# TravisWheelerLab/sufr

Hardware: AMD Instinct MI355X
Metric: suffixes sorted/sec (SA+LCP) (higher is better)
Workload: dtype u8 text / u32 indices / u64 packed keys; 1 GPU; syn_human 3.1 Gb stand-in for GRCh38, --dna --ignore-softmask -n 256 (BASELINE configs[3]); text_len=3100000001, num_suffixes=1500223556, parallelism=prefix-bucket shards x1, bits_per_char=3, radix_passes=5, digit_bits=15, levels=7, deep_records=58357696, placement_trials=3

## Files before the change

include/sufr_hip.h:

```cpp
#ifndef SUFR_HIP_H
#define SUFR_HIP_H

#include <stddef.h>
#include <stdint.h>

#ifdef __cplusplus
extern "C" {
#endif

#define SUFR_HIP_ABI_VERSION 3

#define SUFR_OUTFILE_VERSION 6
#define SUFR_SENTINEL_CHARACTER '$'

#define SUFR_HIP_FLAG_DNA              (1u << 0)
#define SUFR_HIP_FLAG_ALLOW_AMBIGUITY  (1u << 1)
#define SUFR_HIP_FLAG_IGNORE_SOFTMASK  (1u << 2)
#define SUFR_HIP_FLAG_RAW_TEXT         (1u << 3)

#define SUFR_HIP_OK              0
#define SUFR_HIP_E_INVALID      -1
#define SUFR_HIP_E_NO_DEVICE    -2
#define SUFR_HIP_E_HIP          -3
#define SUFR_HIP_E_NOMEM        -4
#define SUFR_HIP_E_CAPACITY     -5
#define SUFR_HIP_E_UNSUPPORTED  -6
#define SUFR_HIP_E_IO           -7
#define SUFR_HIP_E_CONFLICT     -8
#define SUFR_HIP_E_SEED_MASK    -9

typedef struct sufr_hip_ctx sufr_hip_ctx;

typedef struct sufr_hip_stats {
    uint64_t text_len;
    uint64_t num_suffixes;
    uint32_t alphabet_size;
    uint32_t bits_per_char;
    uint32_t chars_per_key;
    uint32_t digit_bits;
    uint32_t num_passes;
    uint32_t num_levels;
    uint64_t num_large_groups;
    uint64_t deep_records;
    uint32_t top_lo, top_hi;
    uint32_t partition_workgroups;
    uint32_t partition_variant;
    float ms_total;
    float ms_normalize;
    float ms_hist_text;
    float ms_partition;
    float ms_passes;
    float ms_finish;
    float ms_deep;
    float host_read_s;
    float host_build_s;
    float host_write_s;
    uint32_t num_exceptions;
    float ms_exceptions;
    uint64_t num_reinserted;
} sufr_hip_stats;

int  sufr_hip_abi_version(void);
int  sufr_hip_device_count(void);
sufr_hip_ctx *sufr_hip_create(int device_id);
void sufr_hip_destroy(sufr_hip_ctx *ctx);
const char *sufr_hip_last_error(const sufr_hip_ctx *ctx);
int  sufr_hip_set_stream(sufr_hip_ctx *ctx, void *hip_stream);
int  sufr_hip_synchronize(sufr_hip_ctx *ctx);
int  sufr_hip_set_window(sufr_hip_ctx *ctx, uint64_t window, uint64_t margin);
int  sufr_hip_set_window_retry(sufr_hip_ctx *ctx, uint64_t widest_margin);
uint64_t sufr_hip_window_repairs(const sufr_hip_ctx *ctx);
int  sufr_hip_set_array_budget(sufr_hip_ctx *ctx, uint64_t bytes);
int  sufr_hip_set_overlap_min(sufr_hip_ctx *ctx, uint64_t min_records);
int  sufr_hip_overlapped(const sufr_hip_ctx *ctx);
uint64_t sufr_hip_doublings(const sufr_hip_ctx *ctx);
int  sufr_hip_set_exc_max_affected(sufr_hip_ctx *ctx, uint64_t max_affected);
int  sufr_hip_exc_retry(const sufr_hip_ctx *ctx);
uint64_t sufr_hip_exc_taken(const sufr_hip_ctx *ctx);

int sufr_hip_normalize(const uint8_t *in, uint8_t *out, uint64_t n, int ignore_softmask);

int sufr_hip_sort_device_u32(sufr_hip_ctx *ctx, const void *d_text, uint64_t n, uint32_t flags,
                             uint64_t max_query_len, const char *seed_mask,
                             uint64_t num_partitions, uint64_t random_seed,
                             uint32_t shard_index, uint32_t num_shards,
                             void *d_sa, void *d_lcp, uint64_t cap,
                             uint64_t *num_suffixes_out, sufr_hip_stats *stats);
int sufr_hip_sort_device_u64(sufr_hip_ctx *ctx, const void *d_text, uint64_t n, uint32_t flags,
                             uint64_t max_query_len, const char *seed_mask,
                             uint64_t num_partitions, uint64_t random_seed,
                             uint32_t shard_index, uint32_t num_shards,
                             void *d_sa, void *d_lcp, uint64_t cap,
                             uint64_t *num_suffixes_out, sufr_hip_stats *stats);

int sufr_hip_stitch_device_u32(sufr_hip_ctx *ctx, uint64_t n, const uint64_t *d_bounds, uint32_t shard_index,
                               uint32_t num_shards, void *d_lcp);
int sufr_hip_stitch_device_u64(sufr_hip_ctx *ctx, uint64_t n, const uint64_t *d_bounds, uint32_t shard_index,
                               uint32_t num_shards, void *d_lcp);

int sufr_hip_build_u32(sufr_hip_ctx *ctx, const uint8_t *text, uint64_t n, uint32_t flags,
                       uint64_t max_query_len, const char *seed_mask,
                       uint64_t num_partitions, uint64_t random_seed,
                       uint8_t *norm_text_out, uint32_t *sa_out, uint32_t *lcp_out, uint64_t cap,
                       uint64_t *num_suffixes_out, sufr_hip_stats *stats);
int sufr_hip_build_u64(sufr_hip_ctx *ctx, const uint8_t *text, uint64_t n, uint32_t flags,
                       uint64_t max_query_len, const char *seed_mask,
                       uint64_t num_partitions, uint64_t random_seed,
                       uint8_t *norm_text_out, uint64_t *sa_out, uint64_t *lcp_out, uint64_t cap,
                       uint64_t *num_suffixes_out, sufr_hip_stats *stats);

uint64_t sufr_hip_lcp_pair(const uint8_t *norm_text, uint64_t n, uint64_t a, uint64_t b);

typedef struct sufr_sequence_data {
    uint8_t  *seq;
    uint64_t  seq_len;
    uint64_t *start_positions;
    char    **sequence_names;
    uint64_t  num_sequences;
} sufr_sequence_data;
int  sufr_read_sequence_file(const char *path, uint8_t sequence_delimiter, sufr_sequence_data *out,
                             char *err, size_t errlen);
void sufr_sequence_data_free(sufr_sequence_data *d);

int sufr_write_file(const char *path, int is_dna, int allow_ambiguity, int ignore_softmask,
                    const uint8_t *norm_text, uint64_t text_len, int index_width,
                    const void *sa, const void *lcp, uint64_t num_suffixes,
                    int has_max_query_len, uint64_t max_query_len, const char *seed_mask,
                    const uint64_t *sequence_starts, uint64_t num_sequences,
                    const char *const *sequence_names, char *err, size_t errlen);

typedef struct sufr_create_args {
    const char *input;
    const char *output;
    uint64_t    num_partitions;
    int         has_max_query_len;
    uint64_t    max_query_len;
    int         is_dna;
    int         allow_ambiguity;
    int         ignore_softmask;
    uint8_t     sequence_delimiter;
    const char *seed_mask;
    uint64_t    random_seed;
} sufr_create_args;
int sufr_hip_create_file(sufr_hip_ctx *ctx, const sufr_create_args *args, char *path_out,
                         size_t path_out_len, sufr_hip_stats *stats);
int sufr_hip_create_from_sequence(sufr_hip_ctx *ctx, const sufr_sequence_data *seq,
                                  const sufr_create_args *args, char *path_out, size_t path_out_len,
                                  sufr_hip_stats *stats);


typedef struct sufr_shard_info {
    uint64_t num_suffixes;
    uint64_t first_suffix;
    uint64_t last_suffix;
} sufr_shard_info;
int sufr_hip_shard_build(sufr_hip_ctx *ctx, const sufr_sequence_data *seq, const sufr_create_args *args,
                         uint32_t shard_index, uint32_t num_shards, sufr_shard_info *info, sufr_hip_stats *stats);
int sufr_write_frame(const char *outfile, const sufr_sequence_data *seq, const sufr_create_args *args,
// ... 15 lines not shown
```

sufr_amd/_lib.py:

```python
from __future__ import annotations

import ctypes as C
import os
import subprocess
from pathlib import Path

CSRC = Path(__file__).resolve().parent / "csrc"
LIB_PATH = CSRC / "_build" / "libsufr_hip.so"
if os.environ.get("SUFR_AMD_PROBES_LIB"):
    import sys as _sys
    LIB_PATH = CSRC / "_build" / "libsufr_hip_probes.so"
    print(f"sufr_amd: SUFR_AMD_PROBES_LIB is set -- loading the PROBES build {LIB_PATH.name} (tuning knobs from "
          "SUFR_PROBE_*; for profiling only)", file=_sys.stderr)
CLI_PATH = CSRC / "_build" / "sufr"
HOST_ASAN = bool(os.environ.get("SUFR_AMD_HOST_ASAN_LIB"))
if HOST_ASAN:
    import sys as _sys
    LIB_PATH = CSRC / "_build" / "libsufr_host_asan.so"
    CLI_PATH = CSRC / "_build" / "sufr_host_asan"
    print(f"sufr_amd: SUFR_AMD_HOST_ASAN_LIB is set -- loading the host-only sanitizer build {LIB_PATH.name} (no device code)",
          file=_sys.stderr)


class SufrHipError(RuntimeError):
    def __init__(self, code: int, message: str):
        super().__init__(f"{message} (sufr_hip error {code})")
        self.code = code
        self.message = message


class Stats(C.Structure):
    _fields_ = [
        ("text_len", C.c_uint64), ("num_suffixes", C.c_uint64),
        ("alphabet_size", C.c_uint32), ("bits_per_char", C.c_uint32), ("chars_per_key", C.c_uint32),
        ("digit_bits", C.c_uint32), ("num_passes", C.c_uint32), ("num_levels", C.c_uint32),
        ("num_large_groups", C.c_uint64), ("deep_records", C.c_uint64),
        ("top_lo", C.c_uint32), ("top_hi", C.c_uint32), ("partition_workgroups", C.c_uint32),
        ("partition_variant", C.c_uint32),
        ("ms_total", C.c_float), ("ms_normalize", C.c_float), ("ms_hist_text", C.c_float),
        ("ms_partition", C.c_float), ("ms_passes", C.c_float), ("ms_finish", C.c_float),
        ("ms_deep", C.c_float), ("host_read_s", C.c_float), ("host_build_s", C.c_float),
        ("host_write_s", C.c_float),
        ("num_exceptions", C.c_uint32), ("ms_exceptions", C.c_float), ("num_reinserted", C.c_uint64),
    ]

    def as_dict(self):
        return {n: getattr(self, n) for n, _ in self._fields_}


class SequenceData(C.Structure):
    _fields_ = [("seq", C.POINTER(C.c_uint8)), ("seq_len", C.c_uint64),
                ("start_positions", C.POINTER(C.c_uint64)), ("sequence_names", C.POINTER(C.c_char_p)),
                ("num_sequences", C.c_uint64)]


class CreateArgs(C.Structure):
    _fields_ = [("input", C.c_char_p), ("output", C.c_char_p), ("num_partitions", C.c_uint64),
                ("has_max_query_len", C.c_int), ("max_query_len", C.c_uint64), ("is_dna", C.c_int),
                ("allow_ambiguity", C.c_int), ("ignore_softmask", C.c_int), ("sequence_delimiter", C.c_uint8),
                ("seed_mask", C.c_char_p), ("random_seed", C.c_uint64)]


class ShardInfo(C.Structure):
    _fields_ = [("num_suffixes", C.c_uint64), ("first_suffix", C.c_uint64), ("last_suffix", C.c_uint64)]


FLAG_DNA, FLAG_ALLOW_AMBIGUITY, FLAG_IGNORE_SOFTMASK, FLAG_RAW_TEXT = 1, 2, 4, 8
FLAG_NO_PREFIX_TABLE = 0x100
FLAG_SA_U64 = 0x200

EXPORTS = [
    "sufr_hip_abi_version", "sufr_hip_device_count", "sufr_hip_create", "sufr_hip_destroy",
    "sufr_hip_last_error", "sufr_hip_set_stream", "sufr_hip_synchronize", "sufr_hip_set_window", "sufr_hip_set_window_retry", "sufr_hip_set_array_budget", "sufr_hip_window_repairs", "sufr_hip_set_overlap_min", "sufr_hip_overlapped", "sufr_hip_doublings", "sufr_hip_set_exc_max_affected", "sufr_hip_exc_retry", "sufr_hip_exc_taken", "sufr_hip_normalize", "sufr_hip_sort_device_u32",
    "sufr_hip_sort_device_u64", "sufr_hip_stitch_device_u32", "sufr_hip_stitch_device_u64", "sufr_hip_build_u32", "sufr_hip_build_u64", "sufr_hip_lcp_pair",
    "sufr_read_sequence_file", "sufr_sequence_data_free", "sufr_write_file", "sufr_hip_create_file", "sufr_hip_create_from_sequence",
    "sufr_hip_shard_build", "sufr_write_frame", "sufr_hip_shard_write", "sufr_hip_create_from_sequence_multi",
    "sufr_hip_create_file_multi",
]
QUERY_EXPORTS = [
    "sufr_file_open", "sufr_file_close", "sufr_file_metadata", "sufr_file_text", "sufr_file_seed_mask",
    "sufr_file_suffix_array", "sufr_file_lcp_array", "sufr_file_suffix", "sufr_file_lcp", "sufr_file_sequence_start",
    "sufr_file_sequence_name", "sufr_file_sequence_of", "sufr_file_search", "sufr_file_search_batch",
    "sufr_hip_index_load", "sufr_hip_index_wrap", "sufr_hip_index_free", "sufr_hip_index_width", "sufr_hip_search_batch",
    "sufr_hip_search_batch_device", "sufr_hip_locate_batch_device",
]
MATCH_EXPORTS = [
    "sufr_file_matching_stats", "sufr_file_smems", "sufr_hip_matching_stats_device", "sufr_hip_smems_device", "sufr_hip_smems",
]
MEM_EXPORTS = ["sufr_file_mems", "sufr_hip_mems_device", "sufr_hip_mems"]
MEM_BOTH_STRANDS = 0x1
APPROX_EXPORTS = ["sufr_file_approx", "sufr_hip_approx_device", "sufr_hip_approx"]
APPROX_BOTH_STRANDS = 0x1
EDIT_EXPORTS = ["sufr_file_edit", "sufr_hip_edit_device", "sufr_hip_edit"]
EDIT_BOTH_STRANDS = 0x1
EDIT_LOCAL_MINIMA = 0x2
ALIGN_EXPORTS = ["sufr_file_edit_trace", "sufr_hip_edit_trace_device", "sufr_hip_edit_trace", "sufr_hip_set_trace_scratch"]
KMER_EXPORTS = ["sufr_file_kmers", "sufr_file_unique_lengths", "sufr_hip_kmers_device", "sufr_hip_unique_lengths_device",
                "sufr_hip_set_kmer_tile"]
KMER_BY_POSITION = 0x1


class KmerStats(C.Structure):
    _fields_ = [("whole", C.c_uint64), ("distinct", C.c_uint64), ("unique", C.c_uint64), ("max_count", C.c_uint64)]

    def as_dict(self):
        return {n: int(getattr(self, n)) for n, _ in self._fields_}


REPEAT_EXPORTS = ["sufr_file_repeats", "sufr_hip_repeats_device", "sufr_hip_set_repeat_tile"]
REPEAT_KINDS = {"branching": 0, "maximal": 1, "super": 2, "supermaximal": 2}


class RepeatStats(C.Structure):
    _fields_ = [("records", C.c_uint64), ("longest", C.c_uint64), ("longest_rank", C.c_uint64), ("max_count", C.c_uint64)]

    def as_dict(self):
        return {n: int(getattr(self, n)) for n, _ in self._fields_}


LZ_EXPORTS = ["sufr_file_lpf", "sufr_file_lz", "sufr_hip_lpf_device", "sufr_hip_lz_device", "sufr_hip_set_lz_tile"]


class LzStats(C.Structure):
    _fields_ = [("factors", C.c_uint64), ("literals", C.c_uint64), ("longest", C.c_uint64), ("longest_start", C.c_uint64)]

    def as_dict(self):
        return {n: int(getattr(self, n)) for n, _ in self._fields_}


SHARED_EXPORTS = ["sufr_file_shared", "sufr_file_common", "sufr_hip_shared_device", "sufr_hip_common_device"]


class SharedStats(C.Structure):
    _fields_ = [("records", C.c_uint64), ("longest", C.c_uint64), ("longest_rank", C.c_uint64), ("max_count", C.c_uint64),
                ("max_seqs", C.c_uint64)]

    def as_dict(self):
        return {n: int(getattr(self, n)) for n, _ in self._fields_}


BWT_EXPORTS = ["sufr_file_bwt", "sufr_file_bwt_runs", "sufr_file_lf", "sufr_hip_bwt_device", "sufr_hip_bwt_runs_device", "sufr_hip_lf_device",
               "sufr_hip_set_bwt_tile"]


class BwtStats(C.Structure):
    _fields_ = [("runs", C.c_uint64), ("records", C.c_uint64), ("longest", C.c_uint64), ("longest_rank", C.c_uint64)]

    def as_dict(self):
        return {n: int(getattr(self, n)) for n, _ in self._fields_}


class FileMeta(C.Structure):
    _fields_ = [("version", C.c_uint8), ("is_dna", C.c_uint8), ("allow_ambiguity", C.c_uint8),
                ("ignore_softmask", C.c_uint8), ("index_width", C.c_int),
                ("text_len", C.c_uint64), ("text_pos", C.c_uint64), ("suffix_array_pos", C.c_uint64),
                ("lcp_pos", C.c_uint64), ("len_suffixes", C.c_uint64), ("max_query_len", C.c_uint64),
                ("num_sequences", C.c_uint64), ("seed_mask_len", C.c_uint64), ("file_size", C.c_uint64),
                ("modified", C.c_int64)]

_lib = None


def build_extension(verbose: bool = False) -> Path:
    r = subprocess.run(["make", "-C", str(CSRC)] + (["asan"] if HOST_ASAN else []), capture_output=True, text=True)
    if r.returncode != 0:
        raise RuntimeError("building libsufr_hip.so failed:\n" + r.stdout + r.stderr)
    if verbose:
        print(r.stdout)
    return LIB_PATH


def lib() -> C.CDLL:
    global _lib
    if _lib is not None:
        return _lib
    if not LIB_PATH.exists():
        raise SufrHipError(-2, f"{LIB_PATH} is missing: build it with sufr_amd.build_extension() "
                               "(there is no CPU fallback)")
    import sys
    if "torch" not in sys.modules and not HOST_ASAN:
        try:
            import torch
        except ImportError:
            pass
    L = C.CDLL(str(LIB_PATH))
    vp, u64, u32, cp = C.c_void_p, C.c_uint64, C.c_uint32, C.c_char_p
    L.sufr_hip_abi_version.restype = C.c_int
    L.sufr_hip_device_count.restype = C.c_int
    L.sufr_hip_create.argtypes = [C.c_int]; L.sufr_hip_create.restype = vp
    L.sufr_hip_destroy.argtypes = [vp]; L.sufr_hip_destroy.restype = None
    L.sufr_hip_last_error.argtypes = [vp]; L.sufr_hip_last_error.restype = cp
    L.sufr_hip_set_stream.argtypes = [vp, vp]; L.sufr_hip_set_stream.restype = C.c_int
    L.sufr_hip_synchronize.argtypes = [vp]; L.sufr_hip_synchronize.restype = C.c_int
    L.sufr_hip_set_window.argtypes = [vp, u64, u64]; L.sufr_hip_set_window.restype = C.c_int
    L.sufr_hip_set_window_retry.argtypes = [vp, u64]; L.sufr_hip_set_window_retry.restype = C.c_int
    L.sufr_hip_set_array_budget.argtypes = [vp, u64]; L.sufr_hip_set_array_budget.restype = C.c_int
    L.sufr_hip_window_repairs.argtypes = [vp]; L.sufr_hip_window_repairs.restype = u64
    L.sufr_hip_set_overlap_min.argtypes = [vp, u64]; L.sufr_hip_set_overlap_min.restype = C.c_int
    L.sufr_hip_overlapped.argtypes = [vp]; L.sufr_hip_overlapped.restype = C.c_int
    L.sufr_hip_doublings.argtypes = [vp]; L.sufr_hip_doublings.restype = u64
    L.sufr_hip_set_exc_max_affected.argtypes = [vp, u64]; L.sufr_hip_set_exc_max_affected.restype = C.c_int
    L.sufr_hip_exc_retry.argtypes = [vp]; L.sufr_hip_exc_retry.restype = C.c_int
    L.sufr_hip_exc_taken.argtypes = [vp]; L.sufr_hip_exc_taken.restype = u64
    L.sufr_hip_normalize.argtypes = [vp, vp, u64, C.c_int]; L.sufr_hip_normalize.restype = C.c_int
    dev_sig = [vp, vp, u64, u32, u64, cp, u64, u64, u32, u32, vp, vp, u64, C.POINTER(u64), C.POINTER(Stats)]
    L.sufr_hip_sort_device_u32.argtypes = dev_sig; L.sufr_hip_sort_device_u32.restype = C.c_int
    L.sufr_hip_sort_device_u64.argtypes = dev_sig; L.sufr_hip_sort_device_u64.restype = C.c_int
    host_sig = [vp, vp, u64, u32, u64, cp, u64, u64, vp, vp, vp, u64, C.POINTER(u64), C.POINTER(Stats)]
    L.sufr_hip_build_u32.argtypes = host_sig; L.sufr_hip_build_u32.restype = C.c_int
    L.sufr_hip_build_u64.argtypes = host_sig; L.sufr_hip_build_u64.restype = C.c_int
    L.sufr_hip_lcp_pair.argtypes = [vp, u64, u64, u64]; L.sufr_hip_lcp_pair.restype = u64
    L.sufr_hip_stitch_device_u32.argtypes = [vp, u64, vp, u32, u32, vp]; L.sufr_hip_stitch_device_u32.restype = C.c_int
    L.sufr_hip_stitch_device_u64.argtypes = [vp, u64, vp, u32, u32, vp]; L.sufr_hip_stitch_device_u64.restype = C.c_int
    L.sufr_read_sequence_file.argtypes = [cp, C.c_uint8, C.POINTER(SequenceData), cp, C.c_size_t]
    L.sufr_read_sequence_file.restype = C.c_int
    L.sufr_sequence_data_free.argtypes = [C.POINTER(SequenceData)]; L.sufr_sequence_data_free.restype = None
    L.sufr_write_file.argtypes = [cp, C.c_int, C.c_int, C.c_int, vp, u64, C.c_int, vp, vp, u64, C.c_int, u64, cp,
                                  vp, u64, C.POINTER(cp), cp, C.c_size_t]
    L.sufr_write_file.restype = C.c_int
    L.sufr_hip_create_file.argtypes = [vp, C.POINTER(CreateArgs), cp, C.c_size_t, C.POINTER(Stats)]
    L.sufr_hip_create_file.restype = C.c_int
    L.sufr_hip_create_from_sequence.argtypes = [vp, C.POINTER(SequenceData), C.POINTER(CreateArgs), cp, C.c_size_t,
                                                C.POINTER(Stats)]
    L.sufr_hip_create_from_sequence.restype = C.c_int
    L.sufr_hip_shard_build.argtypes = [vp, C.POINTER(SequenceData), C.POINTER(CreateArgs), u32, u32,
                                       C.POINTER(ShardInfo), C.POINTER(Stats)]
    L.sufr_hip_shard_build.restype = C.c_int
    L.sufr_write_frame.argtypes = [cp, C.POINTER(SequenceData), C.POINTER(CreateArgs), u64, cp, C.c_size_t]
    L.sufr_write_frame.restype = C.c_int
    L.sufr_hip_shard_write.argtypes = [vp, C.POINTER(SequenceData), C.POINTER(CreateArgs), cp, u64, u64, u64, C.c_int,
                                       u64, C.c_int]
    L.sufr_hip_shard_write.restype = C.c_int
    L.sufr_hip_create_from_sequence_multi.argtypes = [C.POINTER(vp), C.c_int, C.POINTER(SequenceData),
                                                      C.POINTER(CreateArgs), cp, C.c_size_t, C.POINTER(Stats)]
    L.sufr_hip_create_from_sequence_multi.restype = C.c_int
    L.sufr_hip_create_file_multi.argtypes = [C.POINTER(vp), C.c_int, C.POINTER(CreateArgs), cp, C.c_size_t,
                                             C.POINTER(Stats)]
    L.sufr_hip_create_file_multi.restype = C.c_int
    L.sufr_file_open.argtypes = [cp, C.POINTER(vp), cp, C.c_size_t]; L.sufr_file_open.restype = C.c_int
    L.sufr_file_close.argtypes = [vp]; L.sufr_file_close.restype = None
    L.sufr_file_metadata.argtypes = [vp, C.POINTER(FileMeta)]; L.sufr_file_metadata.restype = C.c_int
    for name in ("sufr_file_text", "sufr_file_seed_mask", "sufr_file_suffix_array", "sufr_file_lcp_array"):
        getattr(L, name).argtypes = [vp]; getattr(L, name).restype = vp
    for name in ("sufr_file_suffix", "sufr_file_lcp", "sufr_file_sequence_start", "sufr_file_sequence_of"):
        getattr(L, name).argtypes = [vp, u64]; getattr(L, name).restype = u64
    L.sufr_file_sequence_name.argtypes = [vp, u64]; L.sufr_file_sequence_name.restype = cp
    L.sufr_file_search.argtypes = [vp, cp, C.c_size_t, C.c_int, u64, C.POINTER(u64), C.POINTER(u64)]
    L.sufr_file_search.restype = C.c_int
    L.sufr_file_search_batch.argtypes = [vp, vp, vp, u64, C.c_int, u64, vp, vp, C.c_int]; L.sufr_file_search_batch.restype = C.c_int
    L.sufr_hip_index_load.argtypes = [vp, vp, C.POINTER(vp)]; L.sufr_hip_index_load.restype = C.c_int
    L.sufr_hip_index_wrap.argtypes = [vp, vp, u64, vp, u64, u32, u64, cp, C.POINTER(vp)]; L.sufr_hip_index_wrap.restype = C.c_int
    L.sufr_hip_index_free.argtypes = [vp]; L.sufr_hip_index_free.restype = None
    L.sufr_hip_index_width.argtypes = [vp]; L.sufr_hip_index_width.restype = C.c_int
    L.sufr_hip_search_batch.argtypes = [vp, vp, vp, vp, u64, C.c_int, u64, vp, vp]; L.sufr_hip_search_batch.restype = C.c_int
    L.sufr_hip_search_batch_device.argtypes = [vp, vp, vp, vp, u64, C.c_int, u64, vp, vp]
    L.sufr_hip_search_batch_device.restype = C.c_int
    L.sufr_hip_locate_batch_device.argtypes = [vp, vp, vp, vp, u64, u64, vp, vp, u64, C.POINTER(u64)]
    L.sufr_hip_locate_batch_device.restype = C.c_int
    L.sufr_file_matching_stats.argtypes = [vp, vp, vp, u64, vp, C.c_int]; L.sufr_file_matching_stats.restype = C.c_int
    L.sufr_file_smems.argtypes = [vp, vp, vp, u64, u32, u64, vp, vp, vp, vp, vp, C.POINTER(u64), C.c_int]
    L.sufr_file_smems.restype = C.c_int
    L.sufr_hip_matching_stats_device.argtypes = [vp, vp, vp, vp, u64, vp]; L.sufr_hip_matching_stats_device.restype = C.c_int
    L.sufr_hip_smems_device.argtypes = [vp, vp, vp, vp, u64, u32, vp, u64, vp, vp, vp, vp, vp, C.POINTER(u64)]
    L.sufr_hip_smems_device.restype = C.c_int
    L.sufr_hip_smems.argtypes = [vp, vp, vp, vp, u64, u32, u64, vp, vp, vp, vp, vp, C.POINTER(u64)]
    L.sufr_hip_smems.restype = C.c_int
    L.sufr_file_mems.argtypes = [vp, vp, vp, u64, u32, u64, u32, u64, vp, vp, vp, vp, vp, C.POINTER(u64), C.c_int]
    L.sufr_file_mems.restype = C.c_int
    L.sufr_hip_mems_device.argtypes = [vp, vp, vp, vp, u64, u32, u64, u32, u64, vp, vp, vp, vp, vp, C.POINTER(u64)]
    L.sufr_hip_mems_device.restype = C.c_int
    L.sufr_hip_mems.argtypes = [vp, vp, vp, vp, u64, u32, u64, u32, u64, vp, vp, vp, vp, vp, C.POINTER(u64)]
    L.sufr_hip_mems.restype = C.c_int
    L.sufr_file_approx.argtypes = [vp, vp, vp, u64, u32, u64, u32, u64, vp, vp, vp, vp, C.POINTER(u64), C.c_int]
    L.sufr_file_approx.restype = C.c_int
    L.sufr_hip_approx_device.argtypes = [vp, vp, vp, vp, u64, u32, u64, u32, u64, vp, vp, vp, vp, C.POINTER(u64)]
    L.sufr_hip_approx_device.restype = C.c_int
    L.sufr_hip_approx.argtypes = [vp, vp, vp, vp, u64, u32, u64, u32, u64, vp, vp, vp, vp, C.POINTER(u64)]
    L.sufr_hip_approx.restype = C.c_int
    L.sufr_file_edit.argtypes = [vp, vp, vp, u64, u32, u64, u32, u64, vp, vp, vp, vp, C.POINTER(u64), C.c_int]
    L.sufr_file_edit.restype = C.c_int
    L.sufr_hip_edit_device.argtypes = [vp, vp, vp, vp, u64, u32, u64, u32, u64, vp, vp, vp, vp, C.POINTER(u64)]
    L.sufr_hip_edit_device.restype = C.c_int
    L.sufr_hip_edit.argtypes = [vp, vp, vp, vp, u64, u32, u64, u32, u64, vp, vp, vp, vp, C.POINTER(u64)]
# ... 24 lines not shown
    L.sufr_hip_set_lz_tile.argtypes = [vp, u64, u64]; L.sufr_hip_set_lz_tile.restype = C.c_int
    L.sufr_file_shared.argtypes = [vp, u32, u64, u64, u64, u64, u64, u64, vp, vp, vp, vp, C.POINTER(u64), C.POINTER(SharedStats), C.c_int]
    L.sufr_file_shared.restype = C.c_int
    L.sufr_file_common.argtypes = [vp, vp, C.c_int]; L.sufr_file_common.restype = C.c_int
    L.sufr_hip_shared_device.argtypes = [vp, vp, vp, vp, u64, u32, u64, u64, u64, u64, u64, u64, vp, vp, vp, vp, C.POINTER(u64),
                                         C.POINTER(SharedStats)]
    L.sufr_hip_shared_device.restype = C.c_int
    L.sufr_hip_common_device.argtypes = [vp, vp, vp, vp, u64, vp]; L.sufr_hip_common_device.restype = C.c_int
    L.sufr_file_bwt.argtypes = [vp, vp, vp, C.c_int]; L.sufr_file_bwt.restype = C.c_int
    L.sufr_file_bwt_runs.argtypes = [vp, u64, u64, vp, vp, vp, vp, C.POINTER(u64), C.POINTER(BwtStats), C.c_int]; L.sufr_file_bwt_runs.restype = C.c_int
    L.sufr_file_lf.argtypes = [vp, vp, C.c_int]; L.sufr_file_lf.restype = C.c_int
    L.sufr_hip_bwt_device.argtypes = [vp, vp, vp, vp]; L.sufr_hip_bwt_device.restype = C.c_int
    L.sufr_hip_bwt_runs_device.argtypes = [vp, vp, u64, u64, vp, vp, vp, vp, C.POINTER(u64), C.POINTER(BwtStats)]
    L.sufr_hip_bwt_runs_device.restype = C.c_int
    L.sufr_hip_lf_device.argtypes = [vp, vp, vp]; L.sufr_hip_lf_device.restype = C.c_int
    L.sufr_hip_set_bwt_tile.argtypes = [vp, u64]; L.sufr_hip_set_bwt_tile.restype = C.c_int
    _lib = L
    return L


class Context:

    def __init__(self, device: int = 0):
        L = lib()
        self._h = L.sufr_hip_create(device)
        if not self._h:
            raise SufrHipError(-2, L.sufr_hip_last_error(None).decode())
        self.device = device

    def close(self):
        if getattr(self, "_h", None):
            lib().sufr_hip_destroy(self._h)
            self._h = None

    def __del__(self):
        try:
            self.close()
        except Exception:
            pass

    def check(self, rc: int):
        if rc != 0:
            raise SufrHipError(rc, lib().sufr_hip_last_error(self._h).decode())

    def set_window(self, window: int = 0, margin: int = 0):
        self.check(lib().sufr_hip_set_window(self._h, window, margin))

    def set_window_retry(self, widest_margin: int = 0):
        self.check(lib().sufr_hip_set_window_retry(self._h, widest_margin))

    def set_array_budget(self, nbytes: int = 0):
        self.check(lib().sufr_hip_set_array_budget(self._h, nbytes))

    def set_trace_scratch(self, nbytes: int = 0):
        self.check(lib().sufr_hip_set_trace_scratch(self._h, nbytes))

    def set_kmer_tile(self, ranks: int = 0):
        self.check(lib().sufr_hip_set_kmer_tile(self._h, ranks))

    def set_repeat_tile(self, ranks: int = 0):
        self.check(lib().sufr_hip_set_repeat_tile(self._h, ranks))

    def set_lz_tile(self, ranks: int = 0, positions: int = 0):
        self.check(lib().sufr_hip_set_lz_tile(self._h, ranks, positions))

    def set_bwt_tile(self, ranks: int = 0):
        self.check(lib().sufr_hip_set_bwt_tile(self._h, ranks))

    @property
    def window_repairs(self) -> int:
        return int(lib().sufr_hip_window_repairs(self._h))

    def set_overlap_min(self, min_records: int = 0):
        self.check(lib().sufr_hip_set_overlap_min(self._h, min_records))

    @property
    def overlapped(self) -> int:
        return int(lib().sufr_hip_overlapped(self._h))

    @property
    def doublings(self) -> int:
        return int(lib().sufr_hip_doublings(self._h))

    def set_exc_max_affected(self, max_affected: int = 0):
        self.check(lib().sufr_hip_set_exc_max_affected(self._h, max_affected))

    @property
    def exc_retry(self) -> int:
        return int(lib().sufr_hip_exc_retry(self._h))

    @property
    def exc_taken(self) -> int:
        return int(lib().sufr_hip_exc_taken(self._h))

    def synchronize(self):
        self.check(lib().sufr_hip_synchronize(self._h))

    @property
    def handle(self):
        return self._h
```

sufr_amd/csrc/sufr_capi.inc:

```

struct sufr_hip_ctx {
    sufr::Pipeline pl;
    uint64_t wide_window = 0, wide_margin = 0;
    uint64_t array_budget = 0;
    sufr::DevBuf wtext, wsa, wlcp, wblk;
    sufr::DevBuf mtmp, mpoff, mbytes;
    sufr::DevBuf xq, xoff, xlo, xhi, xcand, xsum;
    sufr::DevBuf ecnt, ekeys, ekeys2, ehist;
    sufr::DevBuf tsc, trows, tmisc;
    uint64_t trace_scratch = 0;
    sufr::DevBuf kbits, ksum, kstarts;
    std::vector<uint64_t> kmer_starts;
    uint32_t kmer_tile = 0;
    sufr::DevBuf rell, rpyr, rbits, rsum;
    uint32_t repeat_tile = 0;
    sufr::DevBuf lzpyr, lzarr, lztab, lzsum;
    uint32_t lz_rank_tile = 0, lz_pos_tile = 0;
    sufr::DevBuf bwtbytes, bwtsum, bwttab;
    uint32_t bwt_tile = 0;
    sufr::DevBuf shkeys, shhist, shpre, shsum;
    bool wide(uint64_t n) const { return n >= sufr::SUFR_MAX_TEXT_LEN || (wide_window && n > wide_window); }
};

#include <atomic>
// ... 170 lines not shown
        delete ctx;
        return nullptr;
    }
    return ctx;
}

extern "C" void sufr_io_release_ctx_(const sufr_hip_ctx* ctx);

void sufr_hip_destroy(sufr_hip_ctx* ctx)
{
    if (!ctx) return;
    sufr_io_release_ctx_(ctx);
    (void)hipSetDevice(ctx->pl.device);
    for (sufr::DevBuf* b : {&ctx->wtext, &ctx->wsa, &ctx->wlcp, &ctx->wblk, &ctx->mtmp, &ctx->mpoff, &ctx->mbytes,
                            &ctx->xq, &ctx->xoff, &ctx->xlo, &ctx->xhi, &ctx->xcand, &ctx->xsum,
                            &ctx->ecnt, &ctx->ekeys, &ctx->ekeys2, &ctx->ehist, &ctx->tsc, &ctx->trows, &ctx->tmisc,
                            &ctx->kbits, &ctx->ksum, &ctx->kstarts, &ctx->rell, &ctx->rpyr, &ctx->rbits, &ctx->rsum,
                            &ctx->lzpyr, &ctx->lzarr, &ctx->lztab, &ctx->lzsum,
                            &ctx->bwtbytes, &ctx->bwtsum, &ctx->bwttab,
                            &ctx->shkeys, &ctx->shhist, &ctx->shpre, &ctx->shsum}) ctx->pl.release(*b);
    ctx->pl.destroy();
    delete ctx;
}

const char* sufr_hip_last_error(const sufr_hip_ctx* ctx)
{
    return ctx ? ctx->pl.err.c_str() : g_create_error.c_str();
}

int sufr_hip_is_wide_(const sufr_hip_ctx* ctx, uint64_t n) { return ctx && ctx->wide(n) ? 1 : 0; }
int sufr_hip_ctx_device_(const sufr_hip_ctx* ctx) { return ctx ? ctx->pl.device : -1; }

void sufr_hip_set_error_(sufr_hip_ctx* ctx, const char* msg)
{
    if (ctx) ctx->pl.set_error(msg ? msg : "");
}

int sufr_hip_set_stream(sufr_hip_ctx* ctx, void* hip_stream)
{
    if (!ctx) return SUFR_HIP_E_INVALID;
    if (ctx->pl.own_stream && ctx->pl.stream) (void)hipStreamDestroy(ctx->pl.stream);
    ctx->pl.own_stream = false;
    ctx->pl.stream = (hipStream_t)hip_stream;
    return 0;
}

int sufr_hip_set_window(sufr_hip_ctx* ctx, uint64_t window, uint64_t margin)
{
    if (!ctx) return SUFR_HIP_E_INVALID;
    if (window && window < 16) { ctx->pl.set_error("window below 16 positions"); return SUFR_HIP_E_INVALID; }
    ctx->wide_window = window;
    ctx->wide_margin = margin;
    return 0;
}

int sufr_hip_set_array_budget(sufr_hip_ctx* ctx, uint64_t bytes)
{
    if (!ctx) return SUFR_HIP_E_INVALID;
    ctx->array_budget = bytes;
    return 0;
}

uint64_t sufr_hip_array_budget_(const sufr_hip_ctx* ctx) { return ctx ? ctx->array_budget : 0; }

int sufr_hip_set_window_retry(sufr_hip_ctx* ctx, uint64_t widest_margin)
{
    if (!ctx) return SUFR_HIP_E_INVALID;
    ctx->pl.opt_wide_retry = widest_margin;
    return 0;
}

uint64_t sufr_hip_window_repairs(const sufr_hip_ctx* ctx) { return ctx ? ctx->pl.wide_orphans : 0; }

int sufr_hip_set_overlap_min(sufr_hip_ctx* ctx, uint64_t min_records)
{
    if (!ctx) return SUFR_HIP_E_INVALID;
    ctx->pl.opt_overlap_min = min_records;
    return 0;
}

int sufr_hip_overlapped(const sufr_hip_ctx* ctx) { return ctx ? (int)ctx->pl.last_overlapped : 0; }
uint64_t sufr_hip_doublings(const sufr_hip_ctx* ctx) { return ctx ? ctx->pl.last_doublings : 0; }

int sufr_hip_set_exc_max_affected(sufr_hip_ctx* ctx, uint64_t max_affected)
{
    if (!ctx) return SUFR_HIP_E_INVALID;
    if (max_affected > sufr::Pipeline::EXC_MAX_AFFECTED_DEFAULT) {
        ctx->pl.set_error("max_affected " + std::to_string(max_affected) + " > 2^22: the whole-text sort of the affected suffixes and its buffers are sized for 2^22");
        return SUFR_HIP_E_INVALID;
    }
    ctx->pl.opt_exc_max_affected = max_affected;
    return 0;
}

int sufr_hip_exc_retry(const sufr_hip_ctx* ctx) { return ctx ? (int)ctx->pl.last_exc_retry : 0; }
uint64_t sufr_hip_exc_taken(const sufr_hip_ctx* ctx) { return ctx ? ctx->pl.last_exc_taken : 0; }

int sufr_hip_synchronize(sufr_hip_ctx* ctx)
{
    if (!ctx) return SUFR_HIP_E_INVALID;
    if (hipSetDevice(ctx->pl.device) != hipSuccess || hipStreamSynchronize(ctx->pl.stream) != hipSuccess) {
        ctx->pl.set_error("hipStreamSynchronize failed");
        return SUFR_HIP_E_HIP;
    }
    return 0;
}

int sufr_hip_sort_device_u32(sufr_hip_ctx* ctx, const void* d_text, uint64_t n, uint32_t flags,
                             uint64_t max_query_len, const char* seed_mask, uint64_t num_partitions,
                             uint64_t random_seed, uint32_t shard_index, uint32_t num_shards, void* d_sa,
                             void* d_lcp, uint64_t cap, uint64_t* num_suffixes_out, sufr_hip_stats* stats)
{
    (void)num_partitions; (void)random_seed;
    if (!ctx) return SUFR_HIP_E_INVALID;
    ctx->pl.err.clear();
    int rc = take_options(ctx, max_query_len, seed_mask);
    if (rc) return rc;
    if (ctx->wide(n)) {
        if (n >= 0xFFFFFFFFull) { ctx->pl.set_error("text_len >= 2^32 - 1 takes the u64 entry points (suffix_array.rs:461)"); return SUFR_HIP_E_INVALID; }
        if (num_shards == 0 || shard_index >= num_shards) { ctx->pl.set_error("bad shard index"); return SUFR_HIP_E_INVALID; }
        ctx->pl.wide_shard_index = shard_index; ctx->pl.wide_num_shards = num_shards;
        rc = sufr::sort_device_wide<uint32_t>(ctx->pl, d_text, n, flags, ctx->wide_window, ctx->wide_margin, (uint32_t*)d_sa,
                                              (uint32_t*)d_lcp, cap, num_suffixes_out, stats, ctx->wtext, ctx->wsa, ctx->wlcp, ctx->wblk);
        ctx->pl.wide_shard_index = 0; ctx->pl.wide_num_shards = 1;
        return rc;
    }
    return ctx->pl.sort_device_u32(d_text, n, flags, shard_index, num_shards, (uint32_t*)d_sa, (uint32_t*)d_lcp,
                                   cap, num_suffixes_out, stats);
}

int sufr_hip_sort_device_u64(sufr_hip_ctx* ctx, const void* d_text, uint64_t n, uint32_t flags,
                             uint64_t max_query_len, const char* seed_mask, uint64_t num_partitions,
                             uint64_t random_seed, uint32_t shard_index, uint32_t num_shards, void* d_sa,
                             void* d_lcp, uint64_t cap, uint64_t* num_suffixes_out, sufr_hip_stats* stats)
{
    (void)num_partitions; (void)random_seed;
    if (!ctx) return SUFR_HIP_E_INVALID;
    ctx->pl.err.clear();
    int rc = take_options(ctx, max_query_len, seed_mask);
    if (rc) return rc;
    sufr::Pipeline& pl = ctx->pl;
    if (ctx->wide(n)) {
        if (num_shards == 0 || shard_index >= num_shards) { pl.set_error("bad shard index"); return SUFR_HIP_E_INVALID; }
        pl.wide_shard_index = shard_index; pl.wide_num_shards = num_shards;
        rc = sufr::sort_device_wide<uint64_t>(pl, d_text, n, flags, ctx->wide_window, ctx->wide_margin, (uint64_t*)d_sa,
                                              (uint64_t*)d_lcp, cap, num_suffixes_out, stats, ctx->wtext, ctx->wsa, ctx->wlcp, ctx->wblk);
        pl.wide_shard_index = 0; pl.wide_num_shards = 1;
        return rc;
    }
    if (hipSetDevice(pl.device) != hipSuccess) { pl.set_error("hipSetDevice failed"); return SUFR_HIP_E_HIP; }
    uint64_t cap32 = cap < n ? cap : n;
    if ((rc = pl.ensure(pl.sa32, cap32 * 4 + 4))) return rc;
    if ((rc = pl.ensure(pl.lcp32, cap32 * 4 + 4))) return rc;
    uint64_t s = 0;
    rc = pl.sort_device_u32(d_text, n, flags, shard_index, num_shards, (uint32_t*)pl.sa32.p, (uint32_t*)pl.lcp32.p,
                            cap32, &s, stats);
    if (num_suffixes_out) *num_suffixes_out = s;
    if (rc) return rc;
    if (s) {
        hipLaunchKernelGGL(sufr::k_widen, dim3((uint32_t)((s + 255) / 256)), dim3(256), 0, pl.stream,
                           (const uint32_t*)pl.sa32.p, (uint64_t*)d_sa, s);
        hipLaunchKernelGGL(sufr::k_widen, dim3((uint32_t)((s + 255) / 256)), dim3(256), 0, pl.stream,
                           (const uint32_t*)pl.lcp32.p, (uint64_t*)d_lcp, s);
        if (hipStreamSynchronize(pl.stream) != hipSuccess) { pl.set_error("widen failed"); return SUFR_HIP_E_HIP; }
    }
    return 0;
// ... 244 lines not shown
```

sufr_amd/csrc/sufr_host_stubs.cpp:

```cpp
#include <stdint.h>
#include <stddef.h>
#include <string>

#include <hip/hip_runtime_api.h>

#include "../../include/sufr_hip.h"
#include "../../include/sufr_query.h"
#include "../../include/sufr_match.h"
#include "../../include/sufr_mem.h"
#include "../../include/sufr_approx.h"
#include "../../include/sufr_edit.h"
#include "../../include/sufr_align.h"
#include "../../include/sufr_kmer.h"
#include "../../include/sufr_repeat.h"
#include "../../include/sufr_lz.h"
#include "../../include/sufr_shared.h"
#include "../../include/sufr_bwt.h"

struct sufr_hip_ctx { std::string err; };

namespace {
const char* const NO_DEVICE = "host-only sanitizer build: no HIP device (libsufr_host_asan.so has no device code)";
int no_device(sufr_hip_ctx* ctx) { if (ctx) ctx->err = NO_DEVICE; return SUFR_HIP_E_NO_DEVICE; }
}

extern "C" {

hipError_t hipHostMalloc(void** p, size_t, unsigned int) { if (p) *p = nullptr; return hipErrorNoDevice; }
hipError_t hipHostFree(void*) { return hipSuccess; }
const char* hipGetErrorString(hipError_t) { return "no device"; }
hipError_t hipMalloc(void** p, size_t) { if (p) *p = nullptr; return hipErrorNoDevice; }
hipError_t hipFree(void*) { return hipSuccess; }
hipError_t hipMemcpy(void*, const void*, size_t, hipMemcpyKind) { return hipErrorNoDevice; }
hipError_t hipMemcpyAsync(void*, const void*, size_t, hipMemcpyKind, hipStream_t) { return hipErrorNoDevice; }
hipError_t hipSetDevice(int) { return hipErrorNoDevice; }
hipError_t hipStreamCreateWithFlags(hipStream_t* s, unsigned int) { if (s) *s = nullptr; return hipErrorNoDevice; }
hipError_t hipStreamDestroy(hipStream_t) { return hipSuccess; }
hipError_t hipStreamSynchronize(hipStream_t) { return hipErrorNoDevice; }

int sufr_hip_abi_version(void) { return SUFR_HIP_ABI_VERSION; }
int sufr_hip_device_count(void) { return 0; }
sufr_hip_ctx* sufr_hip_create(int) { return nullptr; }
void sufr_hip_destroy(sufr_hip_ctx* ctx) { delete ctx; }
const char* sufr_hip_last_error(const sufr_hip_ctx* ctx) { return ctx ? ctx->err.c_str() : NO_DEVICE; }
int sufr_hip_set_stream(sufr_hip_ctx* ctx, void*) { return no_device(ctx); }
int sufr_hip_synchronize(sufr_hip_ctx* ctx) { return no_device(ctx); }
int sufr_hip_set_window(sufr_hip_ctx* ctx, uint64_t, uint64_t) { return no_device(ctx); }
int sufr_hip_set_window_retry(sufr_hip_ctx* ctx, uint64_t) { return no_device(ctx); }
int sufr_hip_set_array_budget(sufr_hip_ctx* ctx, uint64_t) { return no_device(ctx); }
uint64_t sufr_hip_window_repairs(const sufr_hip_ctx*) { return 0; }
int sufr_hip_set_overlap_min(sufr_hip_ctx* ctx, uint64_t) { return no_device(ctx); }
int sufr_hip_overlapped(const sufr_hip_ctx*) { return 0; }
uint64_t sufr_hip_doublings(const sufr_hip_ctx*) { return 0; }
int sufr_hip_set_exc_max_affected(sufr_hip_ctx* ctx, uint64_t) { return no_device(ctx); }
int sufr_hip_exc_retry(const sufr_hip_ctx*) { return 0; }
uint64_t sufr_hip_exc_taken(const sufr_hip_ctx*) { return 0; }
int sufr_hip_sort_device_u32(sufr_hip_ctx* ctx, const void*, uint64_t, uint32_t, uint64_t, const char*, uint64_t, uint64_t,
                             uint32_t, uint32_t, void*, void*, uint64_t, uint64_t*, sufr_hip_stats*) { return no_device(ctx); }
int sufr_hip_sort_device_u64(sufr_hip_ctx* ctx, const void*, uint64_t, uint32_t, uint64_t, const char*, uint64_t, uint64_t,
                             uint32_t, uint32_t, void*, void*, uint64_t, uint64_t*, sufr_hip_stats*) { return no_device(ctx); }
int sufr_hip_stitch_device_u32(sufr_hip_ctx* ctx, uint64_t, const uint64_t*, uint32_t, uint32_t, void*) { return no_device(ctx); }
int sufr_hip_stitch_device_u64(sufr_hip_ctx* ctx, uint64_t, const uint64_t*, uint32_t, uint32_t, void*) { return no_device(ctx); }
int sufr_hip_build_u32(sufr_hip_ctx* ctx, const uint8_t*, uint64_t, uint32_t, uint64_t, const char*, uint64_t, uint64_t, uint8_t*,
                       uint32_t*, uint32_t*, uint64_t, uint64_t*, sufr_hip_stats*) { return no_device(ctx); }
int sufr_hip_build_u64(sufr_hip_ctx* ctx, const uint8_t*, uint64_t, uint32_t, uint64_t, const char*, uint64_t, uint64_t, uint8_t*,
                       uint64_t*, uint64_t*, uint64_t, uint64_t*, sufr_hip_stats*) { return no_device(ctx); }

void sufr_hip_set_error_(sufr_hip_ctx* ctx, const char* msg) { if (ctx) ctx->err = msg ? msg : ""; }
int sufr_hip_is_wide_(const sufr_hip_ctx*, uint64_t) { return 0; }
int sufr_hip_ctx_device_(const sufr_hip_ctx*) { return -1; }
uint64_t sufr_hip_array_budget_(const sufr_hip_ctx*) { return 0; }
void sufr_hip_release_build_arrays_(sufr_hip_ctx*, int) {}
void sufr_hip_release_wide_arrays_(sufr_hip_ctx*) {}
int sufr_hip_build_resident_(sufr_hip_ctx* ctx, const uint8_t*, uint64_t, uint32_t, uint64_t, const char*, uint32_t, uint32_t,
                             uint64_t*, sufr_hip_stats*, int*, const void**, const void**, const void**) { return no_device(ctx); }
int sufr_hip_resident_ends_(sufr_hip_ctx* ctx, uint64_t, uint64_t*, uint64_t*) { return no_device(ctx); }
int sufr_hip_resident_stitch_(sufr_hip_ctx* ctx, uint64_t, uint64_t, uint64_t*) { return no_device(ctx); }
int sufr_hip_resident_arrays_(sufr_hip_ctx* ctx, int*, const void**, const void**, const void**) { return no_device(ctx); }

struct sufr_hip_index { int unused; };
int sufr_hip_index_load(sufr_hip_ctx* ctx, const sufr_file*, sufr_hip_index** out) { if (out) *out = nullptr; return no_device(ctx); }
int sufr_hip_index_wrap(sufr_hip_ctx* ctx, const void*, uint64_t, const void*, uint64_t, uint32_t, uint64_t, const char*,
                        sufr_hip_index** out) { if (out) *out = nullptr; return no_device(ctx); }
void sufr_hip_index_free(sufr_hip_index*) {}
int sufr_hip_index_width(const sufr_hip_index*) { return 0; }
int sufr_hip_search_batch(sufr_hip_ctx* ctx, const sufr_hip_index*, const uint8_t*, const uint64_t*, uint64_t, int, uint64_t,
                          uint64_t*, uint64_t*) { return no_device(ctx); }
int sufr_hip_search_batch_device(sufr_hip_ctx* ctx, const sufr_hip_index*, const void*, const void*, uint64_t, int, uint64_t,
                                 void*, void*) { return no_device(ctx); }
int sufr_hip_locate_batch_device(sufr_hip_ctx* ctx, const sufr_hip_index*, const void*, const void*, uint64_t, uint64_t, void*,
                                 void*, uint64_t, uint64_t*) { return no_device(ctx); }


int sufr_hip_matching_stats_device(sufr_hip_ctx* ctx, const sufr_hip_index*, const void*, const void*, uint64_t, void*) { return no_device(ctx); }
int sufr_hip_smems_device(sufr_hip_ctx* ctx, const sufr_hip_index*, const void*, const void*, uint64_t, uint32_t, void*, uint64_t, void*,
                          void*, void*, void*, void*, uint64_t* total_out) { if (total_out) *total_out = 0; return no_device(ctx); }
int sufr_hip_smems(sufr_hip_ctx* ctx, const sufr_hip_index*, const uint8_t*, const uint64_t*, uint64_t, uint32_t, uint64_t, uint64_t*,
                   uint32_t*, uint32_t*, uint64_t*, uint64_t*, uint64_t* total_out) { if (total_out) *total_out = 0; return no_device(ctx); }

int sufr_hip_mems_device(sufr_hip_ctx* ctx, const sufr_hip_index*, const void*, const void*, uint64_t, uint32_t, uint64_t, uint32_t,
                         uint64_t, void*, void*, void*, void*, void*, uint64_t* total_out) { if (total_out) *total_out = 0; return no_device(ctx); }
int sufr_hip_mems(sufr_hip_ctx* ctx, const sufr_hip_index*, const uint8_t*, const uint64_t*, uint64_t, uint32_t, uint64_t, uint32_t, uint64_t,
                  uint64_t*, uint32_t*, uint8_t*, uint32_t*, uint64_t*, uint64_t* total_out) { if (total_out) *total_out = 0; return no_device(ctx); }

int sufr_hip_approx_device(sufr_hip_ctx* ctx, const sufr_hip_index*, const void*, const void*, uint64_t, uint32_t, uint64_t, uint32_t,
                           uint64_t, void*, void*, void*, void*, uint64_t* total_out) { if (total_out) *total_out = 0; return no_device(ctx); }
int sufr_hip_approx(sufr_hip_ctx* ctx, const sufr_hip_index*, const uint8_t*, const uint64_t*, uint64_t, uint32_t, uint64_t, uint32_t, uint64_t,
                    uint64_t*, uint8_t*, uint64_t*, uint8_t*, uint64_t* total_out) { if (total_out) *total_out = 0; return no_device(ctx); }

int sufr_hip_edit_device(sufr_hip_ctx* ctx, const sufr_hip_index*, const void*, const void*, uint64_t, uint32_t, uint64_t, uint32_t,
                         uint64_t, void*, void*, void*, void*, uint64_t* total_out) { if (total_out) *total_out = 0; return no_device(ctx); }
int sufr_hip_edit(sufr_hip_ctx* ctx, const sufr_hip_index*, const uint8_t*, const uint64_t*, uint64_t, uint32_t, uint64_t, uint32_t, uint64_t,
                  uint64_t*, uint8_t*, uint64_t*, uint8_t*, uint64_t* total_out) { if (total_out) *total_out = 0; return no_device(ctx); }

int sufr_hip_edit_trace_device(sufr_hip_ctx* ctx, const sufr_hip_index*, const void*, const void*, uint64_t, uint64_t, const void*, const void*,
                               const void*, const void*, uint64_t, void*, void*, void*, uint64_t* total_out) { if (total_out) *total_out = 0; return no_device(ctx); }
int sufr_hip_edit_trace(sufr_hip_ctx* ctx, const sufr_hip_index*, const uint8_t*, const uint64_t*, uint64_t, uint64_t, const uint64_t*, const uint8_t*,
                        const uint64_t*, const uint8_t*, uint64_t, uint64_t*, uint64_t*, uint32_t*, uint64_t* total_out) { if (total_out) *total_out = 0; return no_device(ctx); }
int sufr_hip_set_trace_scratch(sufr_hip_ctx* ctx, uint64_t) { return no_device(ctx); }

int sufr_hip_kmers_device(sufr_hip_ctx* ctx, const sufr_hip_index*, const void*, const uint64_t*, uint64_t, uint64_t, uint32_t, uint64_t, void*,
                          void*, sufr_kmer_stats* stats_out) { if (stats_out) *stats_out = sufr_kmer_stats{0, 0, 0, 0}; return no_device(ctx); }
int sufr_hip_unique_lengths_device(sufr_hip_ctx* ctx, const sufr_hip_index*, const void*, const uint64_t*, uint64_t, uint32_t, void*) { return no_device(ctx); }
int sufr_hip_set_kmer_tile(sufr_hip_ctx* ctx, uint64_t) { return no_device(ctx); }

int sufr_hip_repeats_device(sufr_hip_ctx* ctx, const sufr_hip_index*, const void*, const uint64_t*, uint64_t, uint32_t, uint64_t, uint64_t, uint64_t,
                            uint64_t, void*, void*, void*, uint64_t* total_out, sufr_repeat_stats* stats_out)
{
    if (total_out) *total_out = 0;
    if (stats_out) *stats_out = sufr_repeat_stats{0, 0, 0, 0};
    return no_device(ctx);
}
int sufr_hip_set_repeat_tile(sufr_hip_ctx* ctx, uint64_t) { return no_device(ctx); }

int sufr_hip_lpf_device(sufr_hip_ctx* ctx, const sufr_hip_index*, const void*, const uint64_t*, uint64_t, void*, void*) { return no_device(ctx); }
int sufr_hip_lz_device(sufr_hip_ctx* ctx, const sufr_hip_index*, const void*, const uint64_t*, uint64_t, uint64_t, void*, void*, void*,
// ... 30 lines not shown
```

sufr_amd/csrc/sufr_kernels.hip:

```cpp

#include <hip/hip_runtime.h>
#include <stdint.h>
#include <type_traits>

#include "sufr_device.h"
#include "sufr_runkey.h"

namespace sufr {
#ifdef SUFR_HIP_PROBES
__device__ unsigned long long g_phase[3][16];
#define SUFR_STAMP(acc, i) { const unsigned long long t__ = __builtin_amdgcn_s_memtime(); acc[i] += t__ - stamp__; stamp__ = t__; }
#define SUFR_STAMP_DECL(n) unsigned long long ph__[n] = {}; unsigned long long stamp__ = __builtin_amdgcn_s_memtime();
#define SUFR_STAMP_FLUSH(k, n) if ((threadIdx.x & 63u) == 0 && (threadIdx.x >> 6) == gridDim.y * 0 + (blockDim.x >> 6) - 1) { for (int i__ = 0; i__ < n; i__++) atomicAdd(&g_phase[k][i__], ph__[i__]); }
#else
#define SUFR_STAMP(acc, i)
#define SUFR_STAMP_DECL(n)
#define SUFR_STAMP_FLUSH(k, n)
#endif
}

namespace sufr {

static constexpr int WAVE = 64;
static_assert(RUN_TILE == (uint32_t)TILE, "run-end table granularity");

__device__ __forceinline__ uint32_t lane_id() { return threadIdx.x & 63u; }
__device__ __forceinline__ uint64_t rec_key(const Rec& r) { return ((uint64_t)r.khi << 32) | r.klo; }
__device__ __forceinline__ Rec make_rec(uint64_t key, uint32_t idx)
{
    Rec r; r.klo = (uint32_t)key; r.khi = (uint32_t)(key >> 32); r.idx = idx;
    return r;
}

#define SUFR_LDS_VOLATILE(T, p) ((__attribute__((address_space(3))) volatile T*)(p))

__device__ __forceinline__ uint64_t shfl64(uint64_t v, int src)
{
    uint32_t lo = (uint32_t)v, hi = (uint32_t)(v >> 32);
    lo = __shfl(lo, src, WAVE);
    hi = __shfl(hi, src, WAVE);
    return ((uint64_t)hi << 32) | lo;
}
__device__ __forceinline__ uint64_t shfl64_xor(uint64_t v, int m)
{
    uint32_t lo = (uint32_t)v, hi = (uint32_t)(v >> 32);
    lo = __shfl_xor(lo, m, WAVE);
    hi = __shfl_xor(hi, m, WAVE);
    return ((uint64_t)hi << 32) | lo;
}
__device__ __forceinline__ uint64_t shfl64_up1(uint64_t v)
{
    uint32_t lo = (uint32_t)v, hi = (uint32_t)(v >> 32);
    lo = __shfl_up(lo, 1, WAVE);
    hi = __shfl_up(hi, 1, WAVE);
    return ((uint64_t)hi << 32) | lo;
}

__global__ void __launch_bounds__(256)
k_normalize_bytehist(const uint8_t* __restrict__ in, uint8_t* __restrict__ out, uint64_t n,
                     int normalize, int ignore_softmask, unsigned long long* __restrict__ ghist,
                     uint32_t* __restrict__ first_end, uint64_t* __restrict__ run_ends,
                     uint64_t* __restrict__ tile_any)
{
    __shared__ uint32_t h[256 * 32];
    __shared__ uint8_t s_first[256 + 4];
    __shared__ uint32_t s_min;
    __shared__ uint32_t s_any[2];
    for (int i = threadIdx.x; i < 256 * 32; i += 256) h[i] = 0;
    __syncthreads();
    const uint32_t copy = threadIdx.x & 31u;
    const uint64_t ntiles = (n + TILE - 1) / TILE;
    auto norm = [&](uint32_t b) -> uint32_t {
        if (normalize && b >= 97u && b <= 122u) b = ignore_softmask ? 78u : (b & 0x5Fu);
        return b;
    };
    for (uint64_t tile = blockIdx.x; tile < ntiles; tile += gridDim.x) {
        const uint64_t p0 = tile * TILE + (uint64_t)threadIdx.x * 16;
        uint32_t by[17];
        if (threadIdx.x == 0) { s_min = 0xffffffffu; s_any[0] = 0; s_any[1] = 0; }
        if (p0 + 16 <= n) {
            uint4 w = *reinterpret_cast<const uint4*>(in + p0);
            uint32_t ws[4] = {w.x, w.y, w.z, w.w};
#pragma unroll
            for (int k = 0; k < 4; k++) {
                uint32_t y = 0;
#pragma unroll
                for (int j = 0; j < 4; j++) {
                    uint32_t b = norm((ws[k] >> (8 * j)) & 0xffu);
                    by[4 * k + j] = b;
// ... 1231 lines not shown
    uint64_t m = M0 & (~0ull >> (63 - slot));
    return m ? 63 - __clzll(m) : -1;
}
__device__ __forceinline__ int mask_next_set(uint64_t M0, uint64_t M1, int slot, int none)
{
    if (slot < 64) {
        uint64_t m = slot == 63 ? 0ull : (M0 & (~0ull << (slot + 1)));
        if (m) return __builtin_ctzll(m);
        return M1 ? 64 + __builtin_ctzll(M1) : none;
    }
    uint64_t m = slot == 127 ? 0ull : (M1 & (~0ull << (slot - 63)));
    return m ? 64 + __builtin_ctzll(m) : none;
}

#ifdef SUFR_HIP_PROBES
__device__ unsigned long long g_walk_stats[4];
#endif

static constexpr uint32_t WALK_CAP = 4096;

__device__ __forceinline__ uint64_t walk_lcp(const uint8_t* __restrict__ text, uint64_t n, uint64_t a, uint64_t b,
                                             uint64_t cap = ~0ull)
{
    uint64_t lim = n - (a > b ? a : b);
    if (lim > cap) lim = cap;
    uint64_t k = 0;
    while (k + 64 <= lim) {
        uint64_t x[8];
#pragma unroll
        for (int u = 0; u < 8; u++) x[u] = load_u64_unaligned(text + a + k + 8 * u) ^ load_u64_unaligned(text + b + k + 8 * u);
#pragma unroll
        for (int u = 0; u < 8; u++)
            if (x[u]) return k + 8 * u + (uint64_t)(__builtin_ctzll(x[u]) >> 3);
        k += 64;
    }
    while (k < lim && text[a + k] == text[b + k]) k++;
    return k;
}

__device__ __forceinline__ uint64_t walk_lcp_packed(const uint8_t* __restrict__ packed, int bits, uint64_t n, uint64_t a, uint64_t b,
                                                    uint64_t cap, uint32_t& ca, uint32_t& cb)
{
    uint64_t lim = n - (a > b ? a : b);
    if (lim > cap) lim = cap;
    const uint32_t K = div_by_bits(64u, bits);
    uint64_t k = 0;
    ca = cb = 0;
    while (k < lim) {
        const uint64_t oa = (a + k) * (uint64_t)bits, ob = (b + k) * (uint64_t)bits;
        const uint8_t* pa = packed + (oa >> 3);
        const uint8_t* pb = packed + (ob >> 3);
        uint64_t wa[3], wb[3];
#pragma unroll
        for (int u = 0; u < 3; u++) { wa[u] = __builtin_bswap64(load_u64_unaligned(pa + 8 * u)); wb[u] = __builtin_bswap64(load_u64_unaligned(pb + 8 * u)); }
        const uint32_t sa = (uint32_t)(oa & 7u), sb = (uint32_t)(ob & 7u);
        const uint32_t K3raw = div_by_bits(192u - 7u - 2u * K * (uint32_t)bits, bits);
        const uint32_t K3 = K3raw < K ? K3raw : K;
#pragma unroll
        for (int j = 0; j < 3; j++) {
            const uint32_t qa = sa + (uint32_t)j * K * (uint32_t)bits, qb = sb + (uint32_t)j * K * (uint32_t)bits;
            const uint32_t ra = qa & 63u, rb = qb & 63u;
            const uint64_t ha = qa < 64u ? wa[0] : (qa < 128u ? wa[1] : wa[2]), la = qa < 64u ? wa[1] : (qa < 128u ? wa[2] : 0ull);
            const uint64_t hb = qb < 64u ? wb[0] : (qb < 128u ? wb[1] : wb[2]), lb = qb < 64u ? wb[1] : (qb < 128u ? wb[2] : 0ull);
            const uint64_t va = ra ? ((ha << ra) | (la >> (64u - ra))) : ha;
            const uint64_t vb = rb ? ((hb << rb) | (lb >> (64u - rb))) : hb;
            const uint32_t Kj = j < 2 ? K : K3;
            const int sparej = 64 - (int)Kj * bits;
            if (Kj == 0u) break;
            const uint64_t x = (va ^ vb) >> sparej;
            if (x) {
                const uint32_t c = div_by_bits((uint32_t)__builtin_clzll(x << sparej), bits);
                k += c;
                if (k >= lim) return lim;
                const int sh = 64 - (int)(c + 1u) * bits;
                ca = (uint32_t)(va >> sh) & ((1u << bits) - 1u);
                cb = (uint32_t)(vb >> sh) & ((1u << bits) - 1u);
                return k;
            }
            k += Kj;
            if (k >= lim) return lim;
        }
    }
    return lim;
}

static constexpr uint64_t WALK_MAX = (1ull << 62) - 1;
__device__ __forceinline__ uint64_t walk_key(bool is_ref, bool below, uint64_t L)
{
    return is_ref ? (1ull << 62) : (below ? L : ((2ull << 62) | (WALK_MAX - L)));
}
__device__ __forceinline__ uint64_t walk_key_len(uint64_t k)
{
    const uint32_t cls = (uint32_t)(k >> 62);
    return cls == 0 ? k : (cls == 1 ? (uint64_t)WALK_CAP : WALK_MAX - (k & WALK_MAX));
}
__device__ __forceinline__ uint32_t walk_key_common(uint64_t a, uint64_t b)
{
    const uint64_t la = walk_key_len(a), lb = walk_key_len(b);
    return (uint32_t)(la < lb ? la : lb);
}

template <bool DEEP, bool TIES_OUT, bool PLANNED>
__global__ void __launch_bounds__(256, 5)
k_finish(const uint64_t* __restrict__ keys, const uint32_t* idxs,
         const uint32_t* __restrict__ segs, const uint32_t* __restrict__ opos,
         const uint32_t* __restrict__ segdepth, uint32_t m,
         const uint8_t* __restrict__ text, uint64_t n, RunTable R,
         const uint16_t* __restrict__ glut, KeyParams kp, int sorted_bits,
         uint32_t* __restrict__ SA, uint32_t* __restrict__ LCP,
         uint32_t* __restrict__ wl_flag, uint32_t* __restrict__ wl_head,
         uint32_t* idx_writeback, unsigned long long* __restrict__ wmask, uint32_t* __restrict__ wcnt,
         uint32_t ncross)
{
#ifdef SUFR_HIP_PROBES
    const uint32_t popts = ncross >> 29;
    ncross &= 0x1fffffffu;
#else
    constexpr uint32_t popts = 0;
#endif
    __shared__ uint64_t sh_key[4][128];
    __shared__ uint32_t sh_idx[4][128];
    __shared__ uint32_t sh_gid[4][128];
    __shared__ uint16_t s_lut[256];
    for (int i = threadIdx.x; i < 256; i += 256) s_lut[i] = glut[i];
    __syncthreads();

    const uint32_t wave = (blockIdx.x * 256 + threadIdx.x) >> 6;
    if (PLANNED ? (wave >= ncross) : ((uint64_t)wave * 128 >= m)) return;
    uint64_t base64 = PLANNED ? (uint64_t)wl_head[wave] : (uint64_t)wave * 128;
    const uint32_t wcount = PLANNED ? wl_flag[wave] : 128u;
    const int wv = threadIdx.x >> 6;
    auto sk = SUFR_LDS_VOLATILE(uint64_t, sh_key[wv]);
    auto si = SUFR_LDS_VOLATILE(uint32_t, sh_idx[wv]);
    auto sg = SUFR_LDS_VOLATILE(uint32_t, sh_gid[wv]);
    const int ln = (int)lane_id();
    const bool whole = sorted_bits == 0;
    const int group_shift = whole ? 0 : 64 - sorted_bits;
    uint32_t own_limit = 128u;
    if (DEEP && !TIES_OUT && !PLANNED) {
        const uint32_t b0 = (uint32_t)base64;
        const uint32_t a0 = b0 + (uint32_t)ln, a1 = b0 + 64u + (uint32_t)ln;
        const bool v0 = a0 < m, v1 = a1 < m;
        const uint64_t pk0 = v0 ? keys[a0] : ~0ull, pk1 = v1 ? keys[a1] : ~0ull;
        const uint32_t ps_0 = v0 ? segs[a0] : 0xffffffffu, ps_1 = v1 ? segs[a1] : 0xffffffffu;
        uint64_t q0 = shfl64_up1(pk0), q1 = shfl64_up1(pk1);
        uint32_t r0 = __shfl_up(ps_0, 1, WAVE), r1 = __shfl_up(ps_1, 1, WAVE);
        const uint64_t l0k = shfl64(pk0, 63); const uint32_t l0s = __shfl(ps_0, 63, WAVE);
        if (ln == 0) {
            q1 = l0k; r1 = l0s;
            if (b0 > 0) { q0 = keys[b0 - 1]; r0 = segs[b0 - 1]; }
        }
        const bool e0 = !v0 || (ln == 0 && b0 == 0) || r0 != ps_0 || (!whole && (q0 >> group_shift) != (pk0 >> group_shift));
        const bool e1 = !v1 || r1 != ps_1 || (!whole && (q1 >> group_shift) != (pk1 >> group_shift));
        const uint64_t E0 = __ballot(e0), E1 = __ballot(e1);
        const uint32_t first = E0 ? (uint32_t)__builtin_ctzll(E0) : (E1 ? 64u + (uint32_t)__builtin_ctzll(E1) : 128u);
        if (first >= 128u || (uint64_t)b0 + first >= m) {
            if (ln == 0) wl_flag[wave] = 0u;
            return;
        }
        base64 += first;
        own_limit = 128u - first;
    }
    const uint32_t base = (uint32_t)base64;
    const uint32_t j0 = base + ln, j1 = base + 64 + ln;
    const bool in0 = j0 < m && (uint32_t)ln < wcount, in1 = j1 < m && 64u + (uint32_t)ln < wcount;

// ... 47 lines not shown
    }
    if (!PLANNED) {
        const uint64_t any_large = __ballot(lg0 || lg1);
        if (ln == 0) wl_flag[wave] = any_large ? 1u : 0u;
    }
    bool act0 = small0 && !(h0 && nx0 == ln + 1);
    bool act1 = small1 && !(h1 && nx1 == 64 + ln + 1);
    uint32_t gid0 = act0 ? (uint32_t)g0 : (0x10000u | (uint32_t)ln);
    uint32_t gid1 = act1 ? (uint32_t)g1 : (0x10000u | (uint32_t)(64 + ln));
    uint32_t ge0 = act0 ? (uint32_t)nx0 : 0u, ge1 = act1 ? (uint32_t)nx1 : 0u;

    int ktype = DEEP ? 1 : 0;
    uint32_t extra0 = 0, extra1 = 0;
    const uint64_t max_round = n + 8;
    bool lt0 = false, lt1 = false;
    SUFR_STAMP_DECL(8)
    for (uint64_t round = 0; __ballot(act0 || act1) != 0ull && round < max_round; round++) {
        SUFR_STAMP(ph__, 0)
#ifdef SUFR_HIP_PROBES
        ph__[5] += 1000;
#endif
        sk[ln] = k0; sk[64 + ln] = k1;
        uint32_t np0 = (uint32_t)ln, np1 = (uint32_t)(64 + ln);
        auto rank_in = [&](uint64_t kme, uint32_t me, uint32_t g, uint32_t e) -> uint32_t {
            uint32_t cnt = 0, t = g;
            for (; t + 4u <= e; t += 4u) {
                const uint64_t a = sk[t], b = sk[t + 1], c = sk[t + 2], d = sk[t + 3];
                cnt += (a < kme || (a == kme && t < me)) ? 1u : 0u;
                cnt += (b < kme || (b == kme && t + 1u < me)) ? 1u : 0u;
                cnt += (c < kme || (c == kme && t + 2u < me)) ? 1u : 0u;
                cnt += (d < kme || (d == kme && t + 3u < me)) ? 1u : 0u;
            }
            for (; t < e; t++) {
                const uint64_t a = sk[t];
                cnt += (a < kme || (a == kme && t < me)) ? 1u : 0u;
            }
            return cnt;
        };
        if (act0) np0 = gid0 + rank_in(k0, (uint32_t)ln, gid0, ge0);
        if (act1) np1 = gid1 + rank_in(k1, (uint32_t)(64 + ln), gid1, ge1);
        if (act0) { sk[np0] = k0; si[np0] = i0; }
        if (act1) { sk[np1] = k1; si[np1] = i1; }
        if (act0) { k0 = sk[ln]; i0 = si[ln]; }
        if (act1) { k1 = sk[64 + ln]; i1 = si[64 + ln]; }
        uint64_t q0 = (act0 && ln > 0) ? sk[ln - 1] : 0ull;
        uint64_t q1 = act1 ? sk[63 + ln] : 0ull;
        const bool same0 = act0 && (uint32_t)ln > gid0;
        const bool same1 = act1 && (uint32_t)(64 + ln) > gid1;
        const bool tie0 = same0 && q0 == k0, tie1 = same1 && q1 == k1;
        auto common = [&](uint64_t a, uint64_t b2) -> uint32_t {
            return ktype == 0 ? plain_key_common(a, b2, kp.b, kp.K) : (ktype == 1 ? run_key_common(a, b2, kp.b) : walk_key_common(a, b2));
        };
        auto advance = [&](uint64_t k) -> uint32_t {
            return ktype == 0 ? (uint32_t)kp.K : (ktype == 1 ? run_key_advance(k, 64, kp.b) : (uint32_t)walk_key_len(k));
        };
        if (same0 && !tie0) lcp0 = dd0 + common(q0, k0);
        if (same1 && !tie1) lcp1 = dd1 + common(q1, k1);
        const uint64_t T0 = __ballot(tie0), T1 = __ballot(tie1);
        const int ng0 = mask_prev_set(~T0, ~T1, ln), ng1 = mask_prev_set(~T0, ~T1, 64 + ln);
        const bool s0n = ln < 63 ? ((T0 >> (ln + 1)) & 1ull) : (T1 & 1ull);
        const bool s1n = ln < 63 ? ((T1 >> (ln + 1)) & 1ull) : false;
        act0 = act0 && (tie0 || s0n);
        act1 = act1 && (tie1 || s1n);
        gid0 = act0 ? (uint32_t)ng0 : (0x10000u | (uint32_t)ln);
        gid1 = act1 ? (uint32_t)ng1 : (0x10000u | (uint32_t)(64 + ln));
        ge0 = (uint32_t)mask_next_set(~T0, ~T1, ln, 128);
        ge1 = (uint32_t)mask_next_set(~T0, ~T1, 64 + ln, 128);
        lt0 = tie0; lt1 = tie1;
        if (TIES_OUT) break;
        SUFR_STAMP(ph__, 1)
        const uint64_t TN0 = (T0 >> 1) | (T1 << 63), TN1 = T1 >> 1;
        const uint64_t TNN0 = (T0 >> 2) | (T1 << 62), TNN1 = T1 >> 2;
        const uint64_t TP0 = T0 << 1, TP1 = (T1 << 1) | (T0 >> 63);
        const uint64_t PH0 = ~T0 & TN0 & ~TNN0, PH1 = ~T1 & TN1 & ~TNN1;
        const uint64_t PS0 = T0 & ~TN0 & ~TP0, PS1 = T1 & ~TN1 & ~TP1;
        if (!(popts & 1u) && (PH0 | PH1) != 0ull) {
            const bool ph0 = act0 && ((PH0 >> ln) & 1ull) != 0ull;
            const bool ph1 = act1 && ((PH1 >> ln) & 1ull) != 0ull;
            const bool ps0 = act0 && ((PS0 >> ln) & 1ull) != 0ull;
            const bool ps1 = act1 && ((PS1 >> ln) & 1ull) != 0ull;
            if (__ballot(ph0 || ph1) != 0ull) {
                auto walk = [&](uint32_t slot, uint32_t mine, uint32_t dnew) {
                    const uint32_t other = si[slot + 1];
                    const uint64_t a = (uint64_t)mine + dnew, b = (uint64_t)other + dnew;
                    const uint64_t lim = n - (a > b ? a : b);
                    uint32_t ca = 0, cb = 0;
                    const uint64_t k = kp.packed ? walk_lcp_packed(kp.packed, kp.b, n, a, b, WALK_CAP, ca, cb)
                                                 : walk_lcp(text, n, a, b, WALK_CAP);
                    if (k == WALK_CAP && k < lim) {
                        sg[slot] = 0xffffffffu; sg[slot + 1] = 0xffffffffu;
                        return;
                    }
                    const bool mine_first = k == lim ? a > b : (kp.packed ? ca < cb : text[a + k] < text[b + k]);
                    si[slot] = mine_first ? mine : other;
                    si[slot + 1] = mine_first ? other : mine;
                    sg[slot] = 0u;
                    sg[slot + 1] = dnew + (uint32_t)k;
#ifdef SUFR_HIP_PROBES
                    if (popts & 4u) {
                        atomicAdd(&g_walk_stats[0], 1ull); atomicAdd(&g_walk_stats[1], (unsigned long long)k);
                        atomicMax(&g_walk_stats[2], (unsigned long long)k);
                    }
#endif
                };
                if (ph0) walk((uint32_t)ln, i0, dd0 + advance(k0));
                if (ph1) walk((uint32_t)(64 + ln), i1, dd1 + advance(k1));
                if (ph0 || ps0) {
                    const uint32_t v = sg[ln];
                    if (v == 0xffffffffu) extra0 = WALK_CAP;
                    else { i0 = si[ln]; if (ps0) lcp0 = v; act0 = false; gid0 = 0x10000u | (uint32_t)ln; lt0 = false; }
                }
                if (ph1 || ps1) {
                    const uint32_t v = sg[64 + ln];
                    if (v == 0xffffffffu) extra1 = WALK_CAP;
                    else { i1 = si[64 + ln]; if (ps1) lcp1 = v; act1 = false; gid1 = 0x10000u | (uint32_t)(64 + ln); lt1 = false; }
                }
            }
        }
        SUFR_STAMP(ph__, 2)
        const bool walk_next = ktype == 1 && round >= 1 && !(popts & 2u) && __ballot(extra0 | extra1) == 0ull;
        if (walk_next) {
            auto wkey = [&](uint32_t mine, uint32_t ref, uint32_t d) -> uint64_t {
                const uint64_t a = (uint64_t)mine + d, r2 = (uint64_t)ref + d;
                const uint64_t lim = n - (a > r2 ? a : r2);
                uint32_t ca = 0, cb = 0;
                const uint64_t L = kp.packed ? walk_lcp_packed(kp.packed, kp.b, n, a, r2, WALK_CAP, ca, cb)
                                             : walk_lcp(text, n, a, r2, WALK_CAP);
                if (L == WALK_CAP && L < lim) return walk_key(true, false, 0);
                const bool below = L == lim ? a > r2 : (kp.packed ? ca < cb : text[a + L] < text[r2 + L]);
                return walk_key(false, below, L);
            };
            if (act0) {
                dd0 += advance(k0);
                const uint32_t ref = si[gid0];
                k0 = gid0 == (uint32_t)ln ? walk_key(true, false, 0) : wkey(i0, ref, dd0);
            }
            if (act1) {
                dd1 += advance(k1);
                const uint32_t ref = si[gid1];
                k1 = gid1 == (uint32_t)(64 + ln) ? walk_key(true, false, 0) : wkey(i1, ref, dd1);
            }
            ktype = 2;
        } else {
            if (act0) { dd0 += advance(k0) + extra0; extra0 = 0; }
            if (act1) { dd1 += advance(k1) + extra1; extra1 = 0; }
            if (kp.packed) {
                PackedPair f0 = {0ull, 0ull}, f1 = {0ull, 0ull};
                if (act0) f0 = packed_fetch16(kp.packed, kp.b, (uint64_t)i0 + dd0 - 1u);
                if (act1) f1 = packed_fetch16(kp.packed, kp.b, (uint64_t)i1 + dd1 - 1u);
                if (act0) k0 = make_run_key_packed(n, R, kp.b, (uint64_t)i0 + dd0, kp.packed, f0);
                if (act1) k1 = make_run_key_packed(n, R, kp.b, (uint64_t)i1 + dd1, kp.packed, f1);
            } else {
                if (act0) k0 = make_run_key(text, n, R, s_lut, kp.b, (uint64_t)i0 + dd0, 1u, nullptr);
                if (act1) k1 = make_run_key(text, n, R, s_lut, kp.b, (uint64_t)i1 + dd1, 1u, nullptr);
            }
            ktype = 1;
        }
        SUFR_STAMP(ph__, 3)
    }
    SUFR_STAMP(ph__, 0)
    if (TIES_OUT) {
        const uint64_t M0 = __ballot(act0), M1 = __ballot(act1);
        const uint64_t Hd0 = __ballot(act0 && !lt0), Hd1 = __ballot(act1 && !lt1);
        if (ln == 0) {
            wmask[(size_t)wave * 4 + 0] = M0; wmask[(size_t)wave * 4 + 1] = M1;
            wmask[(size_t)wave * 4 + 2] = Hd0; wmask[(size_t)wave * 4 + 3] = Hd1;
            const uint32_t nwin = (m + 127u) / 128u;
            wcnt[wave] = (uint32_t)(__popcll(M0) + __popcll(M1));
            wcnt[(size_t)nwin + wave] = (uint32_t)(__popcll(Hd0) + __popcll(Hd1));
        }
        if (act0) idx_writeback[j0] = i0;
        if (act1) idx_writeback[j1] = i1;
    }
    if (small0) {
        const bool tied = TIES_OUT && act0;
        uint32_t o = DEEP ? opos[j0] : j0;
        if (!tied) SA[o] = i0;
        if (!tied || !lt0) {
            if (!first0) LCP[o] = lcp0;
            else if (!DEEP) LCP[o] = 0;
        }
    }
    if (small1) {
        const bool tied = TIES_OUT && act1;
        uint32_t o = DEEP ? opos[j1] : j1;
        if (!tied) SA[o] = i1;
        if ((!tied || !lt1) && !first1) LCP[o] = lcp1;
    }
    SUFR_STAMP(ph__, 4)
    if (DEEP && !TIES_OUT) { SUFR_STAMP_FLUSH(2, 8) }
}

static constexpr uint32_t PLAN_CH = 2048, PLAN_W = 48, PLAN_L = 24;

__global__ void __launch_bounds__(256)
k_plan_windows(const uint64_t* __restrict__ keys, const uint32_t* __restrict__ segs, const uint32_t* __restrict__ opos,
               const uint32_t* __restrict__ segdepth, uint32_t m, int sorted_bits, int bits,
               uint32_t* __restrict__ LCP, uint2* __restrict__ wslots, uint32_t* __restrict__ lslots,
               uint32_t* __restrict__ wcnt, uint32_t* __restrict__ lcnt, uint32_t nchunk)
{
    const uint32_t chunk = (blockIdx.x * 256 + threadIdx.x) >> 6;
    if (chunk >= nchunk) return;
    const uint32_t ln = lane_id();
    const uint64_t c0 = (uint64_t)chunk * PLAN_CH;
    const bool whole = sorted_bits == 0;
    const int shift = whole ? 0 : 64 - sorted_bits;
    uint64_t hv = 0;
    uint64_t lastk = 0; uint32_t lasts = 0;
    if (c0 > 0) { lastk = keys[c0 - 1]; lasts = segs[c0 - 1]; }
#pragma unroll 2
    for (uint32_t it = 0; it < 34u; it++) {
        const uint64_t j = c0 + 64ull * it + ln;
        const bool valid = j < m;
// ... 41 lines not shown
            }
            nl++;
            pos = next_head(lim + 1u, 32);
        }
    }
    if (ln == 0) { wcnt[chunk] = nw < PLAN_W ? nw : PLAN_W; lcnt[chunk] = nl < PLAN_L ? nl : PLAN_L; }
}

__global__ void __launch_bounds__(256)
k_plan_compact(const uint2* __restrict__ wslots, const uint32_t* __restrict__ lslots, const uint32_t* __restrict__ wcnt,
               const uint32_t* __restrict__ lcnt, const uint32_t* __restrict__ woff, const uint32_t* __restrict__ loff,
               uint32_t nchunk, uint32_t* __restrict__ win_start, uint32_t* __restrict__ win_count,
               uint32_t* __restrict__ heads)
{
    const uint32_t t = blockIdx.x * 256 + threadIdx.x;
    const uint32_t chunk = t / (PLAN_W + PLAN_L), slot = t % (PLAN_W + PLAN_L);
    if (chunk >= nchunk) return;
    if (slot < PLAN_W) {
        if (slot < wcnt[chunk]) {
            const uint2 w = wslots[(size_t)chunk * PLAN_W + slot];
            win_start[woff[chunk] + slot] = w.x; win_count[woff[chunk] + slot] = w.y;
        }
    } else if (slot - PLAN_W < lcnt[chunk])
        heads[loff[chunk] + slot - PLAN_W] = lslots[(size_t)chunk * PLAN_L + slot - PLAN_W];
}

template <bool DENSE>
__global__ void __launch_bounds__(256)
k_build_ties(const unsigned long long* __restrict__ wmask, const uint32_t* __restrict__ rec_off,
             const uint32_t* __restrict__ run_off, const uint32_t* __restrict__ idxs, uint32_t m,
             uint32_t depth0, uint32_t* __restrict__ idx_new, uint32_t* __restrict__ seg_new,
             uint32_t* __restrict__ opos_new, uint32_t* __restrict__ newdepth, uint8_t* __restrict__ newperiod)
{
    const uint32_t w = DENSE ? (blockIdx.x * 256 + threadIdx.x) >> 6 : blockIdx.x * 256 + threadIdx.x;
    const uint64_t base64 = (uint64_t)w * 128;
    if (base64 >= m) return;
    const uint32_t base = (uint32_t)base64;
    const ulonglong2 mm = *reinterpret_cast<const ulonglong2*>(wmask + (size_t)w * 4);
    if ((mm.x | mm.y) == 0ull) return;
    const ulonglong2 hh = *reinterpret_cast<const ulonglong2*>(wmask + (size_t)w * 4 + 2);
    const uint32_t t0 = rec_off[w];
    const uint32_t s0 = run_off[w] - 1u;
    if (DENSE) {
        const uint64_t M0 = mm.x, M1 = mm.y, H0 = hh.x, H1 = hh.y;
        const uint32_t ln = lane_id();
        const uint64_t lt = (1ull << ln) - 1ull, le = lt | (1ull << ln);
        if ((M0 >> ln) & 1ull) {
            const uint32_t t = t0 + (uint32_t)__popcll(M0 & lt);
            const uint32_t g = s0 + (uint32_t)__popcll(H0 & le);
            idx_new[t] = idxs[base + ln];
            seg_new[t] = g;
            opos_new[t] = base + ln;
            if ((H0 >> ln) & 1ull) { newdepth[g] = depth0; newperiod[g] = 1; }
        }
        if ((M1 >> ln) & 1ull) {
            const uint32_t t = t0 + (uint32_t)(__popcll(M0) + __popcll(M1 & lt));
            const uint32_t g = s0 + (uint32_t)(__popcll(H0) + __popcll(H1 & le));
            idx_new[t] = idxs[base + 64u + ln];
            seg_new[t] = g;
            opos_new[t] = base + 64u + ln;
            if ((H1 >> ln) & 1ull) { newdepth[g] = depth0; newperiod[g] = 1; }
        }
    } else {
        const uint64_t M[2] = {mm.x, mm.y}, H[2] = {hh.x, hh.y};
        uint32_t t = t0, sgm = s0;
        for (int half = 0; half < 2; half++) {
            uint64_t left = M[half];
            while (left) {
                const int bit = __builtin_ctzll(left);
                left &= left - 1;
                const uint32_t slot = (uint32_t)(half * 64 + bit);
                if ((H[half] >> bit) & 1ull) {
                    sgm++;
                    newdepth[sgm] = depth0;
                    newperiod[sgm] = 1;
                }
                idx_new[t] = idxs[base + slot];
                seg_new[t] = sgm;
                opos_new[t] = base + slot;
                t++;
            }
        }
    }
}

__global__ void __launch_bounds__(256)
k_compact_large(const uint32_t* __restrict__ wl_flag, const uint32_t* __restrict__ wl_off,
                const uint32_t* __restrict__ wl_head, uint32_t nwin, uint32_t* __restrict__ heads)
{
    uint32_t w = blockIdx.x * 256 + threadIdx.x;
    if (w < nwin && wl_flag[w]) heads[wl_off[w]] = wl_head[w];
}

__global__ void __launch_bounds__(256)
k_gather_keys(const uint8_t* __restrict__ text, uint64_t n, RunTable R,
              const uint16_t* __restrict__ glut, const uint32_t* __restrict__ idx,
              const uint32_t* __restrict__ seg, const uint32_t* __restrict__ segdepth,
              const uint8_t* __restrict__ segperiod, uint32_t m, KeyParams kp, uint64_t* __restrict__ keys,
              uint32_t* __restrict__ max_token_bits)
{
    __shared__ uint16_t s_lut[256];
    for (int i = threadIdx.x; i < 256; i += 256) s_lut[i] = glut[i];
    __syncthreads();
    uint32_t e = blockIdx.x * 256 + threadIdx.x;
    uint32_t tb = 0;
    if (e < m) {
        const uint64_t k =
            make_run_key(text, n, R, s_lut, kp.b, (uint64_t)idx[e] + segdepth[seg[e]], segperiod[seg[e]], kp.packed);
        keys[e] = k;
        tb = (uint32_t)decode_run_token(k).tokbits;
    }
    if (max_token_bits) {
#pragma unroll
        for (int o = 32; o > 0; o >>= 1) tb = max(tb, (uint32_t)__shfl_down(tb, o, WAVE));
        if (lane_id() == 0 && tb > 34u) atomicMax(max_token_bits, tb);
    }
}

__global__ void __launch_bounds__(256)
k_gather_keys_listed(const uint8_t* __restrict__ text, uint64_t n, RunTable R, const uint16_t* __restrict__ glut,
                     const uint32_t* __restrict__ idx, const uint32_t* __restrict__ list, const uint32_t* __restrict__ start,
                     const uint32_t* __restrict__ size, const uint32_t* __restrict__ segdepth,
                     const uint8_t* __restrict__ segperiod, KeyParams kp, uint64_t* __restrict__ keys)
{
    __shared__ uint16_t s_lut[256];
    for (int i = threadIdx.x; i < 256; i += 256) s_lut[i] = glut[i];
    __syncthreads();
    const uint32_t g = list[blockIdx.x];
    const uint32_t t0 = start[g], t1 = t0 + size[g];
    const uint32_t d = segdepth[g], pi = segperiod[g];
    for (uint32_t t = t0 + blockIdx.y * 256u + threadIdx.x; t < t1; t += 256u * gridDim.y)
        keys[t] = make_run_key(text, n, R, s_lut, kp.b, (uint64_t)idx[t] + d, pi, kp.packed);
}

template <bool DEEP>
__global__ void __launch_bounds__(256)
k_group_extent(const uint64_t* __restrict__ keys, const uint32_t* __restrict__ segs,
               const uint32_t* __restrict__ segdepth, uint32_t m, int sorted_bits, KeyParams kp,
               const uint32_t* __restrict__ heads, const uint32_t* __restrict__ idxs,
               const uint8_t* __restrict__ text, uint32_t L, uint32_t* __restrict__ sizes,
               uint32_t* __restrict__ newdepth, uint8_t* __restrict__ newperiod, uint32_t* __restrict__ maxsize,
               uint32_t* __restrict__ periodic_list = nullptr)
{
    uint32_t k = blockIdx.x * 256 + threadIdx.x;
    if (k >= L) return;
    const bool whole = sorted_bits == 0;
    const int group_shift = whole ? 0 : 64 - sorted_bits;
    uint32_t h = heads[k];
    uint64_t hk = keys[h];
    uint64_t top = whole ? 0ull : (hk >> group_shift);
    uint32_t sg = DEEP ? segs[h] : 0u;
    uint32_t lo = h + 1, hi = m;
    while (lo < hi) {
        uint32_t mid = lo + (hi - lo) / 2;
        bool in_group = (!DEEP || segs[mid] == sg) && (whole || (keys[mid] >> group_shift) == top);
        if (in_group) lo = mid + 1; else hi = mid;
    }
    uint32_t sz = lo - h;
    sizes[k] = sz;
    const uint32_t nd = DEEP ? segdepth[sg] + run_key_advance(hk, sorted_bits, kp.b)
                             : (uint32_t)(sorted_bits / kp.b);
    newdepth[k] = nd;
    uint32_t pi = 1;
    if (nd >= 12 && kp.detect_period) {
        const uint8_t* e = text + (uint64_t)idxs[h] + nd;
        const uint32_t win = nd < 16 ? nd : 16;
// ... 648 lines not shown
```

sufr_amd/csrc/sufr_launch.inc:

```

#include <math.h>
#include <stdio.h>
#include <stdlib.h>
#include <string.h>

#include <chrono>
#include <functional>
#include <memory>
#include <string>
#include <thread>
#include <vector>

#include "../../include/sufr_hip.h"

namespace sufr {

#define HIP_TRY(call)                                                                        \
    do {                                                                                     \
        hipError_t e__ = (call);                                                             \
        if (e__ != hipSuccess) {                                                             \
            set_error(std::string(#call) + ": " + hipGetErrorString(e__));                   \
            return SUFR_HIP_E_HIP;                                                           \
        }                                                                                    \
    } while (0)

static constexpr uint64_t SUFR_MAX_TEXT_LEN = 0xFFFFFFFFull - (1ull << 24);

struct DevBuf {
    void* p = nullptr;
    size_t cap = 0;
};

struct LevelArrays {
    DevBuf keyA, keyB, idxA, idxB, segA, segB, opos;
};

class Pipeline;
struct ExcShard { int sharded; uint32_t raw_lo, raw_hi; int D; int allow_amb; uint32_t cap; };
int exc_reinsert(Pipeline& pl, uint8_t* d_text, uint64_t n, const uint32_t* bsa, const uint32_t* blcp, uint32_t s,
                 const uint32_t* d_exc, uint32_t E, uint32_t* out_sa, uint32_t* out_lcp, uint64_t out_cap, uint64_t* affected_out,
                 const ExcShard& shard, uint64_t* s_out);
static constexpr uint32_t EXC_MAX_LIST = 1u << 20;

class Pipeline {
public:
    int device = 0;
    hipStream_t stream = nullptr;
    bool own_stream = false;
    std::string err;
    uint64_t resident_text_len = 0;
    uint32_t stitch_weight = 0;
    uint64_t stitch_cap = 0;
    DevBuf stitchoffs;
    StitchOrder stitch_order() const { StitchOrder so; so.offs = stitch_weight ? (const uint32_t*)stitchoffs.p : nullptr; so.weight = stitch_weight; so.cap = stitch_cap; return so; }
    bool debug = false;

    DevBuf text, bytehist, lut, table, bintot, binbase, scalars;
    DevBuf keyA, keyB, idxA, idxB;
    DevBuf recA, recB;
    DevBuf rankbuf, dposbuf, deferbuf, unresbuf, posbitsbuf, dblf[7], dblg[6];
    DevBuf headsA, headsB, sizes, starts, partials;
    DevBuf tilefirst, runends, tileany, nexttile, nextblk, depthA, depthB, period, remapbuf, flagsbuf, packedbuf, wmaskbuf, wcntbuf, recoff, runoff, wlflag, wlhead, wloff, candbuf, keepbuf, plancnt, fixbuf;
    DevBuf rg_misc, rg_blk, rg_blkoff, rg_rs, rg_rl, rg_E, rg_L, rg_V, rg_tab[2], rg_off[2], rg_long[2], rg_tmax[2], rg_hist, rg_depth;
    DevBuf cumbuf, dmapbuf, identbuf[16], grouptab, gcur, leafcnt, leafoff, leafbase, leafcur, bigflag, bigoff;
    DevBuf rawtab, presbuf, rawtot, valsbuf, startbuf;
    DevBuf exc_pos, exc_byte, exc_sorted, exc_sa, exc_lcp, exc_bits, exc_blk, exc_off, exc_list, exc_list2, exc_pmin, exc_roff;
    std::unique_ptr<Pipeline> helper;
    bool overlap_chains = true;
    static constexpr uint64_t OVERLAP_MIN_DEFAULT = (uint64_t)1 << 22;
    uint64_t opt_overlap_min = 0;
    uint32_t last_overlapped = 0;
    uint64_t dbl_entries = 0;
    uint64_t last_doublings = 0;
    std::function<int()> before_doubling;
    uint32_t exc_pending = 0;
    bool mql_fast_ok = true;
    bool exc_disable = false;
    static constexpr uint64_t EXC_MAX_AFFECTED_DEFAULT = (uint64_t)1 << 22;
    uint64_t opt_exc_max_affected = 0;
    uint64_t exc_max_affected() const { return opt_exc_max_affected ? opt_exc_max_affected : EXC_MAX_AFFECTED_DEFAULT; }
    uint32_t last_exc_retry = 0;
    uint64_t last_exc_taken = 0;
    DevBuf exc_all_sa, exc_all_lcp;
    bool no_exceptions = false;
    std::vector<uint32_t> rawtot_host, valshost;
    uint16_t h_lut[256];
    uint32_t h_seg0[2];
    DevBuf segst[2], segsz[2], tunits, upre, tdesc, wunits, wpre, wdesc, wslow;
    std::vector<uint8_t> dmaphost, identhost[16];
    std::vector<uint16_t> remaphost;
    std::vector<uint32_t> cumhost;
    int segcur = 0;
    uint32_t text_wgs = 2048, pairs_wgs = 1024;
    uint32_t num_cus = 0;
    bool part_r3 = false;
    bool no_dna_table = false;
    bool detect_period = true;
    uint32_t msd_groups = 8;
    int deep_digit_bits = 10;
    uint32_t dbl_min_share = 1;
    int mask_digit_bits = 10;
    bool mask_lcp_from_keys = true;
    bool group_sort = true;
    static constexpr uint32_t GS_CAP = 4096;
    uint32_t gs_giant = 1u << 14;
    uint32_t gs_giant_knob = 0;
    DevBuf gs_leafbase, gs_pst, gs_psz, gs_wcnt, gs_wpre, gs_wdesc, gs_flag, gs_off, gs_big, gs_lg, gs_lsz, gs_loff;
    bool run_groups = true;
    bool key_carry = true;
    int p2min_knob = 0;
    int key_chars_knob = 0;
    static bool packed_ok_for_knob(int b) { return b >= 2 && b <= 4; }
    uint32_t finish_opts = 0;
    LevelArrays lv[2];
    RunTable rtab{nullptr, nullptr, nullptr, nullptr, 0};
    DevBuf sa32, lcp32;
    DevBuf optA, optB, optC, optD, optE;
    DevBuf wideoffs;
    uint64_t opt_max_query_len = 0;
    uint64_t opt_wide_retry = 0;
    uint32_t wide_shard_index = 0, wide_num_shards = 1;
    uint64_t wide_text_len = 0;
    uint64_t wide_orphans = 0;
    std::vector<uint32_t> opt_mask_offsets;
    hipEvent_t ev[16];
    bool have_events = false;

    static constexpr int LEAF_E = 8;
    int leaf_nt = 512;
    uint32_t LEAF_CAP = 4096;
    uint32_t LEAF_BIG = 4096;
    bool leaf_dna3 = false;
    uint32_t leaf_bmax = 256;
    int leaf_t1 = 12;
    int ms_e = 8;
    static constexpr int ms_nt = 512;

    void set_error(const std::string& s) { err = s; }

    static constexpr size_t PIN_CAP = (size_t)512 << 10;
    uint8_t* pin = nullptr;
    size_t pin_used = 0;
    struct PinItem { void* dst; size_t off, bytes; };
    std::vector<PinItem> pin_items;
    hipError_t d2h_at(void* dst, const void* src, size_t bytes)
    {
        if (!pin || pin_used + bytes > PIN_CAP) { copies_queued = true; return hipMemcpyAsync(dst, src, bytes, hipMemcpyDeviceToHost, stream); }
        const hipError_t e = hipMemcpyAsync(pin + pin_used, src, bytes, hipMemcpyDeviceToHost, stream);
        if (e == hipSuccess) { pin_items.push_back({dst, pin_used, bytes}); pin_used += (bytes + 63) & ~(size_t)63; copies_queued = true; }
        return e;
    }
    static constexpr size_t PUB_CAP = 8192;
    uint8_t* pub = nullptr;
// ... 86 lines not shown
        return e;
    }

    int init(int dev)
    {
        device = dev;
        int cnt = 0;
        if (hipGetDeviceCount(&cnt) != hipSuccess || cnt <= 0) {
            set_error("no HIP device available (libsufr_hip has no CPU fallback)");
            return SUFR_HIP_E_NO_DEVICE;
        }
        if (dev < 0 || dev >= cnt) { set_error("device id out of range"); return SUFR_HIP_E_INVALID; }
        HIP_TRY(hipSetDevice(dev));
        {
            int cus = 0;
            if (hipDeviceGetAttribute(&cus, hipDeviceAttributeMultiprocessorCount, dev) == hipSuccess && cus > 0) num_cus = (uint32_t)cus;
        }
        HIP_TRY(hipStreamCreateWithFlags(&stream, hipStreamNonBlocking));
        own_stream = true;
        for (auto& e : ev) HIP_TRY(hipEventCreate(&e));
        have_events = true;
        if (hipHostMalloc((void**)&pin, PIN_CAP, hipHostMallocDefault) != hipSuccess) { pin = nullptr; (void)hipGetLastError(); }
        if (hipHostMalloc((void**)&pub, PUB_CAP + 64, hipHostMallocMapped) != hipSuccess ||
            hipHostGetDevicePointer((void**)&pub_dev, pub, 0) != hipSuccess) {
            if (pub) (void)hipHostFree(pub);
            pub = nullptr; pub_dev = nullptr; (void)hipGetLastError();
        } else {
            memset(pub, 0, PUB_CAP + 64);
        }
        read_env();
        return 0;
    }

    void read_env()
    {
        const char* d = getenv("SUFR_HIP_DEBUG");
        debug = d && d[0] && d[0] != '0';
#ifdef SUFR_HIP_PROBES
        pub_drop = getenv("SUFR_PROBE_PUBLISH_DROP") && atoi(getenv("SUFR_PROBE_PUBLISH_DROP"));
        if (const char* e = getenv("SUFR_PROBE_TEXT_WGS")) if (atoi(e) > 0) text_wgs = (uint32_t)atoi(e);
        if (const char* e = getenv("SUFR_PROBE_PAIRS_WGS")) if (atoi(e) > 0) pairs_wgs = (uint32_t)atoi(e);
        if (const char* e = getenv("SUFR_PROBE_GROUPS")) if (atoi(e) > 0 && atoi(e) <= 64) msd_groups = (uint32_t)atoi(e);
        part_r3 = getenv("SUFR_PROBE_PART_R3") && atoi(getenv("SUFR_PROBE_PART_R3"));
        if (const char* e = getenv("SUFR_PROBE_DEEP_BITS")) { int v = atoi(e); if (v >= 4 && v <= 12) deep_digit_bits = v; }
        no_dna_table = getenv("SUFR_PROBE_NO_DNA_TABLE") && atoi(getenv("SUFR_PROBE_NO_DNA_TABLE"));
        no_exceptions = getenv("SUFR_PROBE_NO_EXCEPTIONS") && atoi(getenv("SUFR_PROBE_NO_EXCEPTIONS"));
        mql_fast_ok = !(getenv("SUFR_PROBE_NO_MQL_FAST") && atoi(getenv("SUFR_PROBE_NO_MQL_FAST")));
        overlap_chains = !(getenv("SUFR_PROBE_NO_OVERLAP") && atoi(getenv("SUFR_PROBE_NO_OVERLAP")));
        detect_period = !getenv("SUFR_PROBE_NO_PERIOD");
        if (const char* e = getenv("SUFR_PROBE_LEAF_NT")) if (atoi(e) == 512 || atoi(e) == 1024) leaf_nt = atoi(e);
        LEAF_CAP = (uint32_t)(leaf_nt * LEAF_E); LEAF_BIG = 4096;
        leaf_t1 = 12;
        if (const char* e = getenv("SUFR_PROBE_LEAF_BIG")) if (atoi(e) >= 64) LEAF_BIG = (uint32_t)atoi(e);
        if (LEAF_BIG > LEAF_CAP) LEAF_BIG = LEAF_CAP;
        if (const char* e = getenv("SUFR_PROBE_FINISH_OPTS")) finish_opts = (uint32_t)atoi(e) << 29;
        if (const char* e = getenv("SUFR_PROBE_DBL_SHARE")) dbl_min_share = (uint32_t)atoi(e);
        if (const char* e = getenv("SUFR_PROBE_P2MIN")) p2min_knob = atoi(e);
        key_carry = !getenv("SUFR_PROBE_NO_KEY_CARRY");
        run_groups = !getenv("SUFR_PROBE_NO_RUN_GROUPS");
        mask_lcp_from_keys = !getenv("SUFR_PROBE_MASK_LCP_TEXT");
        if (const char* e = getenv("SUFR_PROBE_MASK_DIGIT_BITS")) { int v = atoi(e); if (v >= 4 && v <= 12) mask_digit_bits = v; }
        if (const char* e = getenv("SUFR_PROBE_GROUP_SORT")) group_sort = atoi(e) != 0;
        if (const char* e = getenv("SUFR_PROBE_GIANT")) if (atoi(e) >= (int)GS_CAP) gs_giant_knob = (uint32_t)atoi(e);
        if (const char* e = getenv("SUFR_PROBE_KEY_CHARS")) key_chars_knob = atoi(e);
        if (const char* e = getenv("SUFR_PROBE_BMAX")) if (atoi(e) >= 1) leaf_bmax = (uint32_t)atoi(e);
        if (const char* e = getenv("SUFR_PROBE_LEAF_ABL")) leaf_bmax |= (uint32_t)atoi(e) << 24;
        if (const char* e = getenv("SUFR_PROBE_MS_E")) if (atoi(e) == 4 || atoi(e) == 6 || atoi(e) == 8) ms_e = atoi(e);
        if (const char* e = getenv("SUFR_PROBE_T1")) if (atoi(e) >= 11 && atoi(e) <= 13) leaf_t1 = atoi(e);
        if (leaf_nt == 512 && leaf_t1 == 13) leaf_t1 = 12;
        if (leaf_nt == 1024 && leaf_t1 == 11) leaf_t1 = 12;
#endif
        if (text_wgs > 16384u) text_wgs = 16384u;
        if (pairs_wgs > 16384u) pairs_wgs = 16384u;
    }

    void release(DevBuf& b) { if (b.p) (void)hipFree(b.p); b.p = nullptr; b.cap = 0; }

    void destroy()
    {
        if (helper) { helper->destroy(); helper.reset(); }
        (void)hipSetDevice(device);
        DevBuf* all[] = {&text, &bytehist, &lut, &table, &bintot, &binbase, &scalars, &keyA, &keyB, &idxA,
                         &idxB, &recA, &recB, &headsA, &headsB, &sizes, &starts, &partials, &sa32, &lcp32,
                         &tilefirst, &runends, &tileany, &nexttile, &nextblk, &depthA, &depthB, &period, &remapbuf, &flagsbuf, &packedbuf, &wmaskbuf, &wcntbuf, &recoff, &runoff, &wlflag, &wlhead, &wloff, &candbuf, &keepbuf, &plancnt, &fixbuf,
                         &rg_misc, &rg_blk, &rg_blkoff, &rg_rs, &rg_rl, &rg_E, &rg_L, &rg_V, &rg_tab[0], &rg_tab[1], &rg_off[0], &rg_off[1], &rg_long[0], &rg_long[1], &rg_tmax[0], &rg_tmax[1], &rg_hist, &rg_depth,
                         &exc_pos, &exc_byte, &exc_sorted, &exc_sa, &exc_lcp, &exc_bits, &exc_blk, &exc_off, &exc_list, &exc_list2, &exc_pmin, &exc_roff, &exc_all_sa, &exc_all_lcp,
                         &cumbuf, &dmapbuf, &rawtab, &presbuf, &rawtot, &valsbuf, &startbuf, &grouptab, &gcur, &leafcnt, &leafoff, &leafbase, &leafcur, &bigflag, &bigoff,
                         &segst[0], &segst[1], &segsz[0], &segsz[1], &tunits, &upre, &tdesc, &wunits, &wpre, &wdesc, &wslow,
                         &optA, &optB, &optC, &optD, &optE, &stitchoffs, &wideoffs,
                         &gs_leafbase, &gs_pst, &gs_psz, &gs_wcnt, &gs_wpre, &gs_wdesc, &gs_flag, &gs_off, &gs_big, &gs_lg, &gs_lsz, &gs_loff};
        for (auto& b : identbuf) release(b);
        for (auto& b : dblf) release(b);
        for (auto& b : dblg) release(b);
        release(rankbuf); release(dposbuf); release(deferbuf); release(unresbuf); release(posbitsbuf);
        for (auto* b : all) release(*b);
        for (auto& l : lv) { release(l.keyA); release(l.keyB); release(l.idxA); release(l.idxB);
                             release(l.segA); release(l.segB); release(l.opos); }
        if (have_events) for (auto& e : ev) (void)hipEventDestroy(e);
        if (pin) { (void)hipHostFree(pin); pin = nullptr; }
        if (pub) { (void)hipHostFree(pub); pub = nullptr; pub_dev = nullptr; }
        if (own_stream && stream) (void)hipStreamDestroy(stream);
    }

    void release_build_arrays(bool also_text)
    {
        if (helper) helper->release_build_arrays(false);
        (void)hipSetDevice(device);
        if (also_text) { release(text); resident_text_len = 0; }
        DevBuf* big[] = {&recA, &recB, &keyA, &keyB, &idxA, &idxB, &packedbuf, &runends, &startbuf, &wmaskbuf, &wcntbuf, &fixbuf, &exc_sa, &exc_lcp, &exc_bits, &exc_all_sa, &exc_all_lcp,
                         &headsA, &headsB, &rankbuf, &dposbuf, &deferbuf, &unresbuf, &posbitsbuf, &depthA, &depthB, &period,
                         &recoff, &runoff, &candbuf, &keepbuf, &optA, &optB, &optC, &optD, &optE};
        for (auto* b : big) if (b->cap >= ((size_t)16 << 20)) release(*b);
        for (auto& b : dblf) release(b);
        for (auto& b : dblg) release(b);
        for (auto& l : lv) { release(l.keyA); release(l.keyB); release(l.idxA); release(l.idxB);
                             release(l.segA); release(l.segB); release(l.opos); }
    }

    int ensure_keep(DevBuf& b, size_t bytes)
    {
        if (b.cap >= bytes || !b.p) return ensure(b, bytes);
        DevBuf nb;
        int rc = ensure(nb, bytes + bytes / 2);
        if (rc) return rc;
        if (hipMemcpyAsync(nb.p, b.p, b.cap, hipMemcpyDeviceToDevice, stream) != hipSuccess || sync_reads() != hipSuccess) {
            (void)hipFree(nb.p);
            set_error("growing a buffer failed");
            return SUFR_HIP_E_HIP;
        }
        (void)hipFree(b.p);
        b = nb;
        return 0;
    }
    int ensure(DevBuf& b, size_t bytes)
    {
        if (bytes < 256) bytes = 256;
        if (b.cap >= bytes) return 0;
        if (b.p) { (void)hipFree(b.p); b.p = nullptr; b.cap = 0; }
        size_t want = bytes + bytes / 16;
        hipError_t e = hipMalloc(&b.p, want);
        if (e != hipSuccess) {
            b.p = nullptr;
            (void)hipGetLastError();
            set_error("hipMalloc(" + std::to_string(want) + " bytes): " + hipGetErrorString(e));
            return SUFR_HIP_E_NOMEM;
        }
        b.cap = want;
        return 0;
    }
    enum { SC_TOTAL = 0, SC_LARGE = 1, SC_MAXSIZE = 2, SC_SCANTOTAL = 3, SC_BAD = 4, SC_MAXTOK = 5, SC_WTOTAL = 6,
           SC_UTOTAL = 7, SC_NBIG = 8, SC_MBIG = 9, SC_MAXBIG = 10, SC_NFIX = 11, SC_TMP0 = 13, SC_TMP1 = 14, SC_GSBIG = 15, SC_GSLARGE = 16 , SC_N = 24 };
    unsigned long long* sc(int i) { return reinterpret_cast<unsigned long long*>(scalars.p) + i; }

    static int ceil_log2_u64(uint64_t v) { int b = 0; while ((1ull << b) < v && b < 63) b++; return b; }

    int radix_pass_pairs(const uint64_t* in_key, const uint32_t* in_idx, const uint32_t* in_seg, uint32_t m,
                         uint32_t nbins, uint32_t raw_bins, const uint16_t* remap, int shift, bool from_seg,
                         uint64_t* out_key, uint32_t* out_idx, uint32_t* out_seg)
    {
        const uint32_t tiles = (m + TILE - 1) / TILE;
        uint32_t nwg = tiles < pairs_wgs ? tiles : pairs_wgs;
        if (nwg < 1) nwg = 1;
        uint32_t tiles_per = (tiles + nwg - 1) / nwg;
        tiles_per = (tiles_per + 1u) & ~1u;
        uint32_t chunk = tiles_per * TILE;
        nwg = (m + chunk - 1) / chunk;
        const int nbits = ceil_log2_u64(nbins) < 1 ? 1 : ceil_log2_u64(nbins);
        int rc;
        if ((rc = ensure(table, (size_t)nwg * nbins * 4))) return rc;
        if ((rc = ensure(bintot, (size_t)nbins * 4))) return rc;
        if ((rc = ensure(binbase, (size_t)nbins * 4))) return rc;
        const size_t rm_bytes = remap ? (size_t)((raw_bins + 7u) & ~7u) * 2 : 0;
        hipLaunchKernelGGL(k_hist_pairs, dim3(nwg), dim3(THREADS), (size_t)nbins * 4 + rm_bytes, stream, in_key,
                           from_seg ? in_seg : (const uint32_t*)nullptr, m, nbins, raw_bins, remap, shift, chunk,
                           (uint32_t*)table.p);
        hipLaunchKernelGGL(k_scan_table_cols, dim3((nbins + 255) / 256), dim3(256), 0, stream,
                           (uint32_t*)table.p, nwg, nbins, (uint32_t*)bintot.p);
        hipLaunchKernelGGL(k_scan_bins, dim3(1), dim3(256), 0, stream, (const uint32_t*)bintot.p, nbins,
                           (uint32_t*)binbase.p, (unsigned long long*)nullptr);
        const bool has_seg = in_seg != nullptr;
        const size_t nba = (nbins + 3u) & ~3u;
#define SUFR_LAUNCH_PAIRS_NB(SEG, NT_, E_, NB_)                                                                 \
        {                                                                                                      \
            size_t stage = (size_t)(NT_ * E_) * (SEG ? 16 : 12);                                              \
            size_t wc = ((size_t)(NT_ / 64) * nbins * 2 + 15) & ~(size_t)15;                                  \
            size_t lds = nba * 12 + 128 + rm_bytes + (stage > wc ? stage : wc);                               \
            HIP_TRY(hipFuncSetAttribute((const void*)k_scatter_pairs<SEG, NT_, E_, NB_>,                      \
                                        hipFuncAttributeMaxDynamicSharedMemorySize, (int)lds));               \
            hipLaunchKernelGGL((k_scatter_pairs<SEG, NT_, E_, NB_>), dim3(nwg), dim3(NT_), lds, stream, in_key, \
                               in_idx, in_seg, m, nbins, nbits, raw_bins, remap, shift, from_seg ? 1 : 0,     \
                               chunk, (const uint32_t*)table.p, (const uint32_t*)binbase.p, out_key, out_idx, \
                               out_seg);                                                                      \
        }
#define SUFR_LAUNCH_PAIRS(SEG, NT_, E_)                                                   \
// ... 1079 lines not shown
                           (const uint32_t*)segst[segcur].p, (const uint32_t*)segsz[segcur].p, nseg,
                           (const uint32_t*)leafbase.p, NB, (uint32_t)LEAF_CAP, (uint32_t)LEAF_BIG, (uint32_t*)wunits.p,
                           (const uint32_t*)nullptr, (uint4*)nullptr, (uint32_t*)bigflag.p);
        if ((rc = scan_u32((const uint32_t*)wunits.p, nseg, (uint32_t*)wpre.p, sc(SC_WTOTAL)))) return rc;
        hipLaunchKernelGGL(k_pack_windows<true>, dim3((nseg + 3) / 4), dim3(256), 0, stream,
                           (const uint32_t*)segst[segcur].p, (const uint32_t*)segsz[segcur].p, nseg,
                           (const uint32_t*)leafbase.p, NB, (uint32_t)LEAF_CAP, (uint32_t)LEAF_BIG, (uint32_t*)nullptr,
                           (const uint32_t*)wpre.p, (uint4*)wdesc.p, (uint32_t*)nullptr);
        if ((rc = scan_u32((const uint32_t*)bigflag.p, (uint32_t)cells, (uint32_t*)bigoff.p, sc(SC_NBIG)))) return rc;
        const uint64_t bigcap = m / (LEAF_BIG + 1) + 1;
        if ((rc = ensure(segst[segcur ^ 1], bigcap * 4))) return rc;
        if ((rc = ensure(segsz[segcur ^ 1], bigcap * 4))) return rc;
        hipLaunchKernelGGL(k_compact_big, dim3((uint32_t)((cells + 255) / 256)), dim3(256), 0, stream,
                           (const uint32_t*)bigflag.p, (const uint32_t*)bigoff.p, (const uint32_t*)leafbase.p,
                           (const uint32_t*)segst[segcur].p, (const uint32_t*)segsz[segcur].p, nseg, NB,
                           (uint32_t*)segst[segcur ^ 1].p, (uint32_t*)segsz[segcur ^ 1].p, sc(SC_MBIG));
        unsigned long long two[3] = {0, 0, 0};
        {
            const uint32_t gmax = leaf_nt == 1024 ? 1024u : 2048u;
            const uint32_t grid = wub < gmax ? wub : gmax;
            const size_t lds = (size_t)LEAF_CAP * 12 + (size_t)LEAF_KEY_PAD * 8 + msd_map_bytes_host(dm.rows) +
                               (leaf_dna3 ? (size_t)DNA3_HALF_ENTRIES * 2 : (size_t)LEAF_CS_MAX * 8) +
                               128 + ((size_t)1 << leaf_t1) * 4;
#define SUFR_LEAF(NT_, T1_, D3_)                                                                                         \
            {                                                                                                            \
                HIP_TRY(hipFuncSetAttribute((const void*)k_leaf_sort<NT_, LEAF_E, T1_, D3_>,                            \
                                            hipFuncAttributeMaxDynamicSharedMemorySize, (int)lds));                     \
                hipLaunchKernelGGL((k_leaf_sort<NT_, LEAF_E, T1_, D3_>), dim3(grid), dim3(NT_), lds, stream, rsrc,      \
                                   rdst, (const uint4*)wdesc.p, (const unsigned long long*)sc(SC_WTOTAL),              \
                                   (uint32_t*)wslow.p, hibit, dm, cc, fo, leaf_bmax);                                   \
            }
#define SUFR_LEAF_D(NT_, T1_) { if (leaf_dna3) SUFR_LEAF(NT_, T1_, true) else SUFR_LEAF(NT_, T1_, false) }
            if (leaf_nt == 1024) { if (leaf_t1 == 13) SUFR_LEAF_D(1024, 13) else SUFR_LEAF_D(1024, 12) }
            else { if (leaf_t1 == 11) SUFR_LEAF_D(512, 11) else SUFR_LEAF_D(512, 12) }
#undef SUFR_LEAF_D
#undef SUFR_LEAF
            const size_t lds2 = (size_t)LEAF_CAP * 12 + msd_map_bytes_host(dm.rows) + 128 + 256 * 4 +
                                (size_t)(leaf_nt / 64) * 256 * 2;
#define SUFR_LEAF_LSD(NT_)                                                                                               \
            {                                                                                                            \
                HIP_TRY(hipFuncSetAttribute((const void*)k_leaf_sort_lsd<NT_, LEAF_E>,                                  \
                                            hipFuncAttributeMaxDynamicSharedMemorySize, (int)lds2));                    \
                hipLaunchKernelGGL((k_leaf_sort_lsd<NT_, LEAF_E>), dim3(grid), dim3(NT_), lds2, stream, rsrc, rdst,     \
                                   (const uint4*)wdesc.p, (const unsigned long long*)sc(SC_WTOTAL),                    \
                                   (const uint32_t*)wslow.p, hibit, cc.lastbit, dm, fo);                               \
            }
            if (leaf_nt == 1024) SUFR_LEAF_LSD(1024) else SUFR_LEAF_LSD(512)
#undef SUFR_LEAF_LSD
            hipLaunchKernelGGL(k_advance_fix, dim3(1), dim3(64), 0, stream, (uint32_t*)sc(SC_NFIX),
                               (const unsigned long long*)sc(SC_WTOTAL), 0u);
        }
        HIP_TRY(hipGetLastError());
        HIP_TRY(read_at_sync(two, sc(SC_NBIG), 24));
        HIP_TRY(sync_reads());
        nbig = (uint32_t)two[0];
        mbig = two[1];
        maxbig = two[2];
        return 0;
    }

    int plan_tiles(uint32_t nseg, uint64_t m, uint32_t G, uint32_t unit, uint32_t& SG, uint32_t& tub)
    {
        int rc;
        SG = (nseg + G - 1) / G;
        const uint32_t slots = G * SG;
        tub = (uint32_t)(m / unit + nseg);
        if ((rc = ensure(tunits, (size_t)slots * 4))) return rc;
        if ((rc = ensure(upre, (size_t)slots * 4))) return rc;
        if ((rc = ensure(tdesc, (size_t)tub * 16))) return rc;
        hipLaunchKernelGGL(k_seg_units, dim3((slots + 255) / 256), dim3(256), 0, stream, (const uint32_t*)segsz[segcur].p,
                           nseg, G, SG, unit, (uint32_t*)tunits.p);
        if ((rc = scan_u32((const uint32_t*)tunits.p, slots, (uint32_t*)upre.p, sc(SC_UTOTAL)))) return rc;
        hipLaunchKernelGGL(k_msd_tiles, dim3((tub + 255) / 256), dim3(256), 0, stream, (const uint32_t*)segst[segcur].p,
                           (const uint32_t*)segsz[segcur].p, G, SG, unit, (const uint32_t*)upre.p,
                           (const unsigned long long*)sc(SC_UTOTAL), (uint4*)tdesc.p);
        HIP_TRY(hipGetLastError());
        return 0;
    }

    int sort_device_u32(const void* d_in, uint64_t n, uint32_t flags, uint32_t shard_index,
                        uint32_t num_shards, uint32_t* d_sa, uint32_t* d_lcp, uint64_t cap,
                        uint64_t* num_suffixes_out, sufr_hip_stats* st_out)
    {
        last_overlapped = 0; last_doublings = 0; dbl_entries = 0;
        if (helper) helper->dbl_entries = 0;
        if (!exc_disable) { last_exc_retry = 0; last_exc_taken = 0; }
        const int rc = sort_build(d_in, n, flags, shard_index, num_shards, d_sa, d_lcp, cap, num_suffixes_out, st_out);
        before_doubling = nullptr;
        last_doublings = dbl_entries + (helper ? helper->dbl_entries : 0);
        if (exc_pending) {
            const uint32_t E = exc_pending;
            exc_pending = 0;
            hipLaunchKernelGGL(k_exc_restore, dim3((E + 255) / 256), dim3(256), 0, stream, (uint8_t*)text.p,
                               (const uint32_t*)exc_pos.p, (const uint8_t*)exc_byte.p, E);
            if ((hipGetLastError() != hipSuccess || hipStreamSynchronize(stream) != hipSuccess) && !rc) {
                set_error("putting the listed bytes back into the text failed");
                return SUFR_HIP_E_HIP;
            }
        }
        return rc;
    }

    struct Build {
        const void* d_in_caller = nullptr;
        uint64_t n = 0, cap = 0;
        uint32_t flags = 0, shard_index = 0, num_shards = 1;
        bool is_dna = false, allow_amb = false, raw = false, softmask = false, masked = false;
        uint32_t* caller_sa = nullptr; uint32_t* caller_lcp = nullptr;
        uint64_t* num_suffixes_out = nullptr;
        sufr_hip_stats* st_out = nullptr;
        sufr_hip_stats st;
        uint8_t* d_text = nullptr;
        const void* d_in = nullptr;
        uint32_t ngrid = 0, G1 = 0;
        uint64_t nwg_t = 0, tchunk = 0;
        bool small_tiles = false;
        bool dna_table = false;
        uint32_t nexc = 0;
        unsigned long long hist[256];
        std::vector<uint64_t> pwords;
        std::vector<uint32_t> pflags;
        KeyParams kp;
        uint64_t eligible_total = 0;
        bool packed_path = false, mql_fast = false;
        int mql_charbits = 0, mbits = 0;
        DigitMap dm;
        std::vector<uint32_t> present_vals;
        uint32_t NB = 0;
        const uint16_t* d_remap = nullptr;
        CharModel cc;
        uint32_t raw_lo = 0, raw_hi = 0, bin_lo = 0, bin_hi = 0;
        uint64_t s = 0;
        uint32_t m0 = 0;
        uint32_t* d_sa = nullptr; uint32_t* d_lcp = nullptr;
        Rec* xr[2] = {nullptr, nullptr};
        uint32_t nwin = 0, wcnt_stride = 0, fixcap = 0;
        FinishOut fo;
        uint32_t mql_count = 0;
    };
    struct LeftOver { uint32_t groups = 0; uint64_t records = 0; uint32_t depth = 0; uint64_t maxbig = 0; };
    struct LeftChain { std::thread th; int rc = 0; sufr_hip_stats st = {}; ~LeftChain() { if (th.joinable()) th.join(); } };

    int done(Build& B) { if (B.st_out) *B.st_out = B.st; return 0; }
    int check_capacity(uint64_t s, uint64_t cap, const uint32_t* d_sa, const uint32_t* d_lcp)
    {
        if (s > cap || !d_sa || !d_lcp) {
            set_error("output capacity " + std::to_string(cap) + " < num_suffixes " + std::to_string(s));
            return SUFR_HIP_E_CAPACITY;
        }
        return 0;
    }

    int sort_build(const void* d_in, uint64_t n, uint32_t flags, uint32_t shard_index,
                   uint32_t num_shards, uint32_t* d_sa, uint32_t* d_lcp, uint64_t cap,
                   uint64_t* num_suffixes_out, sufr_hip_stats* st_out)
    {
        Build B;
        LeftChain chain;
        int rc;
        if ((rc = check_call(B, d_in, n, flags, shard_index, num_shards, d_sa, d_lcp, cap, num_suffixes_out, st_out))) return rc;
        if (n == 0) return done(B);
        if ((rc = open_text(B))) return rc;
        if ((rc = plan_text_chunks(B))) return rc;
        if ((rc = text_stage(B))) return rc;
        if ((rc = code_table(B))) return rc;
        if (B.eligible_total == 0) return done(B);
        if (B.masked) {
// ... 647 lines not shown
                if (lds > PART_LDS_MAX) { set_error("first-level digit map too large for the partition kernel"); return SUFR_HIP_E_UNSUPPORTED; } \
                HIP_TRY(hipFuncSetAttribute((const void*)k_msd_part_text<BB, NT_, RN_, SH>,                             \
                                            hipFuncAttributeMaxDynamicSharedMemorySize, (int)lds));                     \
                if (BB == 3 && mql_fast) {                                                                               \
                    HIP_TRY(hipFuncSetAttribute((const void*)k_msd_part_text<3, NT_, RN_, SH, true>,                     \
                                                hipFuncAttributeMaxDynamicSharedMemorySize, (int)lds));                 \
                    hipLaunchKernelGGL((k_msd_part_text<3, NT_, RN_, SH, true>), dim3((uint32_t)nwg_t), dim3(NT_), lds, stream, \
                                       n, kp, dm, tchunk, raw_lo, raw_hi, G1, (uint32_t*)gcur.p, xr[0],                 \
                                       (const uint64_t*)startbuf.p, (uint32_t)(~0ull << (64 - kp.K * kp.b)),            \
                                       (uint32_t)(kp.K * kp.b - 32));                                                   \
                } else                                                                                                   \
                hipLaunchKernelGGL((k_msd_part_text<BB, NT_, RN_, SH>), dim3((uint32_t)nwg_t), dim3(NT_), lds, stream,  \
                                   n, kp, dm, tchunk, raw_lo, raw_hi, G1, (uint32_t*)gcur.p, xr[0],                     \
                                   (const uint64_t*)startbuf.p, (uint32_t)(~0ull << (64 - kp.K * kp.b)), 0u);           \
            }
#define SUFR_PART_TEXT(BB, NT_, SH)                                                                                      \
            {                                                                                                            \
                if (BB == 3 && NT_ == 1024 && PartGeom<3, 1024, 2>::lds_bytes(dm.raw_mask + 1u, NB) > PART_LDS_MAX) {    \
                    half_tiles = true;                                                                                   \
                    SUFR_PART_TEXT_G(3, 1024, 1, SH)                                                                     \
                } else SUFR_PART_TEXT_G(BB, NT_, 2, SH)                                                                  \
            }
#ifdef SUFR_HIP_PROBES
#define SUFR_PART_TEXT_R3(BB, NT_, SH)                                                                                   \
            {                                                                                                            \
                using Geom = PartGeomR3<BB, NT_, 2>;                                                                     \
                const size_t lds = Geom::lds_bytes((uint32_t)msd_map_bytes_host(dm.rows), NB);                          \
                HIP_TRY(hipFuncSetAttribute((const void*)k_msd_part_text_r3<BB, NT_, 2, SH>,                            \
                                            hipFuncAttributeMaxDynamicSharedMemorySize, (int)lds));                     \
                hipLaunchKernelGGL((k_msd_part_text_r3<BB, NT_, 2, SH>), dim3((uint32_t)nwg_t), dim3(NT_), lds, stream, \
                                   n, kp, dm, tchunk, raw_lo, raw_hi, G1, (uint32_t*)gcur.p, xr[0],                     \
                                   (const uint64_t*)startbuf.p, (uint32_t)(~0ull << (64 - kp.K * kp.b)));               \
            }
#define SUFR_PART_TEXT_V(BB, NT_, SH) { if (part_r3) SUFR_PART_TEXT_R3(BB, NT_, SH) else SUFR_PART_TEXT(BB, NT_, SH) }
#else
#define SUFR_PART_TEXT_V(BB, NT_, SH) SUFR_PART_TEXT(BB, NT_, SH)
#endif
#define SUFR_PART_TEXT_B(BB)                                                                                             \
            {                                                                                                            \
                if (small_tiles) { if (sh) SUFR_PART_TEXT_V(BB, 256, true) else SUFR_PART_TEXT_V(BB, 256, false) }       \
                else { if (sh) SUFR_PART_TEXT_V(BB, 1024, true) else SUFR_PART_TEXT_V(BB, 1024, false) }                 \
            }
            const bool sh = num_shards > 1;
            bool half_tiles = false;
            if (!B.dna_table) {
                const uint32_t nw64 = (uint32_t)((n + 63) / 64);
#define SUFR_STARTBITS(BB) hipLaunchKernelGGL(k_startbits_packed<BB>, dim3((nw64 + 255) / 256), dim3(256), 0, stream, \
                                              kp.packed, n, kp.elig_codes, (uint64_t*)startbuf.p)
                if (kp.b == 2) SUFR_STARTBITS(2); else if (kp.b == 3) SUFR_STARTBITS(3); else SUFR_STARTBITS(4);
#undef SUFR_STARTBITS
            }
            if (kp.b == 2) SUFR_PART_TEXT_B(2) else if (kp.b == 3) SUFR_PART_TEXT_B(3) else SUFR_PART_TEXT_B(4)
#undef SUFR_PART_TEXT_B
#undef SUFR_PART_TEXT_V
#undef SUFR_PART_TEXT
#undef SUFR_PART_TEXT_G
            B.st.partition_variant = half_tiles ? 4u : 3u;
        } else {
            if ((rc = launch_scatter_text((uint32_t)nwg_t, B.d_text, n, kp, B.d_remap, kp.top_shift, tchunk, raw_lo, raw_hi,
                                          num_shards > 1, xr[0]))) return rc;
            B.st.partition_variant = 0u;
        }
        HIP_TRY(hipEventRecord(ev[5], stream));
        HIP_TRY(hipGetLastError());
        return 0;
    }

    int msd_levels(Build& B, LeftOver& left)
    {
        const uint64_t n = B.n, s = B.s;
        const uint32_t m0 = B.m0, NB = B.NB;
        const int mbits = B.mbits;
        const bool mql_fast = B.mql_fast;
        const KeyParams& kp = B.kp; const DigitMap& dm = B.dm; Rec* const* const xr = B.xr; FinishOut& fo = B.fo;
        int rc;
        const uint32_t nwin = B.nwin = (m0 + 127) / 128;
        const uint32_t fixcap = B.fixcap = (uint32_t)(s / 32 + 65536);
        if ((rc = ensure(wmaskbuf, (size_t)nwin * 32))) return rc;
        B.wcnt_stride = (nwin + 3u) & ~3u;
        if ((rc = ensure(wcntbuf, (size_t)B.wcnt_stride * 8))) return rc;
        if ((rc = ensure(fixbuf, (size_t)fixcap * 4))) return rc;
        HIP_TRY(zero_later(wmaskbuf.p, (size_t)nwin * 32));
        HIP_TRY(zero_later(sc(SC_NFIX), 8));
        HIP_TRY(zero_flush());
        fo.SA = B.d_sa; fo.LCP = B.d_lcp; fo.wmask = (unsigned long long*)wmaskbuf.p; fo.fixlist = (uint32_t*)fixbuf.p;
        fo.nfix = (uint32_t*)sc(SC_NFIX); fo.fixcap = fixcap; fo.b = kp.b; fo.K = kp.K;
        rg_active.clear(); rg_run_off = 0;
        if ((rc = ensure(segst[0], 256))) return rc;
        if ((rc = ensure(segsz[0], 256))) return rc;
        segcur = 0;
        h_seg0[0] = 0u; h_seg0[1] = m0;
        HIP_TRY(hipMemcpyAsync(segst[0].p, &h_seg0[0], 4, hipMemcpyHostToDevice, stream));
        HIP_TRY(hipMemcpyAsync(segsz[0].p, &h_seg0[1], 4, hipMemcpyHostToDevice, stream));
        uint32_t nseg = 1;
        uint64_t m = s;
        int src = 0;
        int bits_done = mbits;
        DigitMap dl = dm;
        const int maxbits = mql_fast ? 64 : kp.K * kp.b;
        const int charbits = mql_fast ? B.mql_charbits : maxbits;
        uint32_t levels = 1;
        for (;;) {
            uint32_t nbig = 0; uint64_t mbig = 0, maxbig = 0;
            if ((rc = leaf_stage(xr[src], xr[1], nseg, m, dl, B.cc, fo, 64 - bits_done, nbig, mbig, maxbig)))
                return rc;
            if (debug) fprintf(stderr, "[sufr_hip debug] msd level %u: segments=%u records=%llu bits=%d -> big leaves=%u records=%llu\n",
                               levels, nseg, (unsigned long long)m, bits_done, nbig, (unsigned long long)mbig);
            if (!nbig) break;
            segcur ^= 1; nseg = nbig; m = mbig;
            if (levels == 1 && B.packed_path && !mql_fast) {
                if ((rc = run_groups_extract(B.d_text, n, kp, xr[src], xr[1], (uint32_t)(mbits / kp.b), s, fo, nseg, m, maxbig))) return rc;
                if (!nseg) break;
            }
            int w = 0;
            const bool in_chars = bits_done < charbits;
            const int digit_end = in_chars ? charbits : maxbits;
            bool char_digit = false;
            if (bits_done < digit_end) {
                w = mbits;
                if (bits_done + w > digit_end) w = digit_end - bits_done;
                uint64_t budget = (1ull << 26) / nseg;
                int wb = 0; while (wb < 12 && (2ull << wb) <= budget) wb++;
                char_digit = in_chars && bits_done % mbits == 0 && w == mbits && (uint64_t)NB <= budget;
                if (!char_digit) { if (w > wb) w = wb; if (w < 1) w = 1; }
            }
            const uint32_t G = (nseg >= 64 && maxbig * msd_groups <= m + m / 2) ? msd_groups : 1u;
            uint32_t SG = 0, tub = 0;
            if ((rc = plan_tiles(nseg, m, G, (uint32_t)(ms_nt * ms_e), SG, tub))) return rc;
            if (w == 0) {
                if (src != 1)
                    hipLaunchKernelGGL(k_copy_tiles, dim3(1024), dim3(256), 0, stream, (const Rec*)xr[src],
                                       (const uint4*)tdesc.p, (const unsigned long long*)sc(SC_UTOTAL), xr[1]);
                hipLaunchKernelGGL(k_append_starts, dim3((nseg + 255) / 256), dim3(256), 0, stream,
                                   (const uint32_t*)segst[segcur].p, nseg, fo.fixlist, fo.nfix, fo.fixcap);
                hipLaunchKernelGGL(k_advance_fix, dim3(1), dim3(64), 0, stream, (uint32_t*)sc(SC_NFIX),
                                   (const unsigned long long*)nullptr, nseg);
                HIP_TRY(hipGetLastError());
                left.groups = nseg; left.records = m; left.depth = (uint32_t)(bits_done / kp.b); left.maxbig = maxbig;
                break;
            }
            DigitMap dn = dm;
            if (!char_digit) { if ((rc = identity_digit_map(w, dn))) return rc; }
            bits_done += w;
            const int shift = 64 - bits_done;
            const uint32_t NBn = dn.nbins;
            const uint64_t cells = (uint64_t)nseg * NBn;
            if ((rc = ensure(leafcnt, cells * 4))) return rc;
            if ((rc = ensure(leafoff, cells * 4))) return rc;
            if ((rc = ensure(leafbase, cells * 4))) return rc;
            if ((rc = ensure(leafcur, cells * 4))) return rc;
            HIP_TRY(hipMemsetAsync(leafcnt.p, 0, cells * 4, stream));
            {
                const size_t lds = msd_map_bytes_host(dn.rows) + (size_t)NBn * 4;
                hipLaunchKernelGGL(k_msd_hist, dim3(2048), dim3(THREADS), lds, stream, (const Rec*)xr[src],
                                   (const uint4*)tdesc.p, (const unsigned long long*)sc(SC_UTOTAL), shift, dn,
                                   (uint32_t*)leafcnt.p);
            }
            if ((rc = scan_u32((const uint32_t*)leafcnt.p, (uint32_t)cells, (uint32_t*)leafoff.p))) return rc;
            hipLaunchKernelGGL(k_msd_leafbase, dim3((uint32_t)((cells + 255) / 256)), dim3(256), 0, stream,
                               (const uint32_t*)leafoff.p, (const uint32_t*)segst[segcur].p, nseg, NBn,
                               (uint32_t*)leafbase.p, (uint32_t*)leafcur.p);
            {
#define SUFR_MSD_SCATTER(NT_, E_)                                                                                        \
                {                                                                                                    \
                    const size_t lds = (size_t)(NT_ * E_) * 14 + msd_map_bytes_host(dn.rows) +                      \
                                       (size_t)((NBn + 3u) & ~3u) * 4 + 128;                                        \
                    HIP_TRY(hipFuncSetAttribute((const void*)k_msd_scatter<NT_, E_>,                                \
                                                hipFuncAttributeMaxDynamicSharedMemorySize, (int)lds));             \
                    hipLaunchKernelGGL((k_msd_scatter<NT_, E_>), dim3(ms_e == 8 ? 1024 : 2048), dim3(NT_), lds, stream, \
                                       (const Rec*)xr[src], (const uint4*)tdesc.p, (const uint32_t*)upre.p, G, SG,  \
                                       (const unsigned long long*)sc(SC_UTOTAL), shift, dn, (uint32_t*)leafcur.p,   \
                                       xr[src ^ 1]);                                                                \
                }
                if (ms_e == 4) SUFR_MSD_SCATTER(512, 4) else if (ms_e == 6) SUFR_MSD_SCATTER(512, 6) else SUFR_MSD_SCATTER(512, 8)
#undef SUFR_MSD_SCATTER
            }
            HIP_TRY(hipGetLastError());
            src ^= 1;
            dl = dn;
            levels++;
        }
        B.st.num_passes = levels;
        HIP_TRY(hipEventRecord(ev[6], stream));
        hipLaunchKernelGGL(k_fix_window_lcp, dim3(1024), dim3(256), 0, stream, (const uint32_t*)fixbuf.p,
                           (const uint32_t*)sc(SC_NFIX), fixcap, (const Rec*)xr[1], B.d_lcp, kp.b, kp.K);
        hipLaunchKernelGGL(k_tie_counts, dim3((nwin + 255) / 256), dim3(256), 0, stream,
                           (const unsigned long long*)wmaskbuf.p, nwin, (uint32_t*)wcntbuf.p, B.wcnt_stride);
        HIP_TRY(hipGetLastError());
        HIP_TRY(hipEventRecord(ev[7], stream));
        B.st.num_levels = 1;
        return 0;
    }

    int join_left_chain(Build& B, LeftChain& chain)
    {
        if (!chain.th.joinable()) return 0;
        chain.th.join();
        if (chain.rc) { err = helper->err; return chain.rc; }
        B.st.num_levels += chain.st.num_levels;
        B.st.num_large_groups += chain.st.num_large_groups;
        B.st.deep_records += chain.st.deep_records;
        return run_groups_expand(B.d_text, B.n, B.kp, B.d_sa, B.d_lcp);
    }

    int start_left_chain(Build& B, const LeftOver& left, LeftChain& chain)
    {
        const uint64_t n = B.n;
        const bool mql_fast = B.mql_fast;
        const KeyParams kp = B.kp;
        uint8_t* const d_text = B.d_text; uint32_t* const d_sa = B.d_sa; uint32_t* const d_lcp = B.d_lcp; Rec* const* const xr = B.xr;
        uint32_t left_groups = left.groups;
        int rc;
        if (left_groups && left.maxbig >= RG_MIN_SIZE && !mql_fast && (rc = run_groups_find(d_text, n, kp, xr[1], xr[1], (const uint32_t*)segst[segcur].p, (uint32_t*)segsz[segcur].p,
                                                 left_groups, (uint32_t)kp.K, RG_MIN_SIZE, false))) return rc;
        uint32_t early = 0;
        for (const RunGroupState& S : rg_active) if (S.K != (uint32_t)kp.K) early++;
        const uint32_t* depth_of = nullptr;
        if (early) {
            const uint32_t Lall = left_groups + early;
            std::vector<uint32_t> hs(early), hz(early), hd(Lall, left.depth);
            uint32_t e = 0;
            for (const RunGroupState& S : rg_active)
                if (S.K != (uint32_t)kp.K) { hs[e] = S.g.start; hz[e] = S.M; hd[left_groups + e] = S.K; e++; }
            if ((rc = ensure_keep(segst[segcur], (size_t)Lall * 4)) || (rc = ensure_keep(segsz[segcur], (size_t)Lall * 4))) return rc;
            if ((rc = ensure(rg_depth, (size_t)Lall * 4))) return rc;
            HIP_TRY(hipMemcpyAsync((uint32_t*)segst[segcur].p + left_groups, hs.data(), (size_t)early * 4, hipMemcpyHostToDevice, stream));
            HIP_TRY(hipMemcpyAsync((uint32_t*)segsz[segcur].p + left_groups, hz.data(), (size_t)early * 4, hipMemcpyHostToDevice, stream));
            HIP_TRY(hipMemcpyAsync(rg_depth.p, hd.data(), (size_t)Lall * 4, hipMemcpyHostToDevice, stream));
            HIP_TRY(sync_reads());
            depth_of = (const uint32_t*)rg_depth.p;
            left_groups = Lall;
        }
        if (!left_groups) return 0;
        LevelState lg;
        lg.k = nullptr; lg.i = (const uint32_t*)xr[1] + 2; lg.istride = 3; lg.s = nullptr; lg.o = nullptr; lg.m = B.m0; lg.deep = false; lg.sbits = 0;
        lg.L = left_groups; lg.heads_cur = &headsA; lg.heads_nxt = &headsB; lg.depth_cur = &depthA;
        lg.depth_nxt = &depthB; lg.which = 0;
        lg.seg_start = (const uint32_t*)segst[segcur].p; lg.seg_size = (const uint32_t*)segsz[segcur].p;
        lg.seg_depth = left.depth; lg.seg_depth_of = depth_of;
        lg.pos_keys = mql_fast;
        if (mql_fast) lg.seg_depth = (uint32_t)kp.K;
        const bool side_by_side = overlap_chains && left.records >= (opt_overlap_min ? opt_overlap_min : OVERLAP_MIN_DEFAULT);
        if (debug) fprintf(stderr, "[sufr_hip debug] left-over buckets: groups=%u records=%llu%s\n", left_groups,
                           (unsigned long long)left.records, side_by_side ? " (on the helper pipeline)" : "");
        if (side_by_side) {
            if (!helper) {
                helper.reset(new Pipeline);
                if ((rc = helper->init(device))) { err = helper->err; helper->destroy(); helper.reset(); return rc; }
            }
            Pipeline& H = *helper;
            H.read_env();
            H.debug = debug;
            H.rtab = rtab;
            if ((rc = H.ensure(H.lut, 512)) || (rc = H.ensure(H.scalars, SC_N * 8))) { err = H.err; return rc; }
            HIP_TRY(hipMemcpyAsync(H.lut.p, lut.p, sizeof h_lut, hipMemcpyDeviceToDevice, stream));
            HIP_TRY(hipEventRecord(ev[11], stream));
            HIP_TRY(hipStreamWaitEvent(H.stream, ev[11], 0));
            lg.heads_cur = &H.headsA; lg.heads_nxt = &H.headsB; lg.depth_cur = &H.depthA; lg.depth_nxt = &H.depthB;
            H.reset_reads();
            chain.st = sufr_hip_stats(); chain.rc = 0;
            H.dbl_entries = 0;
            last_overlapped = 1;
            chain.th = std::thread([&H, &chain, lg, d_text, n, kp, d_sa, d_lcp, this]() {
                (void)hipSetDevice(device);
                chain.rc = H.run_levels(lg, d_text, n, kp, d_sa, d_lcp, chain.st);
                if (hipStreamSynchronize(H.stream) != hipSuccess && !chain.rc) { H.set_error("the helper stream failed"); chain.rc = SUFR_HIP_E_HIP; }
            });
        } else {
            if ((rc = run_levels(lg, d_text, n, kp, d_sa, d_lcp, B.st))) return rc;
            if ((rc = run_groups_expand(d_text, n, kp, d_sa, d_lcp))) return rc;
        }
        return 0;
    }

    template <bool WAVE>
    void launch_build_ties(uint32_t nwin, const uint32_t* icur, uint32_t m0, uint32_t K, LevelArrays& A)
    {
        hipLaunchKernelGGL(k_build_ties<WAVE>, dim3(WAVE ? (nwin + 3) / 4 : (nwin + 255) / 256), dim3(256), 0, stream,
                           (const unsigned long long*)wmaskbuf.p, (const uint32_t*)recoff.p, (const uint32_t*)runoff.p, icur, m0, K,
                           (uint32_t*)A.idxA.p, (uint32_t*)A.segA.p, (uint32_t*)A.opos.p, (uint32_t*)depthA.p, (uint8_t*)period.p);
    }

    int tie_level(Build& B, LeftChain& chain)
    {
        const uint64_t n = B.n;
        const uint32_t m0 = B.m0, nwin = B.nwin, wcnt_stride = B.wcnt_stride, num_shards = B.num_shards;
        const bool mql_fast = B.mql_fast;
        const KeyParams& kp = B.kp; sufr_hip_stats& st = B.st;
        uint8_t* const d_text = B.d_text; uint32_t* const d_sa = B.d_sa; uint32_t* const d_lcp = B.d_lcp;
        int rc;
        uint32_t* cnt = (uint32_t*)wcntbuf.p;
        const uint32_t* icur = d_sa;
        if ((rc = ensure(recoff, (size_t)nwin * 4))) return rc;
        if ((rc = ensure(runoff, (size_t)nwin * 4))) return rc;
        if ((rc = scan_u32((const uint32_t*)cnt, nwin, (uint32_t*)recoff.p, sc(SC_TMP0)))) return rc;
        unsigned long long tot2[2] = {0, 0};
        if ((rc = scan_u32((const uint32_t*)(cnt + wcnt_stride), nwin, (uint32_t*)runoff.p, sc(SC_TMP1)))) return rc;
        unsigned long long nf = 0;
        HIP_TRY(read_at_sync(tot2, sc(SC_TMP0), 16));
        HIP_TRY(read_at_sync(&nf, sc(SC_NFIX), 8));
        HIP_TRY(sync_reads());
        if ((uint32_t)nf > B.fixcap) { set_error("internal error: window list overflow"); return SUFR_HIP_E_HIP; }
        const unsigned long long tot_rec = tot2[0], tot_run = tot2[1];
        const uint32_t m2 = (uint32_t)tot_rec, L2 = (uint32_t)tot_run;
        if (debug) fprintf(stderr, "[sufr_hip debug] tie level: runs=%u records=%u\n", L2, m2);
        if (m2 == 0) return 0;
        st.num_levels++;
        st.num_large_groups += L2;
        st.deep_records += m2;
        LevelArrays& A = lv[0];
        if ((rc = ensure(A.keyA, (size_t)m2 * 8))) return rc;
        if ((rc = ensure(A.idxA, (size_t)m2 * 4))) return rc;
        if ((rc = ensure(A.segA, (size_t)m2 * 4))) return rc;
        if ((rc = ensure(A.opos, (size_t)m2 * 4))) return rc;
        if ((rc = ensure(depthA, (size_t)L2 * 4))) return rc;
        if ((rc = ensure(period, (size_t)L2))) return rc;
        if ((rc = ensure(headsA, ((size_t)m2 / 64 + 2) * 4))) return rc;
        if ((uint64_t)m2 >= (uint64_t)nwin * 8) launch_build_ties<true>(nwin, icur, m0, (uint32_t)kp.K, A);
        else launch_build_ties<false>(nwin, icur, m0, (uint32_t)kp.K, A);
        if (mql_fast)
            hipLaunchKernelGGL(k_pos_keys, dim3((m2 + 255) / 256), dim3(256), 0, stream, (const uint32_t*)A.idxA.p, m2, (uint64_t*)A.keyA.p);
        else
        hipLaunchKernelGGL(k_gather_keys, dim3((m2 + 255) / 256), dim3(256), 0, stream,
                           (const uint8_t*)d_text, n, rtab, (const uint16_t*)lut.p,
                           (const uint32_t*)A.idxA.p, (const uint32_t*)A.segA.p, (const uint32_t*)depthA.p,
                           (const uint8_t*)period.p, m2, kp, (uint64_t*)A.keyA.p, (uint32_t*)nullptr);
        uint32_t Lt = 0;
        if ((rc = finish_level((const uint64_t*)A.keyA.p, (const uint32_t*)A.idxA.p, (const uint32_t*)A.segA.p,
                               (const uint32_t*)A.opos.p, (const uint32_t*)depthA.p, m2, 0, d_text, n, kp, d_sa, d_lcp,
                               &headsA, Lt))) return rc;
        LevelState lt;
        lt.k = (const uint64_t*)A.keyA.p; lt.i = (const uint32_t*)A.idxA.p; lt.s = (const uint32_t*)A.segA.p;
        lt.o = (const uint32_t*)A.opos.p; lt.m = m2; lt.deep = true; lt.sbits = 0; lt.L = Lt;
        lt.heads_cur = &headsA; lt.heads_nxt = &headsB; lt.depth_cur = &depthA; lt.depth_nxt = &depthB;
        lt.which = 1;
        dbl_shard = DblShard{kp.packed, kp.b, B.mbits, B.raw_lo, B.raw_hi, num_shards > 1 ? 1 : 0};
        lt.allow_doubling = !mql_fast && (num_shards <= 1 || (B.packed_path && kp.packed != nullptr)); lt.s_total = m0;
        lt.pos_keys = mql_fast;
        before_doubling = [this, &B, &chain]() { return join_left_chain(B, chain); };
        rc = run_levels(lt, d_text, n, kp, d_sa, d_lcp, st);
        before_doubling = nullptr;
        return rc;
    }

    int finish_stats(Build& B)
    {
        sufr_hip_stats& st = B.st;
#ifdef SUFR_HIP_PROBES
        if (debug) {
            unsigned long long ws[4] = {0, 0, 0, 0}, zero[4] = {0, 0, 0, 0};
            (void)hipMemcpyFromSymbol(ws, HIP_SYMBOL(g_walk_stats), sizeof ws);
            (void)hipMemcpyToSymbol(HIP_SYMBOL(g_walk_stats), zero, sizeof zero);
            fprintf(stderr, "[sufr_hip debug] pair walks: %llu, characters walked: %llu, longest: %llu\n", ws[0], ws[1], ws[2]);
            unsigned long long ph[3][16], phz[3][16];
            memset(phz, 0, sizeof phz);
            (void)hipMemcpyFromSymbol(ph, HIP_SYMBOL(g_phase), sizeof ph);
            (void)hipMemcpyToSymbol(HIP_SYMBOL(g_phase), phz, sizeof phz);
            static const char* names[3] = {"k_msd_part_text", "k_msd_scatter", "k_finish<DEEP> (0 load/flags, 1 ranking, 2 pair walks, 3 re-key, 4 writes, 5 rounds x 1000)"};
            for (int k = 0; k < 3; k++) {
                unsigned long long tot = 0;
                for (int i = 0; i < 16; i++) tot += ph[k][i];
                if (!tot) continue;
                fprintf(stderr, "[sufr_hip debug] %s phases (share of wave 0's cycles):", names[k]);
                for (int i = 0; i < 16; i++) if (ph[k][i]) fprintf(stderr, " %d:%.3f", i, (double)ph[k][i] / (double)tot);
                fprintf(stderr, "  (total %.3g cycles)\n", (double)tot);
            }
        }
#endif
        (void)hipEventElapsedTime(&st.ms_total, ev[0], ev[8]);
        (void)hipEventElapsedTime(&st.ms_normalize, ev[0], ev[1]);
        (void)hipEventElapsedTime(&st.ms_hist_text, ev[2], ev[3]);
        (void)hipEventElapsedTime(&st.ms_partition, ev[4], ev[5]);
        (void)hipEventElapsedTime(&st.ms_passes, ev[5], ev[6]);
        (void)hipEventElapsedTime(&st.ms_finish, ev[6], ev[7]);
        (void)hipEventElapsedTime(&st.ms_deep, ev[7], ev[8]);
        if (B.nexc) (void)hipEventElapsedTime(&st.ms_exceptions, ev[9], ev[10]);
        return done(B);
    }

    static void choose_shard(const std::vector<uint32_t>& tot, uint64_t total, uint32_t r, uint32_t R,
                             uint32_t& lo, uint32_t& hi, uint64_t& count)
    {
        auto boundary = [&](uint32_t k) -> uint32_t {
            if (k == 0) return 0;
            if (k >= R) return (uint32_t)tot.size();
            uint64_t target = (uint64_t)((__uint128_t)total * k / R);
            uint64_t cum = 0;
// ... 14 lines not shown
```

sufr_amd/csrc/sufr_wide.inc:

```

namespace sufr {

static constexpr int WIDE_MAX_WINDOWS = 32;
struct WideWindow { const uint32_t* sa; const uint32_t* lcp; uint64_t base, count; };
struct WideWindows { WideWindow w[WIDE_MAX_WINDOWS]; int num; };

__global__ void __launch_bounds__(256)
k_wide_normalize(const uint8_t* __restrict__ in, uint8_t* __restrict__ out, uint64_t n, int raw, int softmask)
{
    const uint64_t stride = (uint64_t)gridDim.x * 256 * 16;
    for (uint64_t at = ((uint64_t)blockIdx.x * 256 + threadIdx.x) * 16; at < n; at += stride) {
        const int m = n - at < 16 ? (int)(n - at) : 16;
        uint8_t v[16];
        if (m == 16) *reinterpret_cast<uint4*>(v) = *reinterpret_cast<const uint4*>(in + at);
        else for (int k = 0; k < m; k++) v[k] = in[at + k];
        if (raw)
            for (int k = 0; k < 16; k++) if (v[k] >= 97 && v[k] <= 122) v[k] = softmask ? (uint8_t)'N' : (uint8_t)(v[k] & 0x5F);
        if (m == 16) *reinterpret_cast<uint4*>(out + at) = *reinterpret_cast<const uint4*>(v);
        else for (int k = 0; k < m; k++) out[at + k] = v[k];
    }
}

static constexpr int WIDE_BLK = 4096;

// ... 432 lines not shown
        const uint64_t c = wide_rank(wo, text, n, a, y, a_lo + 1, a_hi, l);
        const uint64_t own = b.lcp[k];
        out_sa[k + c] = (OUT)y; out_lcp[k + c] = (OUT)(l > own ? l : own);
    }
}

struct WidePlan { uint64_t H; uint64_t margin; int num; };

inline WidePlan wide_plan(uint64_t n, uint64_t window, uint64_t margin)
{
    const uint64_t limit = SUFR_MAX_TEXT_LEN - 1;
    WidePlan p;
    p.margin = margin ? margin : ((uint64_t)1 << 26);
    if (window) { if (window > limit - 1) window = limit - 1; if (p.margin > limit - window) p.margin = limit - window; }
    else {
        if (p.margin > limit / 2) p.margin = limit / 2;
        window = limit - p.margin;
    }
    const uint64_t cnt = (n + window - 1) / window;
    p.H = (n + cnt - 1) / cnt;
    p.H = (p.H + 15) & ~(uint64_t)15;
    const uint64_t num = (n + p.H - 1) / p.H;
    p.num = num > (uint64_t)WIDE_MAX_WINDOWS ? -1 : (int)num;
    return p;
}

template <typename ORPH>
int repair_window(Pipeline& pl, const WideOrder& wo, const uint8_t* t, uint64_t n, uint64_t base, uint64_t len, uint32_t* out_sa,
                  uint32_t* out_lcp, uint64_t kept, DevBuf& wblk, ORPH& orphans, uint32_t** l_sa, uint32_t** l_lcp, uint64_t* nshort,
                  uint64_t* nrest)
{
    hipStream_t st = pl.stream;
    int rc;
    if ((rc = pl.ensure(pl.sa32, kept * 4 + 4)) || (rc = pl.ensure(pl.lcp32, kept * 4 + 4))) return rc;
    uint8_t* flags = nullptr;
    if (hipMalloc((void**)&flags, kept * 2 + 16) != hipSuccess) { pl.set_error("out of device memory (window repair)"); return SUFR_HIP_E_NOMEM; }
    orphans.bufs.push_back(flags);
    uint8_t *is_short = flags, *not_short = flags + kept;
    if (hipMemcpyAsync(pl.sa32.p, out_sa, kept * 4, hipMemcpyDeviceToDevice, st) != hipSuccess ||
        hipMemcpyAsync(pl.lcp32.p, out_lcp, kept * 4, hipMemcpyDeviceToDevice, st) != hipSuccess) { pl.set_error("window repair: copy failed"); return SUFR_HIP_E_HIP; }
    hipLaunchKernelGGL(k_wide_short_mark, dim3((uint32_t)((kept + 255) / 256)), dim3(256), 0, st, (const uint32_t*)pl.sa32.p,
                       (const uint32_t*)pl.lcp32.p, kept, len, is_short, not_short);
    const uint32_t nblk = (uint32_t)((kept + WIDE_BLK - 1) / WIDE_BLK);
    if ((rc = pl.ensure(wblk, (size_t)nblk * 4))) return rc;
    unsigned long long cnt = 0;
    hipLaunchKernelGGL(k_wide_count, dim3(nblk), dim3(256), 0, st, (const uint32_t*)pl.sa32.p, kept, 0u, (uint32_t*)wblk.p, (const uint8_t*)not_short);
    hipLaunchKernelGGL(k_wide_scan, dim3(1), dim3(1024), 0, st, (uint32_t*)wblk.p, nblk, pl.sc(Pipeline::SC_TOTAL));
    if (hipMemcpyAsync(&cnt, pl.sc(Pipeline::SC_TOTAL), 8, hipMemcpyDeviceToHost, st) != hipSuccess || hipStreamSynchronize(st) != hipSuccess) {
        pl.set_error("window repair: counting failed"); return SUFR_HIP_E_HIP;
    }
    *nshort = cnt; *nrest = kept - cnt;
    if (cnt > ((uint64_t)1 << 22)) return SUFR_HIP_E_UNSUPPORTED;
    uint32_t P = 1;
    while (P < cnt) P <<= 1;
    uint32_t* list = nullptr;
    if (hipMalloc((void**)&list, ((size_t)P * 2 + 4) * 4) != hipSuccess) { pl.set_error("out of device memory (window repair)"); return SUFR_HIP_E_NOMEM; }
    orphans.bufs.push_back(list);
    *l_sa = list; *l_lcp = list + P;
    if (hipMemsetAsync(list, 0xFF, (size_t)P * 4, st) != hipSuccess) { pl.set_error("memset failed"); return SUFR_HIP_E_HIP; }
    hipLaunchKernelGGL(k_wide_compact, dim3(nblk), dim3(256), 0, st, (const uint32_t*)pl.sa32.p, (const uint32_t*)pl.lcp32.p, kept, 0u,
                       (const uint32_t*)wblk.p, *l_sa, *l_lcp, (const uint8_t*)not_short);
    hipLaunchKernelGGL(k_wide_count, dim3(nblk), dim3(256), 0, st, (const uint32_t*)pl.sa32.p, kept, 0u, (uint32_t*)wblk.p, (const uint8_t*)is_short);
    hipLaunchKernelGGL(k_wide_scan, dim3(1), dim3(1024), 0, st, (uint32_t*)wblk.p, nblk, pl.sc(Pipeline::SC_TOTAL));
    hipLaunchKernelGGL(k_wide_compact, dim3(nblk), dim3(256), 0, st, (const uint32_t*)pl.sa32.p, (const uint32_t*)pl.lcp32.p, kept, 0u,
                       (const uint32_t*)wblk.p, out_sa, out_lcp, (const uint8_t*)is_short);
    for (uint32_t k = 2; k <= P; k <<= 1)
        for (uint32_t j = k >> 1; j > 0; j >>= 1)
            hipLaunchKernelGGL(k_wide_bitonic, dim3((P + 255) / 256), dim3(256), 0, st, wo, t, n, base, *l_sa, P, k, j);
    if (cnt) hipLaunchKernelGGL(k_wide_list_lcp, dim3((uint32_t)((cnt + 255) / 256)), dim3(256), 0, st, wo, t, n, base, (const uint32_t*)*l_sa, (uint64_t)cnt, *l_lcp);
    if (hipGetLastError() != hipSuccess || hipStreamSynchronize(st) != hipSuccess) { pl.set_error("window repair failed"); return SUFR_HIP_E_HIP; }
    return 0;
}

template <typename OUT>
int sort_device_wide(Pipeline& pl, const void* d_in, uint64_t n, uint32_t flags, uint64_t window, uint64_t margin, OUT* d_sa,
                     OUT* d_lcp, uint64_t cap, uint64_t* num_suffixes_out, sufr_hip_stats* st_out, DevBuf& wtext, DevBuf& wsa,
                     DevBuf& wlcp, DevBuf& wblk)
{
    if (num_suffixes_out) *num_suffixes_out = 0;
    if (!d_in) { pl.set_error("null text"); return SUFR_HIP_E_INVALID; }
    if (hipSetDevice(pl.device) != hipSuccess) { pl.set_error("hipSetDevice failed"); return SUFR_HIP_E_HIP; }
    struct NotResident { Pipeline& p; ~NotResident() { p.resident_text_len = 0; } } not_resident{pl};
    pl.wide_text_len = 0;
    struct Chains { Pipeline& p; uint32_t overlapped = 0; uint64_t doublings = 0; uint32_t exc_retry = 0; uint64_t exc_taken = 0;
                    ~Chains() { p.last_overlapped = overlapped; p.last_doublings = doublings; p.last_exc_retry = exc_retry; p.last_exc_taken = exc_taken; } } chains{pl};
    WidePlan plan = wide_plan(n, window, margin);
    WideOrder wo = {0, 0u, nullptr, 0u};
    if (!pl.opt_mask_offsets.empty()) {
        wo.mode = 2; wo.weight = (uint32_t)pl.opt_mask_offsets.size();
        const uint64_t span = (uint64_t)pl.opt_mask_offsets.back() + 1;
        if (plan.margin < span) {
            const uint64_t limit = SUFR_MAX_TEXT_LEN - 1;
            if (span + 64 > limit) { pl.set_error("seed mask spans more symbols than a window holds"); return SUFR_HIP_E_UNSUPPORTED; }
            if (plan.H + span > limit) plan = wide_plan(n, limit - span - 16, span);
            if (plan.margin < span) plan.margin = span;
        }
    } else if (pl.opt_max_query_len > 0) {
        if (pl.opt_max_query_len < 0xFFFFFFFFull) { wo.mode = 1; wo.L = (uint32_t)pl.opt_max_query_len; }
    }
    if (plan.num < 1) { pl.set_error("text too long for " + std::to_string(WIDE_MAX_WINDOWS) + " windows"); return SUFR_HIP_E_UNSUPPORTED; }
    hipStream_t st = pl.stream;
    int rc;
    hipEvent_t e0 = nullptr, e1 = nullptr;
    if (hipEventCreate(&e0) != hipSuccess || hipEventCreate(&e1) != hipSuccess) { pl.set_error("hipEventCreate failed"); return SUFR_HIP_E_HIP; }
    struct Ev { hipEvent_t a, b; ~Ev() { (void)hipEventDestroy(a); (void)hipEventDestroy(b); } } evguard{e0, e1};
    (void)hipEventRecord(e0, st);
    if ((rc = pl.ensure(wtext, n + TEXT_PAD))) return rc;
    uint8_t* t = (uint8_t*)wtext.p;
    {
        uint64_t grid = (n / 16 + 255) / 256;
        if (grid > 8192) grid = 8192;
        if (grid < 1) grid = 1;
        if ((uintptr_t)d_in & 15u) {
            if (hipMemcpyAsync(t, d_in, n, hipMemcpyDeviceToDevice, st) != hipSuccess) { pl.set_error("text copy failed"); return SUFR_HIP_E_HIP; }
            d_in = t;
        }
        hipLaunchKernelGGL(k_wide_normalize, dim3((uint32_t)grid), dim3(256), 0, st, (const uint8_t*)d_in, t, n,
                           (flags & SUFR_HIP_FLAG_RAW_TEXT) ? 1 : 0, (flags & SUFR_HIP_FLAG_IGNORE_SOFTMASK) ? 1 : 0);
        if (hipMemsetAsync(t + n, 0, TEXT_PAD, st) != hipSuccess || hipStreamSynchronize(st) != hipSuccess) {
            pl.set_error("normalising the text failed"); return SUFR_HIP_E_HIP;
        }
    }
    const uint32_t wflags = flags & ~(uint32_t)SUFR_HIP_FLAG_RAW_TEXT;
    uint64_t wcap = n;
    if (pl.wide_num_shards > 1) {
        wcap = n / pl.wide_num_shards + n / (2ull * pl.wide_num_shards) + ((uint64_t)1 << 20);
        if (wcap > n) wcap = n;
    }
    if ((rc = pl.ensure(wsa, wcap * 4 + 16)) || (rc = pl.ensure(wlcp, wcap * 4 + 16))) return rc;
    if ((rc = pl.ensure(pl.scalars, Pipeline::SC_N * 8))) return rc;
    const bool sharded = pl.wide_num_shards > 1;
    uint64_t sh_lo = 0, sh_hi = 0;
    bool sh_has_hi = false;
    if (sharded) {
        if (wo.mode == 2) { pl.set_error("seed-mask builds in windows are built on one GPU"); return SUFR_HIP_E_UNSUPPORTED; }
        if (wo.mode == 1 && wo.L < 8) { pl.set_error("a max_query_len below 8 symbols ties suffixes across shards: built on one GPU"); return SUFR_HIP_E_UNSUPPORTED; }
        if (pl.opt_max_query_len > 0 && pl.opt_max_query_len < 8) { pl.set_error("a max_query_len below 8 symbols ties suffixes across shards: built on one GPU"); return SUFR_HIP_E_UNSUPPORTED; }
        if (plan.margin < 8) plan.margin = 8;
        const uint64_t ns = n < ((uint64_t)1 << 20) ? n : ((uint64_t)1 << 20), stride = n / ns;
        if ((rc = pl.ensure(wblk, (size_t)ns * 8))) return rc;
        hipLaunchKernelGGL(k_wide_sample, dim3((uint32_t)((ns + 255) / 256)), dim3(256), 0, st, (const uint8_t*)t, n, stride, ns, (unsigned long long*)wblk.p);
        std::vector<uint64_t> smp(ns);
        if (hipMemcpyAsync(smp.data(), wblk.p, (size_t)ns * 8, hipMemcpyDeviceToHost, st) != hipSuccess || hipStreamSynchronize(st) != hipSuccess) {
            pl.set_error("sampling the text failed"); return SUFR_HIP_E_HIP;
        }
        if ((flags & SUFR_HIP_FLAG_DNA) && !(flags & SUFR_HIP_FLAG_ALLOW_AMBIGUITY)) {
            size_t k = 0;
            for (uint64_t v : smp) { const uint8_t c = (uint8_t)(v >> 56); if (c == 'A' || c == 'C' || c == 'G' || c == 'T' || c == '$') smp[k++] = v; }
            smp.resize(k);
        }
        std::sort(smp.begin(), smp.end());
        auto cut = [&](uint32_t k) -> uint64_t { return smp.empty() ? 0ull : smp[(size_t)((unsigned __int128)smp.size() * k / pl.wide_num_shards)]; };
        sh_lo = pl.wide_shard_index ? cut(pl.wide_shard_index) : 0ull;
        sh_has_hi = pl.wide_shard_index + 1 < pl.wide_num_shards;
        sh_hi = sh_has_hi ? cut(pl.wide_shard_index + 1) : 0ull;
    }
    WideWindows ws;
    ws.num = plan.num;
    pl.wide_orphans = 0;
    struct Orphans { std::vector<void*> bufs; ~Orphans() { for (void* q : bufs) (void)hipFree(q); } } orphans;
    uint64_t kept_total = 0;
    uint64_t woff[WIDE_MAX_WINDOWS] = {0};
    sufr_hip_stats acc;
    memset(&acc, 0, sizeof acc);
    for (int i = 0; i < plan.num; i++) {
        const uint64_t base = (uint64_t)i * plan.H;
        const uint64_t own = n - base < plan.H ? n - base : plan.H;
        const uint64_t limit = SUFR_MAX_TEXT_LEN - 1;
        uint64_t m = plan.margin;
        for (int attempt = 0;; attempt++) {
            uint64_t len = own + m;
            if (len > n - base) len = n - base;
            if (len > limit) len = limit;
            const bool to_end = base + len == n;
            if ((rc = pl.ensure(pl.sa32, len * 4 + 4)) || (rc = pl.ensure(pl.lcp32, len * 4 + 4))) return rc;
            uint64_t s = 0;
            sufr_hip_stats wst;
            rc = pl.sort_device_u32(t + base, len, wflags, 0, 1, (uint32_t*)pl.sa32.p, (uint32_t*)pl.lcp32.p, len, &s, &wst);
            chains.overlapped |= pl.last_overlapped; chains.doublings += pl.last_doublings;
            if (pl.last_exc_retry > chains.exc_retry) chains.exc_retry = pl.last_exc_retry;
            if (pl.last_exc_taken) chains.exc_taken = pl.last_exc_taken;
            if (rc) return rc;
            if (i == 0 && attempt == 0) acc = wst;
            else { acc.ms_total += wst.ms_total; acc.ms_normalize += wst.ms_normalize; acc.ms_hist_text += wst.ms_hist_text;
                   acc.ms_partition += wst.ms_partition; acc.ms_passes += wst.ms_passes; acc.ms_finish += wst.ms_finish;
                   acc.ms_deep += wst.ms_deep; acc.deep_records += wst.deep_records; acc.num_large_groups += wst.num_large_groups;
                   if (wst.num_levels > acc.num_levels) acc.num_levels = wst.num_levels; }
            unsigned long long kept = 0, reach = 0;
            const uint32_t* fsa = (const uint32_t*)pl.sa32.p;
            const uint32_t* flcp = (const uint32_t*)pl.lcp32.p;
            uint32_t skip = 0;
            if (sharded && s) {
                unsigned long long rb[2] = {0, 0};
                hipLaunchKernelGGL(k_wide_shard_bounds, dim3(1), dim3(64), 0, st, (const uint8_t*)(t + base), len, fsa, s, sh_lo, sh_hi,
                                   sh_has_hi ? 1 : 0, pl.sc(Pipeline::SC_TOTAL), pl.sc(Pipeline::SC_BAD));
                if (hipMemcpyAsync(&rb[0], pl.sc(Pipeline::SC_TOTAL), 8, hipMemcpyDeviceToHost, st) != hipSuccess ||
                    hipMemcpyAsync(&rb[1], pl.sc(Pipeline::SC_BAD), 8, hipMemcpyDeviceToHost, st) != hipSuccess ||
                    hipStreamSynchronize(st) != hipSuccess) { pl.set_error("finding the shard's ranks failed"); return SUFR_HIP_E_HIP; }
                if (rb[1] < rb[0]) rb[1] = rb[0];
                const uint64_t a0 = rb[0] & ~(uint64_t)3;
                skip = (uint32_t)(rb[0] - a0);
                fsa += a0; flcp += a0;
                s = rb[1] - a0;
                if (s <= skip) s = 0;
            }
            if ((kept_total + s) * 4 + 16 > wsa.cap || (kept_total + s) * 4 + 16 > wlcp.cap) {
                const uint64_t want = kept_total + s + ((kept_total + s) >> 3);
                if ((rc = pl.ensure_keep(wsa, (want < n ? want : n) * 4 + 16)) || (rc = pl.ensure_keep(wlcp, (want < n ? want : n) * 4 + 16))) return rc;
            }
            uint32_t* out_sa = (uint32_t*)wsa.p + kept_total;
            uint32_t* out_lcp = (uint32_t*)wlcp.p + kept_total;
            if (s) {
                const uint32_t nblk = (uint32_t)((s + WIDE_BLK - 1) / WIDE_BLK);
                if ((rc = pl.ensure(wblk, (size_t)nblk * 4))) return rc;
                hipLaunchKernelGGL(k_wide_count, dim3(nblk), dim3(256), 0, st, fsa, s, (uint32_t)own, (uint32_t*)wblk.p, (const uint8_t*)nullptr, skip);
                hipLaunchKernelGGL(k_wide_scan, dim3(1), dim3(1024), 0, st, (uint32_t*)wblk.p, nblk, pl.sc(Pipeline::SC_TOTAL));
                hipLaunchKernelGGL(k_wide_compact, dim3(nblk), dim3(256), 0, st, fsa, flcp, s,
                                   (uint32_t)own, (const uint32_t*)wblk.p, out_sa, out_lcp, (const uint8_t*)nullptr, skip);
                if (hipMemcpyAsync(&kept, pl.sc(Pipeline::SC_TOTAL), 8, hipMemcpyDeviceToHost, st) != hipSuccess ||
                    hipStreamSynchronize(st) != hipSuccess) { pl.set_error("filtering a window failed"); return SUFR_HIP_E_HIP; }
                if (!to_end && kept > 1) {
                    if (hipMemsetAsync(pl.sc(Pipeline::SC_BAD), 0, 8, st) != hipSuccess) { pl.set_error("memset failed"); return SUFR_HIP_E_HIP; }
                    const uint64_t rblk = (kept + 255) / 256;
                    hipLaunchKernelGGL(k_wide_reach, dim3((uint32_t)(rblk < 4096 ? rblk : 4096)), dim3(256), 0, st, (const uint32_t*)out_sa,
                                       (const uint32_t*)out_lcp, (uint64_t)kept, pl.sc(Pipeline::SC_BAD));
                    if (hipMemcpyAsync(&reach, pl.sc(Pipeline::SC_BAD), 8, hipMemcpyDeviceToHost, st) != hipSuccess ||
                        hipStreamSynchronize(st) != hipSuccess) { pl.set_error("checking a window failed"); return SUFR_HIP_E_HIP; }
                }
            }
            if (!to_end && reach >= len) {
                uint64_t widest = limit - own < n - base - own ? limit - own : n - base - own;
                if (pl.opt_wide_retry && widest > pl.opt_wide_retry) widest = pl.opt_wide_retry;
                if (attempt == 0 && widest > m) { m = widest; continue; }
                if (wo.mode == 2) {
                    pl.set_error("a seed-mask window ran into its end (the margin covers the mask's span: this cannot happen)");
                    return SUFR_HIP_E_HIP;
                }
                if (ws.num >= WIDE_MAX_WINDOWS) { pl.set_error("too many windows need a repair list"); return SUFR_HIP_E_UNSUPPORTED; }
                uint32_t *l_sa = nullptr, *l_lcp = nullptr;
                uint64_t nshort = 0, nrest = 0;
                if ((rc = repair_window(pl, wo, t, n, base, len, out_sa, out_lcp, (uint64_t)kept, wblk, orphans, &l_sa, &l_lcp, &nshort, &nrest))) {
                    if (rc == SUFR_HIP_E_UNSUPPORTED)
                        pl.set_error("a repeat of " + std::to_string(reach - own) + " or more symbols crosses the end of window " + std::to_string(i) +
                                     " and ties " + std::to_string(nshort) + " suffixes through it: more than the whole-text repair takes (2^22)");
                    return rc;
                }
                ws.w[ws.num++] = {l_sa, l_lcp, base, nshort};
                pl.wide_orphans += nshort;
                kept = nrest;
            }
            ws.w[i] = {nullptr, nullptr, base, (uint64_t)kept};
            woff[i] = kept_total;
            kept_total += kept;
            break;
        }
    }
    for (int i = 0; i < plan.num; i++) { ws.w[i].sa = (const uint32_t*)wsa.p + woff[i]; ws.w[i].lcp = (const uint32_t*)wlcp.p + woff[i]; }
    for (int i = plan.num; i < ws.num; i++) kept_total += ws.w[i].count;
    if (num_suffixes_out) *num_suffixes_out = kept_total;
    if (kept_total > cap) {
        pl.set_error("output capacity " + std::to_string(cap) + " < num_suffixes " + std::to_string(kept_total));
        return SUFR_HIP_E_CAPACITY;
// ... 48 lines not shown
```

Baseline: 29.68 billion suffixes/s.

## Resolve two-member tie groups by direct pair walk before tie level

```diff
diff --git a/include/sufr_hip.h b/include/sufr_hip.h
--- a/include/sufr_hip.h
+++ b/include/sufr_hip.h
@@ -74,6 +74,8 @@
 int  sufr_hip_set_overlap_min(sufr_hip_ctx *ctx, uint64_t min_records);
 int  sufr_hip_overlapped(const sufr_hip_ctx *ctx);
 uint64_t sufr_hip_doublings(const sufr_hip_ctx *ctx);
+int  sufr_hip_set_pair_walk(sufr_hip_ctx *ctx, uint32_t mode);
+int  sufr_hip_pairs_walked(const sufr_hip_ctx *ctx, uint64_t *resolved, uint64_t *left_tied);
 int  sufr_hip_set_exc_max_affected(sufr_hip_ctx *ctx, uint64_t max_affected);
 int  sufr_hip_exc_retry(const sufr_hip_ctx *ctx);
 uint64_t sufr_hip_exc_taken(const sufr_hip_ctx *ctx);
diff --git a/sufr_amd/_lib.py b/sufr_amd/_lib.py
--- a/sufr_amd/_lib.py
+++ b/sufr_amd/_lib.py
@@ -71,7 +71,7 @@
 
 EXPORTS = [
     "sufr_hip_abi_version", "sufr_hip_device_count", "sufr_hip_create", "sufr_hip_destroy",
-    "sufr_hip_last_error", "sufr_hip_set_stream", "sufr_hip_synchronize", "sufr_hip_set_window", "sufr_hip_set_window_retry", "sufr_hip_set_array_budget", "sufr_hip_window_repairs", "sufr_hip_set_overlap_min", "sufr_hip_overlapped", "sufr_hip_doublings", "sufr_hip_set_exc_max_affected", "sufr_hip_exc_retry", "sufr_hip_exc_taken", "sufr_hip_normalize", "sufr_hip_sort_device_u32",
+    "sufr_hip_last_error", "sufr_hip_set_stream", "sufr_hip_synchronize", "sufr_hip_set_window", "sufr_hip_set_window_retry", "sufr_hip_set_array_budget", "sufr_hip_window_repairs", "sufr_hip_set_overlap_min", "sufr_hip_overlapped", "sufr_hip_doublings", "sufr_hip_set_pair_walk", "sufr_hip_pairs_walked", "sufr_hip_set_exc_max_affected", "sufr_hip_exc_retry", "sufr_hip_exc_taken", "sufr_hip_normalize", "sufr_hip_sort_device_u32",
     "sufr_hip_sort_device_u64", "sufr_hip_stitch_device_u32", "sufr_hip_stitch_device_u64", "sufr_hip_build_u32", "sufr_hip_build_u64", "sufr_hip_lcp_pair",
     "sufr_read_sequence_file", "sufr_sequence_data_free", "sufr_write_file", "sufr_hip_create_file", "sufr_hip_create_from_sequence",
     "sufr_hip_shard_build", "sufr_write_frame", "sufr_hip_shard_write", "sufr_hip_create_from_sequence_multi",
@@ -199,6 +199,8 @@
     L.sufr_hip_set_overlap_min.argtypes = [vp, u64]; L.sufr_hip_set_overlap_min.restype = C.c_int
     L.sufr_hip_overlapped.argtypes = [vp]; L.sufr_hip_overlapped.restype = C.c_int
     L.sufr_hip_doublings.argtypes = [vp]; L.sufr_hip_doublings.restype = u64
+    L.sufr_hip_set_pair_walk.argtypes = [vp, C.c_uint32]; L.sufr_hip_set_pair_walk.restype = C.c_int
+    L.sufr_hip_pairs_walked.argtypes = [vp, C.POINTER(u64), C.POINTER(u64)]; L.sufr_hip_pairs_walked.restype = C.c_int
     L.sufr_hip_set_exc_max_affected.argtypes = [vp, u64]; L.sufr_hip_set_exc_max_affected.restype = C.c_int
     L.sufr_hip_exc_retry.argtypes = [vp]; L.sufr_hip_exc_retry.restype = C.c_int
     L.sufr_hip_exc_taken.argtypes = [vp]; L.sufr_hip_exc_taken.restype = u64
@@ -389,6 +391,15 @@
     def doublings(self) -> int:
         return int(lib().sufr_hip_doublings(self._h))
 
+    def set_pair_walk(self, mode: int = 0):
+        self.check(lib().sufr_hip_set_pair_walk(self._h, mode))
+
+    @property
+    def pairs_walked(self):
+        r, t = C.c_uint64(0), C.c_uint64(0)
+        self.check(lib().sufr_hip_pairs_walked(self._h, C.byref(r), C.byref(t)))
+        return int(r.value), int(t.value)
+
     def set_exc_max_affected(self, max_affected: int = 0):
         self.check(lib().sufr_hip_set_exc_max_affected(self._h, max_affected))
 
diff --git a/sufr_amd/csrc/sufr_capi.inc b/sufr_amd/csrc/sufr_capi.inc
--- a/sufr_amd/csrc/sufr_capi.inc
+++ b/sufr_amd/csrc/sufr_capi.inc
@@ -276,6 +276,22 @@
 int sufr_hip_overlapped(const sufr_hip_ctx* ctx) { return ctx ? (int)ctx->pl.last_overlapped : 0; }
 uint64_t sufr_hip_doublings(const sufr_hip_ctx* ctx) { return ctx ? ctx->pl.last_doublings : 0; }
 
+int sufr_hip_set_pair_walk(sufr_hip_ctx* ctx, uint32_t mode)
+{
+    if (!ctx) return SUFR_HIP_E_INVALID;
+    if (mode > 2u) { ctx->pl.set_error("pair walk mode " + std::to_string(mode) + ": 0 (default), 1 (always) or 2 (never)"); return SUFR_HIP_E_INVALID; }
+    ctx->pl.opt_pair_walk = mode;
+    return 0;
+}
+
+int sufr_hip_pairs_walked(const sufr_hip_ctx* ctx, uint64_t* resolved, uint64_t* left_tied)
+{
+    if (!ctx) return SUFR_HIP_E_INVALID;
+    if (resolved) *resolved = ctx->pl.last_pairs_resolved;
+    if (left_tied) *left_tied = ctx->pl.last_pairs_left;
+    return 0;
+}
+
 int sufr_hip_set_exc_max_affected(sufr_hip_ctx* ctx, uint64_t max_affected)
 {
     if (!ctx) return SUFR_HIP_E_INVALID;
diff --git a/sufr_amd/csrc/sufr_host_stubs.cpp b/sufr_amd/csrc/sufr_host_stubs.cpp
--- a/sufr_amd/csrc/sufr_host_stubs.cpp
+++ b/sufr_amd/csrc/sufr_host_stubs.cpp
@@ -52,6 +52,13 @@
 int sufr_hip_set_overlap_min(sufr_hip_ctx* ctx, uint64_t) { return no_device(ctx); }
 int sufr_hip_overlapped(const sufr_hip_ctx*) { return 0; }
 uint64_t sufr_hip_doublings(const sufr_hip_ctx*) { return 0; }
+int sufr_hip_set_pair_walk(sufr_hip_ctx* ctx, uint32_t) { return no_device(ctx); }
+int sufr_hip_pairs_walked(const sufr_hip_ctx*, uint64_t* resolved, uint64_t* left_tied)
+{
+    if (resolved) *resolved = 0;
+    if (left_tied) *left_tied = 0;
+    return 0;
+}
 int sufr_hip_set_exc_max_affected(sufr_hip_ctx* ctx, uint64_t) { return no_device(ctx); }
 int sufr_hip_exc_retry(const sufr_hip_ctx*) { return 0; }
 uint64_t sufr_hip_exc_taken(const sufr_hip_ctx*) { return 0; }
diff --git a/sufr_amd/csrc/sufr_kernels.hip b/sufr_amd/csrc/sufr_kernels.hip
--- a/sufr_amd/csrc/sufr_kernels.hip
+++ b/sufr_amd/csrc/sufr_kernels.hip
@@ -5,6 +5,7 @@
 
 #include "sufr_device.h"
 #include "sufr_runkey.h"
+#include "sufr_tiepairs.h"
 
 namespace sufr {
 #ifdef SUFR_HIP_PROBES
@@ -1402,6 +1403,18 @@
         }
     }
     return lim;
+}
+
+struct PairWalk { uint64_t k; bool parted, a_first; };
+__device__ __forceinline__ PairWalk walk_pair(const uint8_t* __restrict__ text, uint64_t n, const KeyParams& kp, uint64_t a, uint64_t b)
+{
+    const uint64_t lim = n - (a > b ? a : b);
+    uint32_t ca = 0, cb = 0;
+    PairWalk w;
+    w.k = kp.packed ? walk_lcp_packed(kp.packed, kp.b, n, a, b, WALK_CAP, ca, cb) : walk_lcp(text, n, a, b, WALK_CAP);
+    w.parted = !(w.k == WALK_CAP && w.k < lim);
+    w.a_first = w.parted && (w.k == lim ? a > b : (kp.packed ? ca < cb : text[a + w.k] < text[b + w.k]));
+    return w;
 }
 
 static constexpr uint64_t WALK_MAX = (1ull << 62) - 1;
@@ -1615,16 +1628,13 @@
             if (__ballot(ph0 || ph1) != 0ull) {
                 auto walk = [&](uint32_t slot, uint32_t mine, uint32_t dnew) {
                     const uint32_t other = si[slot + 1];
-                    const uint64_t a = (uint64_t)mine + dnew, b = (uint64_t)other + dnew;
-                    const uint64_t lim = n - (a > b ? a : b);
-                    uint32_t ca = 0, cb = 0;
-                    const uint64_t k = kp.packed ? walk_lcp_packed(kp.packed, kp.b, n, a, b, WALK_CAP, ca, cb)
-                                                 : walk_lcp(text, n, a, b, WALK_CAP);
-                    if (k == WALK_CAP && k < lim) {
+                    const PairWalk w = walk_pair(text, n, kp, (uint64_t)mine + dnew, (uint64_t)other + dnew);
+                    if (!w.parted) {
                         sg[slot] = 0xffffffffu; sg[slot + 1] = 0xffffffffu;
                         return;
                     }
-                    const bool mine_first = k == lim ? a > b : (kp.packed ? ca < cb : text[a + k] < text[b + k]);
+                    const uint64_t k = w.k;
+                    const bool mine_first = w.a_first;
                     si[slot] = mine_first ? mine : other;
                     si[slot + 1] = mine_first ? other : mine;
                     sg[slot] = 0u;
@@ -1654,14 +1664,9 @@
         const bool walk_next = ktype == 1 && round >= 1 && !(popts & 2u) && __ballot(extra0 | extra1) == 0ull;
         if (walk_next) {
             auto wkey = [&](uint32_t mine, uint32_t ref, uint32_t d) -> uint64_t {
-                const uint64_t a = (uint64_t)mine + d, r2 = (uint64_t)ref + d;
-                const uint64_t lim = n - (a > r2 ? a : r2);
-                uint32_t ca = 0, cb = 0;
-                const uint64_t L = kp.packed ? walk_lcp_packed(kp.packed, kp.b, n, a, r2, WALK_CAP, ca, cb)
-                                             : walk_lcp(text, n, a, r2, WALK_CAP);
-                if (L == WALK_CAP && L < lim) return walk_key(true, false, 0);
-                const bool below = L == lim ? a > r2 : (kp.packed ? ca < cb : text[a + L] < text[r2 + L]);
-                return walk_key(false, below, L);
+                const PairWalk w = walk_pair(text, n, kp, (uint64_t)mine + d, (uint64_t)ref + d);
+                if (!w.parted) return walk_key(true, false, 0);
+                return walk_key(false, w.a_first, w.k);
             };
             if (act0) {
                 dd0 += advance(k0);
@@ -1869,6 +1874,114 @@
             }
         }
     }
+}
+
+static constexpr uint32_t PSC_MEMBERS = 0, PSC_RESOLVED = 64, PSC_PAIRS = 128, PSC_N = 129;
+
+__device__ __forceinline__ bool pair_path_taken(const unsigned long long* __restrict__ psc, uint32_t force, uint32_t min_permille)
+{
+    if (force) return true;
+    unsigned long long mem = psc[PSC_MEMBERS + lane_id()];
+#pragma unroll
+    for (int o = 32; o > 0; o >>= 1) mem += shfl64(mem, (int)(lane_id() ^ (uint32_t)o));
+    return 2ull * psc[PSC_PAIRS] * 1000ull >= mem * (unsigned long long)min_permille;
+}
+
+__device__ __forceinline__ TieMask128 window_pair_heads(const unsigned long long* __restrict__ wmask, uint32_t w, uint32_t nwin)
+{
+    const ulonglong2 mm = *reinterpret_cast<const ulonglong2*>(wmask + (size_t)w * 4);
+    TieMask128 none = {0ull, 0ull};
+    if ((mm.x | mm.y) == 0ull) return none;
+    const ulonglong2 hh = *reinterpret_cast<const ulonglong2*>(wmask + (size_t)w * 4 + 2);
+    uint32_t next = 0;
+    if (((mm.y >> 62) != 0ull) && w + 1 < nwin)
+        next = tie_next_bits(wmask[(size_t)(w + 1) * 4], wmask[(size_t)(w + 1) * 4 + 2]);
+    return tie_pair_heads(mm.x, mm.y, hh.x, hh.y, next);
+}
+
+__device__ __forceinline__ uint32_t block_scan_256(uint32_t v, uint32_t& total)
+{
+    __shared__ uint32_t s_wave[4];
+    const uint32_t ln = lane_id(), wv = threadIdx.x >> 6;
+    uint32_t inc = v;
+#pragma unroll
+    for (int o = 1; o < 64; o <<= 1) { const uint32_t t = (uint32_t)__shfl_up(inc, o, WAVE); if (ln >= (uint32_t)o) inc += t; }
+    if (ln == 63u) s_wave[wv] = inc;
+    __syncthreads();
+    uint32_t before = 0;
+    for (uint32_t k = 0; k < wv; k++) before += s_wave[k];
+    total = s_wave[0] + s_wave[1] + s_wave[2] + s_wave[3];
+    return before + inc - v;
+}
+
+__global__ void __launch_bounds__(256)
+k_pair_counts(const unsigned long long* __restrict__ wmask, uint32_t nwin, uint32_t* __restrict__ blkcnt,
+              unsigned long long* __restrict__ psc)
+{
+    __shared__ uint32_t s_mem[4];
+    const uint32_t w = blockIdx.x * 256 + threadIdx.x;
+    uint32_t mem = 0, cnt = 0;
+    if (w < nwin) {
+        mem = (uint32_t)(__popcll(wmask[(size_t)w * 4]) + __popcll(wmask[(size_t)w * 4 + 1]));
+        if (mem) cnt = tie_mask_count(window_pair_heads(wmask, w, nwin));
+    }
+#pragma unroll
+    for (int o = 32; o > 0; o >>= 1) mem += (uint32_t)__shfl_down(mem, o, WAVE);
+    if (lane_id() == 0) s_mem[threadIdx.x >> 6] = mem;
+    uint32_t total;
+    (void)block_scan_256(cnt, total);
+    if (threadIdx.x == 0) {
+        blkcnt[blockIdx.x] = total;
+        const uint32_t m = s_mem[0] + s_mem[1] + s_mem[2] + s_mem[3];
+        if (m) atomicAdd(&psc[PSC_MEMBERS + (blockIdx.x & 63u)], (unsigned long long)m);
+    }
+}
+
+__global__ void __launch_bounds__(256)
+k_pair_list(const unsigned long long* __restrict__ wmask, uint32_t nwin, const uint32_t* __restrict__ blkcnt,
+            const uint32_t* __restrict__ blkoff, const unsigned long long* __restrict__ psc, uint32_t force, uint32_t min_permille,
+            uint32_t cap, uint32_t* __restrict__ pairlist)
+{
+    if (!pair_path_taken(psc, force, min_permille)) return;
+    if (!blkcnt[blockIdx.x]) return;
+    const uint32_t w = blockIdx.x * 256 + threadIdx.x;
+    TieMask128 ph = {0ull, 0ull};
+    if (w < nwin) ph = window_pair_heads(wmask, w, nwin);
+    uint32_t total;
+    uint32_t e = blkoff[blockIdx.x] + block_scan_256(tie_mask_count(ph), total);
+    for (uint64_t left = ph.lo; left && e < cap; left &= left - 1) pairlist[e++] = w * 128u + (uint32_t)__builtin_ctzll(left);
+    for (uint64_t left = ph.hi; left && e < cap; left &= left - 1) pairlist[e++] = w * 128u + 64u + (uint32_t)__builtin_ctzll(left);
+}
+
+__global__ void __launch_bounds__(256)
+k_pair_walk(const uint32_t* __restrict__ pairlist, unsigned long long* __restrict__ psc, uint32_t force, uint32_t min_permille,
+            uint32_t cap, const uint8_t* __restrict__ text, uint64_t n, KeyParams kp, uint32_t K, uint32_t* SA,
+            uint32_t* __restrict__ LCP, unsigned long long* wmask)
+{
+    if (!pair_path_taken(psc, force, min_permille)) return;
+    const unsigned long long listed = psc[PSC_PAIRS] < cap ? psc[PSC_PAIRS] : (unsigned long long)cap;
+    uint32_t done = 0;
+    for (uint64_t e = (uint64_t)blockIdx.x * 256 + threadIdx.x; e < listed; e += (uint64_t)gridDim.x * 256) {
+        const uint32_t r = pairlist[e];
+        const uint32_t s0 = SA[r], s1 = SA[r + 1];
+        const PairWalk w = walk_pair(text, n, kp, (uint64_t)s0 + K, (uint64_t)s1 + K);
+        if (!w.parted) continue;
+        if (!w.a_first) { SA[r] = s1; SA[r + 1] = s0; }
+        LCP[r + 1] = K + (uint32_t)w.k;
+        const size_t at = (size_t)(r >> 7) * 4 + ((r >> 6) & 1u);
+        const uint32_t bit = r & 63u;
+        atomicAnd(&wmask[at + 2], ~(1ull << bit));
+        if (bit != 63u) atomicAnd(&wmask[at], ~(3ull << bit));
+        else {
+            const uint32_t r1 = r + 1;
+            atomicAnd(&wmask[at], ~(1ull << 63));
+            atomicAnd(&wmask[(size_t)(r1 >> 7) * 4 + ((r1 >> 6) & 1u)], ~1ull);
+        }
+        done++;
+    }
+#pragma unroll
+    for (int o = 32; o > 0; o >>= 1) done += (uint32_t)__shfl_down(done, o, WAVE);
+    if (lane_id() == 0 && done) atomicAdd(&psc[PSC_RESOLVED + (((blockIdx.x * 256 + threadIdx.x) >> 6) & 63u)], (unsigned long long)done);
 }
 
 __global__ void __launch_bounds__(256)
diff --git a/sufr_amd/csrc/sufr_launch.inc b/sufr_amd/csrc/sufr_launch.inc
--- a/sufr_amd/csrc/sufr_launch.inc
+++ b/sufr_amd/csrc/sufr_launch.inc
@@ -60,7 +60,7 @@
     DevBuf recA, recB;
     DevBuf rankbuf, dposbuf, deferbuf, unresbuf, posbitsbuf, dblf[7], dblg[6];
     DevBuf headsA, headsB, sizes, starts, partials;
-    DevBuf tilefirst, runends, tileany, nexttile, nextblk, depthA, depthB, period, remapbuf, flagsbuf, packedbuf, wmaskbuf, wcntbuf, recoff, runoff, wlflag, wlhead, wloff, candbuf, keepbuf, plancnt, fixbuf;
+    DevBuf tilefirst, runends, tileany, nexttile, nextblk, depthA, depthB, period, remapbuf, flagsbuf, packedbuf, wmaskbuf, wcntbuf, recoff, runoff, wlflag, wlhead, wloff, candbuf, keepbuf, plancnt, fixbuf, pairsc, pairbuf;
     DevBuf rg_misc, rg_blk, rg_blkoff, rg_rs, rg_rl, rg_E, rg_L, rg_V, rg_tab[2], rg_off[2], rg_long[2], rg_tmax[2], rg_hist, rg_depth;
     DevBuf cumbuf, dmapbuf, identbuf[16], grouptab, gcur, leafcnt, leafoff, leafbase, leafcur, bigflag, bigoff;
     DevBuf rawtab, presbuf, rawtot, valsbuf, startbuf;
@@ -69,6 +69,9 @@
     bool overlap_chains = true;
     static constexpr uint64_t OVERLAP_MIN_DEFAULT = (uint64_t)1 << 22;
     uint64_t opt_overlap_min = 0;
+    static constexpr uint32_t PAIR_MIN_PERMILLE = 50;
+    uint32_t opt_pair_walk = 0;
+    uint64_t last_pairs_resolved = 0, last_pairs_left = 0;
     uint32_t last_overlapped = 0;
     uint64_t dbl_entries = 0;
     uint64_t last_doublings = 0;
@@ -321,7 +324,7 @@
         (void)hipSetDevice(device);
         DevBuf* all[] = {&text, &bytehist, &lut, &table, &bintot, &binbase, &scalars, &keyA, &keyB, &idxA,
                          &idxB, &recA, &recB, &headsA, &headsB, &sizes, &starts, &partials, &sa32, &lcp32,
-                         &tilefirst, &runends, &tileany, &nexttile, &nextblk, &depthA, &depthB, &period, &remapbuf, &flagsbuf, &packedbuf, &wmaskbuf, &wcntbuf, &recoff, &runoff, &wlflag, &wlhead, &wloff, &candbuf, &keepbuf, &plancnt, &fixbuf,
+                         &tilefirst, &runends, &tileany, &nexttile, &nextblk, &depthA, &depthB, &period, &remapbuf, &flagsbuf, &packedbuf, &wmaskbuf, &wcntbuf, &recoff, &runoff, &wlflag, &wlhead, &wloff, &candbuf, &keepbuf, &plancnt, &fixbuf, &pairsc, &pairbuf,
                          &rg_misc, &rg_blk, &rg_blkoff, &rg_rs, &rg_rl, &rg_E, &rg_L, &rg_V, &rg_tab[0], &rg_tab[1], &rg_off[0], &rg_off[1], &rg_long[0], &rg_long[1], &rg_tmax[0], &rg_tmax[1], &rg_hist, &rg_depth,
                          &exc_pos, &exc_byte, &exc_sorted, &exc_sa, &exc_lcp, &exc_bits, &exc_blk, &exc_off, &exc_list, &exc_list2, &exc_pmin, &exc_roff, &exc_all_sa, &exc_all_lcp,
                          &cumbuf, &dmapbuf, &rawtab, &presbuf, &rawtot, &valsbuf, &startbuf, &grouptab, &gcur, &leafcnt, &leafoff, &leafbase, &leafcur, &bigflag, &bigoff,
@@ -348,7 +351,7 @@
         if (also_text) { release(text); resident_text_len = 0; }
         DevBuf* big[] = {&recA, &recB, &keyA, &keyB, &idxA, &idxB, &packedbuf, &runends, &startbuf, &wmaskbuf, &wcntbuf, &fixbuf, &exc_sa, &exc_lcp, &exc_bits, &exc_all_sa, &exc_all_lcp,
                          &headsA, &headsB, &rankbuf, &dposbuf, &deferbuf, &unresbuf, &posbitsbuf, &depthA, &depthB, &period,
-                         &recoff, &runoff, &candbuf, &keepbuf, &optA, &optB, &optC, &optD, &optE};
+                         &recoff, &runoff, &candbuf, &keepbuf, &pairbuf, &optA, &optB, &optC, &optD, &optE};
         for (auto* b : big) if (b->cap >= ((size_t)16 << 20)) release(*b);
         for (auto& b : dblf) release(b);
         for (auto& b : dblg) release(b);
@@ -1594,7 +1597,7 @@
                         uint32_t num_shards, uint32_t* d_sa, uint32_t* d_lcp, uint64_t cap,
                         uint64_t* num_suffixes_out, sufr_hip_stats* st_out)
     {
-        last_overlapped = 0; last_doublings = 0; dbl_entries = 0;
+        last_overlapped = 0; last_doublings = 0; dbl_entries = 0; last_pairs_resolved = 0; last_pairs_left = 0;
         if (helper) helper->dbl_entries = 0;
         if (!exc_disable) { last_exc_retry = 0; last_exc_taken = 0; }
         const int rc = sort_build(d_in, n, flags, shard_index, num_shards, d_sa, d_lcp, cap, num_suffixes_out, st_out);
@@ -2408,6 +2411,8 @@
         if ((rc = ensure(fixbuf, (size_t)fixcap * 4))) return rc;
         HIP_TRY(zero_later(wmaskbuf.p, (size_t)nwin * 32));
         HIP_TRY(zero_later(sc(SC_NFIX), 8));
+        if ((rc = ensure(pairsc, (size_t)PSC_N * 8))) return rc;
+        HIP_TRY(zero_later(pairsc.p, (size_t)PSC_N * 8));
         HIP_TRY(zero_flush());
         fo.SA = B.d_sa; fo.LCP = B.d_lcp; fo.wmask = (unsigned long long*)wmaskbuf.p; fo.fixlist = (uint32_t*)fixbuf.p;
         fo.nfix = (uint32_t*)sc(SC_NFIX); fo.fixcap = fixcap; fo.b = kp.b; fo.K = kp.K;
@@ -2510,8 +2515,6 @@
         HIP_TRY(hipEventRecord(ev[6], stream));
         hipLaunchKernelGGL(k_fix_window_lcp, dim3(1024), dim3(256), 0, stream, (const uint32_t*)fixbuf.p,
                            (const uint32_t*)sc(SC_NFIX), fixcap, (const Rec*)xr[1], B.d_lcp, kp.b, kp.K);
-        hipLaunchKernelGGL(k_tie_counts, dim3((nwin + 255) / 256), dim3(256), 0, stream,
-                           (const unsigned long long*)wmaskbuf.p, nwin, (uint32_t*)wcntbuf.p, B.wcnt_stride);
         HIP_TRY(hipGetLastError());
         HIP_TRY(hipEventRecord(ev[7], stream));
         B.st.num_levels = 1;
@@ -2619,6 +2622,31 @@
         const uint32_t* icur = d_sa;
         if ((rc = ensure(recoff, (size_t)nwin * 4))) return rc;
         if ((rc = ensure(runoff, (size_t)nwin * 4))) return rc;
+        const bool pair_path = !mql_fast && opt_pair_walk != 2u && !(finish_opts & (1u << 29));
+        const uint32_t pair_cap = m0 / 8u + 4096u;
+        unsigned long long psums[PSC_N];
+        if (pair_path) {
+            if ((rc = ensure(pairbuf, (size_t)pair_cap * 4))) return rc;
+            const uint32_t nblk = (nwin + 255u) / 256u;
+            uint32_t* blkcnt = (uint32_t*)runoff.p; uint32_t* blkoff = (uint32_t*)recoff.p;
+            unsigned long long* psc = (unsigned long long*)pairsc.p;
+            const uint32_t force = opt_pair_walk == 1u ? 1u : 0u;
+            hipLaunchKernelGGL(k_pair_counts, dim3(nblk), dim3(256), 0, stream,
+                               (const unsigned long long*)wmaskbuf.p, nwin, blkcnt, psc);
+            if ((rc = scan_u32(blkcnt, nblk, blkoff, psc + PSC_PAIRS))) return rc;
+            hipLaunchKernelGGL(k_pair_list, dim3(nblk), dim3(256), 0, stream,
+                               (const unsigned long long*)wmaskbuf.p, nwin, (const uint32_t*)blkcnt, (const uint32_t*)blkoff,
+                               (const unsigned long long*)psc, force, PAIR_MIN_PERMILLE, pair_cap, (uint32_t*)pairbuf.p);
+            uint32_t grid = (pair_cap + 255u) / 256u;
+            if (grid > 8192u) grid = 8192u;
+            hipLaunchKernelGGL(k_pair_walk, dim3(grid), dim3(256), 0, stream, (const uint32_t*)pairbuf.p, psc, force,
+                               PAIR_MIN_PERMILLE, pair_cap, (const uint8_t*)d_text, n, kp, (uint32_t)kp.K, d_sa, d_lcp,
+                               (unsigned long long*)wmaskbuf.p);
+            HIP_TRY(hipGetLastError());
+            HIP_TRY(read_at_sync(psums, psc, sizeof psums));
+        }
+        hipLaunchKernelGGL(k_tie_counts, dim3((nwin + 255) / 256), dim3(256), 0, stream,
+                           (const unsigned long long*)wmaskbuf.p, nwin, cnt, wcnt_stride);
         if ((rc = scan_u32((const uint32_t*)cnt, nwin, (uint32_t*)recoff.p, sc(SC_TMP0)))) return rc;
         unsigned long long tot2[2] = {0, 0};
         if ((rc = scan_u32((const uint32_t*)(cnt + wcnt_stride), nwin, (uint32_t*)runoff.p, sc(SC_TMP1)))) return rc;
@@ -2629,6 +2657,16 @@
         if ((uint32_t)nf > B.fixcap) { set_error("internal error: window list overflow"); return SUFR_HIP_E_HIP; }
         const unsigned long long tot_rec = tot2[0], tot_run = tot2[1];
         const uint32_t m2 = (uint32_t)tot_rec, L2 = (uint32_t)tot_run;
+        if (pair_path) {
+            unsigned long long members = 0, resolved = 0;
+            for (uint32_t i = 0; i < 64; i++) { members += psums[PSC_MEMBERS + i]; resolved += psums[PSC_RESOLVED + i]; }
+            const unsigned long long pairs = psums[PSC_PAIRS];
+            const bool taken = opt_pair_walk == 1u || 2ull * pairs * 1000ull >= members * (unsigned long long)PAIR_MIN_PERMILLE;
+            const unsigned long long walked = taken ? (pairs < pair_cap ? pairs : (unsigned long long)pair_cap) : 0ull;
+            last_pairs_resolved += resolved; last_pairs_left += walked - resolved;
+            if (debug) fprintf(stderr, "[sufr_hip debug] pair path: tie records=%llu pairs=%llu %s resolved=%llu handed back=%llu\n",
+                               members, pairs, taken ? "walked" : "(too few: not walked)", resolved, walked - resolved);
+        }
         if (debug) fprintf(stderr, "[sufr_hip debug] tie level: runs=%u records=%u\n", L2, m2);
         if (m2 == 0) return 0;
         st.num_levels++;
diff --git a/sufr_amd/csrc/sufr_tiepairs.h b/sufr_amd/csrc/sufr_tiepairs.h
--- /dev/null
+++ b/sufr_amd/csrc/sufr_tiepairs.h
@@ -0,0 +1,38 @@
+#pragma once
+#include <stdint.h>
+
+#if defined(__HIPCC__)
+#define SUFR_TP_HD __host__ __device__ __forceinline__
+#else
+#define SUFR_TP_HD static inline
+#endif
+
+namespace sufr {
+
+struct TieMask128 { uint64_t lo, hi; };
+
+SUFR_TP_HD TieMask128 tie_continues(uint64_t M0, uint64_t M1, uint64_t H0, uint64_t H1)
+{
+    return TieMask128{M0 & ~H0, M1 & ~H1};
+}
+
+SUFR_TP_HD uint32_t tie_next_bits(uint64_t nextM0, uint64_t nextH0)
+{
+    return (uint32_t)((nextM0 & ~nextH0) & 3ull);
+}
+
+SUFR_TP_HD TieMask128 tie_pair_heads(uint64_t M0, uint64_t M1, uint64_t H0, uint64_t H1, uint32_t next)
+{
+    const TieMask128 T = tie_continues(M0, M1, H0, H1);
+    const uint64_t n0 = (uint64_t)(next & 1u), n1 = (uint64_t)((next >> 1) & 1u);
+    const uint64_t T1lo = (T.lo >> 1) | (T.hi << 63), T1hi = (T.hi >> 1) | (n0 << 63);
+    const uint64_t T2lo = (T.lo >> 2) | (T.hi << 62), T2hi = (T.hi >> 2) | (n0 << 62) | (n1 << 63);
+    return TieMask128{M0 & H0 & T1lo & ~T2lo, M1 & H1 & T1hi & ~T2hi};
+}
+
+SUFR_TP_HD uint32_t tie_mask_count(TieMask128 m)
+{
+    return (uint32_t)(__builtin_popcountll(m.lo) + __builtin_popcountll(m.hi));
+}
+
+}
diff --git a/sufr_amd/csrc/sufr_wide.inc b/sufr_amd/csrc/sufr_wide.inc
--- a/sufr_amd/csrc/sufr_wide.inc
+++ b/sufr_amd/csrc/sufr_wide.inc
@@ -538,8 +538,8 @@
     if (hipSetDevice(pl.device) != hipSuccess) { pl.set_error("hipSetDevice failed"); return SUFR_HIP_E_HIP; }
     struct NotResident { Pipeline& p; ~NotResident() { p.resident_text_len = 0; } } not_resident{pl};
     pl.wide_text_len = 0;
-    struct Chains { Pipeline& p; uint32_t overlapped = 0; uint64_t doublings = 0; uint32_t exc_retry = 0; uint64_t exc_taken = 0;
-                    ~Chains() { p.last_overlapped = overlapped; p.last_doublings = doublings; p.last_exc_retry = exc_retry; p.last_exc_taken = exc_taken; } } chains{pl};
+    struct Chains { Pipeline& p; uint32_t overlapped = 0; uint64_t doublings = 0; uint32_t exc_retry = 0; uint64_t exc_taken = 0, pairs_resolved = 0, pairs_left = 0;
+                    ~Chains() { p.last_pairs_resolved = pairs_resolved; p.last_pairs_left = pairs_left; p.last_overlapped = overlapped; p.last_doublings = doublings; p.last_exc_retry = exc_retry; p.last_exc_taken = exc_taken; } } chains{pl};
     WidePlan plan = wide_plan(n, window, margin);
     WideOrder wo = {0, 0u, nullptr, 0u};
     if (!pl.opt_mask_offsets.empty()) {
@@ -634,6 +634,7 @@
             sufr_hip_stats wst;
             rc = pl.sort_device_u32(t + base, len, wflags, 0, 1, (uint32_t*)pl.sa32.p, (uint32_t*)pl.lcp32.p, len, &s, &wst);
             chains.overlapped |= pl.last_overlapped; chains.doublings += pl.last_doublings;
+            chains.pairs_resolved += pl.last_pairs_resolved; chains.pairs_left += pl.last_pairs_left;
             if (pl.last_exc_retry > chains.exc_retry) chains.exc_retry = pl.last_exc_retry;
             if (pl.last_exc_taken) chains.exc_taken = pl.last_exc_taken;
             if (rc) return rc;
```

Result: faster. 30.15 billion suffixes/s, median of 6 (+1.6%).
